# avikde/robobee3d

Measured on AMD Instinct MI355X. Metric: closed-loop MPC steps/sec (QP+dyn), higher is better.
Workload: dtype f32

## Files before the change

### robobee3d_amd/asmgen.py

```python
import os
import struct

from . import symbolic

HERE = os.path.dirname(os.path.abspath(__file__))

SWITCH_PREFIXES = ("UMPC_ASM_", "UMPC_ASM64_", "UMPC_QP_", "UMPC_X_")
NOT_SWITCHES = ("UMPC_QP_KERNEL", "UMPC_QP_NO_ASM", "UMPC_ASM_SKEW_US", "UMPC_ASM_SKEW_GROUPS")


def generator_switches():
    return {k: v for k, v in sorted(os.environ.items()) if k.startswith(SWITCH_PREFIXES) and k not in NOT_SWITCHES}


def switch_banner():
    sw = generator_switches()
    return "// generator switches: " + (" ".join("%s=%s" % kv for kv in sw.items()) if sw else "none (defaults = the shipped kernels)")

XV_COUNT, XV_BASE = 0, 246
NLDS = 160
NVZ = 36
FAC_L, FAC_DI, FAC_Q, FAC_LOEQ, FAC_M = 0, 213, 297, 342, 378
FAC_ROWS = 390
WS_DS, WS_ES, WS_C, WS_XPREV, WS_DY = 390, 435, 474, 475, 520
# ... 137 lines not shown
    while remaining:
        ready = [o for o in remaining if o[1] in final]
        used, emitted = set(), []
        for o in ready:
            if o[2] in used:
                continue
            for o2 in ready:
                if o2[2] not in used and ok(o, o2):
                    used.update((o[2], o2[2]))
                    emitted.append((o, o2) if reg[o[0]] % 2 == 0 else (o2, o))
                    break
        deferred = []
        for o in ready:
            if o[2] in used:
                continue
            if any(ok(o, o2) for o2 in remaining if o2[1] not in final and o2[2] not in used):
                deferred.append(o)
            else:
                used.add(o[2])
                emitted.append((o,))
        if not emitted:
            used.add(deferred[0][2])
            emitted.append((deferred[0],))
        out += emitted
        for o in remaining:
            if o[2] in used:
                indeg[o[0]] -= 1
                if indeg[o[0]] == 0:
                    final.add(o[0])
        remaining = [o for o in remaining if o[2] not in used]
    return out


def solve_plan(s):
    xs, zs, _, _ = slot_maps(s)
    reg = [w_reg(s, k, xs, zs) for k in range(s.nk)]
    fwd = solve_schedule(s, reg, "fwd", same_src=BCAST)
    couples, late = {}, {}
    if BCAST:
        singles = [(k, g[0]) for k, g in enumerate(fwd) if len(g) == 1]
        used = set()
        for a_, (ka, oa) in enumerate(singles):
            if oa[2] in used:
                continue
            for kb, ob in singles[a_ + 1:]:
                if ob[2] not in used and ob[0] == oa[0] and reg[ob[1]] == (reg[oa[1]] ^ 1):
                    couples[oa[2]] = ob[2]
                    used.update((oa[2], ob[2]))
                    break
        moved = {j for j in couples}
        late = {jb: ja for ja, jb in couples.items()}
        byj = {g[0][2]: g for g in fwd if len(g) == 1}
        out = []
        for g in fwd:
            if len(g) == 1 and g[0][2] in moved:
                continue
            if len(g) == 1 and g[0][2] in late:
                out.append(byj[late[g[0][2]]])
            out.append(g)
        fwd = out
    bwd = []
    k = len(fwd) - 1
    while k >= 0:
        g = fwd[k]
        if len(g) == 1 and g[0][2] in late:
            ob, oa = g[0], fwd[k - 1][0]
            h = [(oa[1], oa[0], oa[2]), (ob[1], ob[0], ob[2])]
            if reg[h[0][0]] % 2:
                h.reverse()
            bwd.append(tuple(h))
            k -= 2
            continue
        h = [(sr, d, j) for (d, sr, j) in g]
        if len(h) == 2 and h[0][0] == h[1][0]:
            bwd.append((h[1],))
            bwd.append((h[0],))
        else:
            if len(h) == 2 and reg[h[0][0]] % 2:
                h.reverse()
            bwd.append(tuple(h))
        k -= 1
    units = []
    k = 0
    while k < len(fwd):
        g = fwd[k]
        if len(g) == 1 and g[0][2] in couples and k + 1 < len(fwd) and len(fwd[k + 1]) == 1 and fwd[k + 1][0][2] == couples[g[0][2]]:
            units.append([g[0][2], fwd[k + 1][0][2]])
            k += 2
        else:
            units.append([o[2] for o in g])
            k += 1
    order, pending = [], []
    for u in units:
        if len(u) == 2 and len(order) % 2:
            pending.append(u)
            continue
        order += u
        while pending and len(order) % 2 == 0:
            order += pending.pop(0)
    assert not pending, "odd number of single entries before a trailing pair"
    pos = [0] * len(s.L_i)
    for p_, j in enumerate(order):
        pos[j] = p_
    for g in fwd + bwd:
        if len(g) == 2:
            a, b = pos[g[0][2]], pos[g[1][2]]
            assert a // 2 == b // 2, "paired entries must share an aligned pair"
    return fwd, bwd, pos


def l_positions(N=3, perm=None):
    return solve_plan(symbolic.analyse(N, perm))[2]


def prologue(e, s):
    import numpy as np
    for reg, val in ((S_ALPHA, 1.6), (S_OMA, float(np.float32(1.0) - np.float32(1.6))), (S_SIGMA, 1e-6),
                     (S_RINV, 0.01), (S_RHO, 100.0)):
        e("s_mov_b32", "s%d" % reg, f32bits(val))
        e("s_mov_b32", "s%d" % (reg + 1), f32bits(val))
    _row_ptr(e, S_P, S_WS, FAC_L + NLDS)
    nrest = len(s.L_i) - NLDS + s.nk + s.nx + 2 * s.N * symbolic.NY + 12
    assert A_LO == nrest - 12 - 2 * s.N * symbolic.NY and A_M == nrest - 12 and nrest <= 256
    for r in range(nrest):
        e("global_load_dword", "a%d" % r, "v0", "s[%d:%d]" % (S_P, S_P + 1))
        _adv(e, S_P)
    e("s_mov_b64", "s[%d:%d]" % (S_P, S_P + 1), "s[%d:%d]" % (S_CTRL, S_CTRL + 1))
    xs, zs, _, _ = slot_maps(s)
    for base, n, sl in ((V_X, s.nx, xs), (V_Y, s.nc, zs), (V_Z, s.nc, zs)):
        for r in range(n):
            e("global_load_dword", "v%d" % (base + sl[r]), "v0", "s[%d:%d]" % (S_P, S_P + 1))
            _adv(e, S_P)
    e("s_waitcnt", "vmcnt(0)")


def epilogue(e, s, z_is_l):
    w = 0
    xs, zs, _, _ = slot_maps(s)
    neq = 2 * s.N * symbolic.NY
    for base, n, sl in ((V_X, s.nx, xs), (V_Y, s.nc, zs), (V_Z, s.nc, zs)):
        for r in range(n):
            if base == V_Z and z_is_l and r < neq:
                t = V_RING + r % 16
                e("v_accvgpr_read_b32", "v%d" % t, "a%d" % (A_LO + r))
                e("ds_write_b32", "v1", "v%d" % t, (w // 4) * 1024 + (w % 4) * 4)
            else:
                e("ds_write_b32", "v1", "v%d" % (base + sl[r]), (w // 4) * 1024 + (w % 4) * 4)
            w += 1
    e("s_waitcnt", "vmcnt(0) lgkmcnt(0)")


class Fetcher:

    def __init__(self, e, la=3):
        self.e, self.la = e, la
        self.nds = 0
        self.waited = -1
        self.lds_ahead = int(os.environ.get("UMPC_ASM_LDS_AHEAD", "12" if NRING == 4 else "20"))
        self.merge = int(os.environ.get("UMPC_ASM_LDS_MERGE", "1" if NRING == 4 else "2"))

    def run(self, ops):
        e = self.e
        n = len(ops)
        inst_of = [None] * n
        insts = []
        slots = [None] * NRING
        for i, op in enumerate(ops):
            if op["src"] and op["src"][0] == "L":
                qd = op["src"][1] // 4
                hit = [k for k in slots if k is not None and insts[k]["quad"] == qd]
                if hit:
                    insts[hit[0]]["last"] = i
                    inst_of[i] = hit[0]
                    continue
                free = [sl for sl in range(NRING) if slots[sl] is None]
                sl = free[0] if free else min(range(NRING), key=lambda q: insts[slots[q]]["last"])
                insts.append(dict(quad=qd, first=i, last=i, slot=sl, prev=slots[sl], issued=None))
                slots[sl] = len(insts) - 1
                inst_of[i] = slots[sl]

        def issue(it):
            e("ds_read_b128", "v[%d:%d]" % (ring_base(it["slot"]), ring_base(it["slot"]) + 3), "v1",
              it["quad"] * 1024)
            it["issued"] = self.nds
            self.nds += 1

        next_inst = 0
        atemp = {}
        next_acc = 0
        acc_rr = 0
        for i in range(n):
            while next_acc < n and next_acc < i + self.la:
                op = ops[next_acc]
                if op["src"] and op["src"][0] in ("A", "A2"):
                    t = V_AT + 2 * (acc_rr % N_ATP)
                    acc_rr += 1
                    e("v_accvgpr_read_b32", "v%d" % t, "a%d" % op["src"][1])
                    if op["src"][0] == "A2":
                        e("v_accvgpr_read_b32", "v%d" % (t + 1), "a%d" % op["src"][2])
                    atemp[next_acc] = t
                next_acc += 1
            while next_inst < len(insts):
                it = insts[next_inst]
                prev = insts[it["prev"]] if it["prev"] is not None else None
                if it["first"] <= i + self.lds_ahead and (prev is None or prev["last"] < i):
                    issue(it)
                    next_inst += 1
                else:
                    break
            op = ops[i]
            if op["src"] is None:
                op["emit"](None)
            elif op["src"][0] in ("A", "A2"):
                op["emit"](atemp.pop(i))
            else:
                it = insts[inst_of[i]]
                if it["issued"] is None:
                    assert inst_of[i] == next_inst and (it["prev"] is None or insts[it["prev"]]["last"] < i)
                    issue(it)
                    next_inst += 1
                if it["first"] == i and it["issued"] > self.waited:
                    upto = min(self.nds - 1, it["issued"] + self.merge)
                    e("s_waitcnt", "lgkmcnt(%d)" % min(15, self.nds - 1 - upto))
                    self.waited = upto if self.nds - 1 - upto <= 15 else it["issued"]
                op["emit"](ring_base(it["slot"]) + op["src"][1] % 4)


def _vp(n):
    assert n % 2 == 0
    return ("v[%d:%d]" % (n, n + 1), 0, 1)


def _vb(n):
    lo = n - (n % 2)
    return ("v[%d:%d]" % (lo, lo + 1), n % 2, n % 2)


def _sb(n):
    assert n % 2 == 0
    return ("s[%d:%d]" % (n, n + 1), 0, 0)


def pk(e, mnem, dst, srcs, neg=None):
    assert dst % 2 == 0
    neg = neg or [0] * len(srcs)
    mods = dict(op_sel=[s_[1] for s_ in srcs], op_sel_hi=[s_[2] for s_ in srcs], neg_lo=list(neg), neg_hi=list(neg))
    e(mnem, "v[%d:%d]" % (dst, dst + 1), *[s_[0] for s_ in srcs], mods)


def despace(ops, window=int(os.environ.get("UMPC_ASM_WINDOW", "12"))):
    pending, out = list(ops), []
    last = [frozenset(), frozenset()]
    while pending:
        best, bscore = 0, None
        blocked_w, blocked_r = set(), set()
        for k, o in enumerate(pending[:window]):
            movable = not (o["r"] & blocked_w) and not (o["w"] & blocked_w) and not (o["w"] & blocked_r)
            if movable:
                score = (2 if (o["r"] | o["w"]) & last[1] else 0) + (1 if (o["r"] | o["w"]) & last[0] else 0)
                if bscore is None or score < bscore:
                    best, bscore = k, score
                    if score == 0:
                        break
            blocked_w |= o["w"]
            blocked_r |= o["r"]
        o = pending.pop(best)
        out.append(o)
        last = [last[1], o["w"]]
    return out


def body(e, s, first, capture, plan, lv=False, delta_in_w=False, qzero=frozenset(), lzero=frozenset(), dy3_in_w=False):
    nx, nc, nk = s.nx, s.nc, s.nk
    neq = 2 * s.N * symbolic.NY
    xs, zs, xinv, zinv = slot_maps(s)
    fwd, bwd, lpos = plan

    def wreg(k):
        return w_reg(s, k, xs, zs)
    W = lambda k: "v%d" % wreg(k)
    WX = lambda j: V_W + xs[j]
    WZ = lambda i: V_WZ + zs[i]
    XR = lambda j: V_X + xs[j]
    YR = lambda i: V_Y + zs[i]
    ZR = lambda i: V_Z + zs[i]
    X = lambda j: "v%d" % XR(j)
    Y = lambda i: "v%d" % YR(i)
    Z = lambda i: "v%d" % ZR(i)
    v = lambda n: "v%d" % n
    sA, sO, sS, sRi, sRh = ("s%d" % r for r in (S_ALPHA, S_OMA, S_SIGMA, S_RINV, S_RHO))
    ptr = "s[%d:%d]" % (S_P2, S_P2 + 1)
    f = Fetcher(e)
    ops = []

    def op(src, fn, w=(), r=()):
        ops.append(dict(src=src, emit=fn, w=frozenset(w), r=frozenset(r)))

    assert NVZ == neq and not (lv and first)

    def l_src(j):
        if lpos[j] < NLDS:
            return ("L", lpos[j])
        if lv and lpos[j] < NLDS + NVZ:
            return ("V", V_Z + lpos[j] - NLDS)
        if NLDS + NVZ <= lpos[j] < NLDS + NVZ + XV_COUNT:
            return ("V", XV_BASE + lpos[j] - NLDS - NVZ)
        return ("A", A_L + lpos[j] - NLDS)

    if capture and not delta_in_w:
        _row_ptr(e, S_P2, S_WS, WS_XPREV)
        for j in range(nx):
            e("global_store_dword", "v0", X(j), ptr)
            _adv(e, S_P2)
    for p_ in range(0, nx - 1, 2):
        j0, j1 = xinv[p_], xinv[p_ + 1]
        rw = dict(w=(V_W + p_, V_W + p_ + 1), r=(V_X + p_, V_X + p_ + 1))
        if j0 in qzero and j1 in qzero:
            op(None, lambda t, p_=p_: pk(e, "v_pk_mul_f32", V_W + p_, [_sb(S_SIGMA), _vp(V_X + p_)]), **rw)
        elif j0 in qzero or j1 in qzero:
            jn, h = (j1, 1) if j0 in qzero else (j0, 0)

            def mixed(t, p_=p_, h=h):
                pk(e, "v_pk_mul_f32", V_W + p_, [_sb(S_SIGMA), _vp(V_X + p_)])
                e("v_sub_f32", v(V_W + p_ + h), v(V_W + p_ + h), v(t))
            op(("A", A_Q + jn), mixed, **rw)
        else:
            op(("A2", A_Q + j0, A_Q + j1),
               lambda t, p_=p_: pk(e, "v_pk_fma_f32", V_W + p_, [_sb(S_SIGMA), _vp(V_X + p_), _vp(t)], [0, 0, 1]), **rw)
    if nx % 2:
        jl = xinv[nx - 1]
        if jl in qzero:
            op(None, lambda t, jl=jl: e("v_mul_f32", v(WX(jl)), sS, X(jl)), w=(WX(jl),), r=(XR(jl),))
        else:
            op(("A", A_Q + jl), lambda t, jl=jl: e("v_fma_f32", v(WX(jl)), sS, X(jl), "-" + v(t)), w=(WX(jl),), r=(XR(jl),))
    assert all(zinv[p_] < neq for p_ in range(neq)) and neq % 2 == 0
    for p_ in range(0, neq, 2):
        if lv:
            i0, i1 = zinv[p_], zinv[p_ + 1]
            rw = dict(w=(V_WZ + p_, V_WZ + p_ + 1), r=(V_Y + p_, V_Y + p_ + 1))
            if i0 in lzero and i1 in lzero:
                op(None, lambda t, p_=p_: pk(e, "v_pk_mul_f32", V_WZ + p_, [_sb(S_RINV), _vp(V_Y + p_)], [1, 0]), **rw)
            elif i0 in lzero or i1 in lzero:
                inz, h = (i1, 1) if i0 in lzero else (i0, 0)

                def mixed_z(t, p_=p_, h=h):
                    pk(e, "v_pk_mul_f32", V_WZ + p_, [_sb(S_RINV), _vp(V_Y + p_)], [1, 0])
                    e("v_add_f32", v(V_WZ + p_ + h), v(V_WZ + p_ + h), v(t))
                op(("A", A_LO + inz), mixed_z, **rw)
            else:
                op(("A2", A_LO + i0, A_LO + i1),
                   lambda t, p_=p_: pk(e, "v_pk_fma_f32", V_WZ + p_, [_sb(S_RINV), _vp(V_Y + p_), _vp(t)], [1, 0, 0]), **rw)
        else:
            op(None, lambda t, p_=p_: pk(e, "v_pk_fma_f32", V_WZ + p_, [_sb(S_RINV), _vp(V_Y + p_), _vp(V_Z + p_)], [1, 0, 0]),
               w=(V_WZ + p_, V_WZ + p_ + 1), r=(V_Y + p_, V_Y + p_ + 1, V_Z + p_, V_Z + p_ + 1))
    for i in range(neq, nc):
        op(("A", A_M + 9 + i - neq), lambda t, i=i: e("v_fma_f32", v(WZ(i)), "-" + v(t), Y(i), Z(i)),
           w=(WZ(i),), r=(YR(i), ZR(i)))

    def solve_ops(sched):
        for g in sched:
            if len(g) == 1:
                d, sr, j = g[0]
                src = l_src(j)
                if src[0] == "V":
                    op(None, lambda t, d=d, sr=sr, r=src[1]: e("v_fmac_f32", W(d), v(r), W(sr)),
                       w=(wreg(d),), r=(wreg(d), wreg(sr)))
                else:
                    op(src, lambda t, d=d, sr=sr: e("v_fmac_f32", W(d), v(t), W(sr)),
                       w=(wreg(d),), r=(wreg(d), wreg(sr)))
                continue
            (d0, s0_, j0), (d1, s1_, j1) = g
            rd, r0, r1 = wreg(d0), wreg(s0_), wreg(s1_)
            assert rd % 2 == 0 and wreg(d1) == rd + 1 and r0 // 2 == r1 // 2 and lpos[j0] // 2 == lpos[j1] // 2
            srcp = ("v[%d:%d]" % (r0 - r0 % 2, r0 - r0 % 2 + 1), r0 % 2, r1 % 2)
            rw = dict(w=(rd, rd + 1), r=(rd, rd + 1, r0, r1))
            pe = lpos[j0] - lpos[j0] % 2
            lsel = (lpos[j0] % 2, lpos[j1] % 2)
            if pe < NLDS:
                op(("L", pe), lambda t, rd=rd, srcp=srcp, lsel=lsel:
                   pk(e, "v_pk_fma_f32", rd, [("v[%d:%d]" % (t, t + 1), lsel[0], lsel[1]), srcp, _vp(rd)], [0, 0, 0]), **rw)
            elif (lv and pe < NLDS + NVZ) or NLDS + NVZ <= pe < NLDS + NVZ + XV_COUNT:
                t = V_Z + pe - NLDS if pe < NLDS + NVZ else XV_BASE + pe - NLDS - NVZ
                op(None, lambda _t, t=t, rd=rd, srcp=srcp, lsel=lsel:
                   pk(e, "v_pk_fma_f32", rd, [("v[%d:%d]" % (t, t + 1), lsel[0], lsel[1]), srcp, _vp(rd)], [0, 0, 0]), **rw)
            else:
                src = ("A2", A_L + lpos[j0] - NLDS, A_L + lpos[j1] - NLDS)
                op(src, lambda t, rd=rd, srcp=srcp: pk(e, "v_pk_fma_f32", rd, [_vp(t), srcp, _vp(rd)], [0, 0, 0]), **rw)

    solve_ops(fwd)
    kof = {wreg(k): k for k in range(nk)}
    for r0 in range(V_W, V_Z, 2):
        k0, k1 = kof.get(r0), kof.get(r0 + 1)
        if k0 is not None and k1 is not None:
            op(("A2", A_D + k0, A_D + k1), lambda t, r0=r0: pk(e, "v_pk_mul_f32", r0, [_vp(r0), _vp(t)]),
               w=(r0, r0 + 1), r=(r0, r0 + 1))
        elif k0 is not None or k1 is not None:
            k, r = (k0, r0) if k0 is not None else (k1, r0 + 1)
            op(("A", A_D + k), lambda t, r=r: e("v_mul_f32", v(r), v(t), v(r)), w=(r,), r=(r,))
    solve_ops(bwd)
    f.run(despace(ops) if os.environ.get("UMPC_ASM_DESPACE", "0") == "1" else ops)
    for p_ in range(0, nx - 1, 2):
        t = V_TT + 2 * ((p_ // 2) % 4)
        pk(e, "v_pk_mul_f32", t, [_sb(S_OMA), _vp(V_X + p_)])
        if capture and delta_in_w:
            pk(e, "v_pk_fma_f32", t, [_sb(S_ALPHA), _vp(V_W + p_), _vp(t)])
            pk(e, "v_pk_add_f32", V_W + p_, [_vp(t), _vp(V_X + p_)], [0, 1])
            e("v_pk_mov_b32", "v[%d:%d]" % (V_X + p_, V_X + p_ + 1), "v[%d:%d]" % (t, t + 1), "v[%d:%d]" % (t, t + 1),
              dict(op_sel=[0, 1], op_sel_hi=[0, 0], neg_lo=[0, 0], neg_hi=[0, 0]))
        else:
            pk(e, "v_pk_fma_f32", V_X + p_, [_sb(S_ALPHA), _vp(V_W + p_), _vp(t)])
    if nx % 2:
        jl = xinv[nx - 1]
        e("v_mul_f32", v(V_TT), sO, X(jl))
        if capture and delta_in_w:
            e("v_fma_f32", v(V_TT), sA, v(WX(jl)), v(V_TT))
            e("v_sub_f32", v(WX(jl)), v(V_TT), X(jl))
            e("v_mov_b32", X(jl), v(V_TT))
        else:
            e("v_fma_f32", X(jl), sA, v(WX(jl)), v(V_TT))
    if capture and first and not delta_in_w:
        _row_ptr(e, S_P2, S_WS, WS_DY)
    if not first:
        for p_ in range(0, neq, 2):
            t = V_TT + 2 * ((p_ // 2) % 2)
            pk(e, "v_pk_add_f32", t, [_vp(V_WZ + p_), _vp(V_Y + p_)], [0, 1])
            if capture and delta_in_w:
                pk(e, "v_pk_mul_f32", V_WZ + p_, [_sb(S_ALPHA), _vp(t)])
            elif capture:
                pk(e, "v_pk_mul_f32", t + 4, [_sb(S_ALPHA), _vp(t)])
                for h in range(2):
                    _row_ptr(e, S_P2, S_WS, WS_DY + zinv[p_ + h])
                    e("global_store_dword", "v0", v(t + 4 + h), ptr)
            pk(e, "v_pk_fma_f32", V_Y + p_, [_sb(S_ALPHA), _vp(t), _vp(V_Y + p_)])
    for i in range(nc):
        eq = i < neq
        if eq and not first:
            continue
        if first and eq and i % 16 == 0:
            for w in range(min(16, neq - i)):
                e("v_accvgpr_read_b32", v(V_RING + w), "a%d" % (A_LO + i + w))
        b = V_TT + 4 * (i % 2)
        t1, t2, t3, t4 = v(b), v(b + 1), v(b + 2), v(b + 3)
        if eq:
            rinv, rho = sRi, sRh
        else:
            k = i - neq
            rinv, rho = v(V_AT), v(V_AT + 1)
            e("v_accvgpr_read_b32", rinv, "a%d" % (A_M + 9 + k))
            e("v_accvgpr_read_b32", rho, "a%d" % (A_M + 6 + k))
            e("v_accvgpr_read_b32", v(V_AT + 2), "a%d" % (A_M + k))
            e("v_accvgpr_read_b32", v(V_AT + 3), "a%d" % (A_M + 3 + k))
        nu = v(WZ(i))
        e("v_fma_f32", t1, "-" + rinv, Y(i), Z(i))
        e("v_fma_f32", t1, rinv, nu, t1)
        e("v_mul_f32", t2, sO, Z(i))
        e("v_fma_f32", t1, sA, t1, t2)
        if eq:
            zn = v(V_RING + i % 16)
            e("v_sub_f32", t2, t1, zn)
        else:
            e("v_fma_f32", t3, rinv, Y(i), t1)
            e("v_max_f32", t3, t3, v(V_AT + 2))
            e("v_min_f32", Z(i), t3, v(V_AT + 3))
            e("v_sub_f32", t2, t1, Z(i))
        if dy3_in_w and not eq and not capture:
            e("v_mul_f32", nu, rho, t2)
            e("v_add_f32", Y(i), Y(i), nu)
            continue
        e("v_mul_f32", t2, rho, t2)
        e("v_add_f32", Y(i), Y(i), t2)
        if capture and delta_in_w:
            e("v_mov_b32", nu, t2)
        elif capture:
            if not first:
                _row_ptr(e, S_P2, S_WS, WS_DY + i)
            e("global_store_dword", "v0", t2, ptr)
            if first:
                _adv(e, S_P2)


def program(N=3, perm=None):
    s = symbolic.analyse(N, perm)
    plan = solve_plan(s)
    e = Emit()
    prologue(e, s)
    e("s_cmp_lt_i32", "s%d" % S_ITERS, 1)
    e("s_cbranch_scc1", "9f")
    body(e, s, first=True, capture=True, plan=plan)
    for p_ in range(NVZ):
        e("v_accvgpr_read_b32", "v%d" % (V_Z + p_), "a%d" % (A_L + p_))
    e("s_sub_i32", "s%d" % S_CNT, "s%d" % S_ITERS, 2)
    e("s_cmp_lt_i32", "s%d" % S_CNT, 1)
    e("s_cbranch_scc1", "8f")
    e("label", "7")
    body(e, s, first=False, capture=False, plan=plan, lv=True)
    e("s_sub_i32", "s%d" % S_CNT, "s%d" % S_CNT, 1)
    e("s_cmp_gt_i32", "s%d" % S_CNT, 0)
    e("s_cbranch_scc1", "7b")
    e("label", "8")
    e("s_cmp_lt_i32", "s%d" % S_ITERS, 2)
    e("s_cbranch_scc1", "6f")
    body(e, s, first=False, capture=True, plan=plan, lv=True)
    e("label", "6")
    epilogue(e, s, z_is_l=True)
    e("s_branch", "5f")
    e("label", "9")
    epilogue(e, s, z_is_l=False)
    e("label", "5")
    return e.ins, s


def fmt(t):
    m = t[0]
    if m == "label":
        return "%s:" % t[1]
    mods = ""
    if isinstance(t[-1], dict):
        d = t[-1]
        t = t[:-1]
        mods = " " + " ".join("%s:[%s]" % (k, ",".join(map(str, d[k]))) for k in ("op_sel", "op_sel_hi", "neg_lo", "neg_hi"))
    a = [("0x%x" % x if (m == "s_mov_b32" and isinstance(x, int)) else str(x)) for x in t[1:]]
    if m in ("ds_read_b128", "ds_write_b128", "ds_write_b32"):
        return "%s %s, %s offset:%s" % (m, a[0], a[1], a[2])
    if m in ("global_load_dword", "global_store_dword"):
        return "%s %s, %s, %s" % (m, a[0], a[1], a[2])
    if m == "s_waitcnt":
        return "s_waitcnt " + " ".join(a)
    return "%s %s%s" % (m, ", ".join(a), mods)


def write(path=None, N=3, perm=None):
    path = path or os.path.join(HERE, "csrc", "umpc_admm_asm.h")
    ins, s = program(N, perm)
    lpos = solve_plan(s)[2]
    store_l = " ".join("LDSW_(%d) = -LX_(%d);" % (lpos[j], j) if lpos[j] < NLDS else "ROW_(%d) = -LX_(%d);" % (FAC_L + lpos[j], j)
                       for j in range(len(lpos)))
    used_s = [S_P, S_P + 1, S_CNT, S_P2, S_P2 + 1] + list(range(S_ALPHA, S_RHO + 2))
    clob = ['"memory"', '"scc"', '"vcc"'] + ['"v%d"' % i for i in range(2, V_END)] + \
           ['"a%d"' % i for i in range(256)] + ['"s%d"' % i for i in used_s]
    lab7 = [k for k, t in enumerate(ins) if t == ("label", "7")][0]
    lab8 = [k for k, t in enumerate(ins) if t == ("label", "8")][0]
    out = ["// GENERATED by robobee3d_amd/asmgen.py -- do not edit.", switch_banner(),
           "// ADMM phase of the fp32 step kernel: %d instructions, middle-iteration body %d." % (len(ins), lab8 - lab7),
           "#pragma once",
           "namespace umpcasm {",
           "constexpr int FAC_L = %d, FAC_DI = %d, FAC_Q = %d, FAC_LOEQ = %d, FAC_M = %d, FAC_ROWS = %d;" %
           (FAC_L, FAC_DI, FAC_Q, FAC_LOEQ, FAC_M, FAC_ROWS),
           "constexpr int WS_DS = %d, WS_ES = %d, WS_C = %d, WS_XPREV = %d, WS_DY = %d, WS_ROWS = %d;" %
           (WS_DS, WS_ES, WS_C, WS_XPREV, WS_DY, WS_ROWS),
           "constexpr int LDS_BYTES_PER_LANE = %d;" % (NLDS * 4),
           "}  // namespace umpcasm",
           "// Phase A -> loop hand-off of the factor: entry j of L (CSC order) goes NEGATED to its storage position (asmgen.solve_plan):",
           "// LDS word LDSW_(p) for p < %d, workspace row ROW_(FAC_L + p) (-> AGPR) otherwise." % NLDS,
           "#define UMPC_ASM_STORE_L(LDSW_, ROW_, LX_) do { %s } while (0)" % store_l,
           "// inputs: v0 = 4*robot, v1 = lane LDS address, s[4:5] = workspace, s[6:7] = ctrl, s10 = 4*B, s11 = maxIter",
           "#define UMPC_ADMM_ASM(voff, ldsaddr, ws, ctrl, stride, iters) asm volatile( \\"]
    for t in ins:
        out.append('  "%s\\n" \\' % fmt(t))
    out.append('  : : "{v0}"(voff), "{v1}"(ldsaddr), "{s[4:5]}"(ws), "{s[6:7]}"(ctrl), "{s10}"(stride), "{s11}"(iters) \\')
    out.append("  : " + ", ".join(clob) + ")")
    txt = "\n".join(out) + "\n"
    old = open(path).read() if os.path.exists(path) else None
    if old != txt:
        with open(path, "w") as fh:
            fh.write(txt)
    return path, len(ins)


WS_BASE, CTRL_BASE, STRIDE = 1 << 20, 1 << 30, 4096


def simulate(ins, mem_ws, mem_ctrl, iters, lds=None):
    import numpy as np
    from . import isasim
    lds = np.zeros(NLDS, np.float32) if lds is None else lds
    m = isasim.Machine(ins, regions=[(WS_BASE, STRIDE, mem_ws), (CTRL_BASE, STRIDE, mem_ctrl)],
                       sgpr={S_WS: WS_BASE, S_CTRL: CTRL_BASE, S_STRIDE: STRIDE, S_ITERS: iters}, vgpr={0: 0},
                       lds=lds.view(np.uint32).reshape(1, -1), max_exec=400000)
    return isasim.run(m)


if __name__ == "__main__":
    p, n = write()
    print("wrote", p, n, "instructions")
```

### robobee3d_amd/asmstep.py

```python
import os
import struct

from . import asmgen, symbolic
from .asmgen import (A_D, A_L, A_LO, A_M, A_Q, NLDS, NVZ, S_ALPHA, S_CNT, S_ITERS, S_OMA, S_RHO, S_RINV, S_SIGMA,
                     V_W, V_WZ, V_X, V_Y, V_Z, Emit, f32bits, pk, _sb, _vp)

HERE = os.path.dirname(os.path.abspath(__file__))

PTRS = ["state", "ctrl", "ref", "ws", "out", "stats", "status", "info", "Ib", "gain", "aT0",
        "taskf", "weights", "wl", "wlu", "wlw",
        "done"]
NPTR_RES = 11
INTS = ["stride", "K", "maxIter", "nsub", "plant", "seq"]
TAIL_INTS = ["refstep"]
FLOATS = ["dt", "dtg", "Tmax", "wpr", "wpf", "ws_", "wvr", "wvf", "wds", "wthrust", "wmom",
          "iwpr", "iwpf", "iws", "iwvr", "iwvf", "iwds", "iwthrust", "iwmom",
          "Ib0", "Ib1", "Ib2", "Ibi0", "Ibi1", "Ibi2", "h", "hh", "h6", "taulim", "gpl", "idt", "mbg"]
WNAMES = ["wpr", "wpf", "ws_", "wvr", "wvf", "wds", "wthrust", "wmom"]
WROW = {"ws_": 0, "wds": 1, "wpr": 2, "wpf": 3, "wvr": 4, "wvf": 5, "wthrust": 6, "wmom": 7}
A_W, A_IW = 230, 238
S_PARAM = 4
S_PBLK = 2
S_PTR = {n: 40 + 2 * k for k, n in enumerate(PTRS[:NPTR_RES])}
S_PTR["taskf"], S_PTR["weights"] = 0, 96
S_PTR["wl"], S_PTR["wlu"], S_PTR["wlw"] = 30, 32, 34
S_INT = {"stride": 10, "K": 13, "maxIter": S_ITERS, "nsub": 5, "plant": 39}
S_F = {n: 64 + k for k, n in enumerate(FLOATS)}
assert max(S_F.values()) <= 95
S_STEP, S_SUB, S_RUIZ = 12, 15, 15
S_MBAD, S_MP0 = 62, 14
S_M0, S_M1, S_M2, S_M3 = 30, 32, 34, 36
S_C = {"minscal": 16, "maxscal": 17, "c45": 18, "eps10": 19, "eps": 38, "rho": 6, "rinv": 7, "rmin": 8,
       "rmininv": 9, "infty_ms": 100, "rhotol": 101}
S_TMP = 4
OFF = {}
_o = 0
for _n in PTRS:
    OFF[_n] = _o
    _o += 8
for _n in INTS + FLOATS + TAIL_INTS:
    OFF[_n] = _o
    _o += 4
PARAM_BYTES = _o
HIST_INTS = ["statestep", "outstep", "statusstep", "infostep"]
HIST_OFF = (PARAM_BYTES + 7) // 8 * 8
for _k, _n in enumerate(HIST_INTS):
    OFF[_n] = HIST_OFF + 4 * _k
HIST_BYTES = 4 * len(HIST_INTS)
S_HIST = 32
IMP_OFF = HIST_OFF + HIST_BYTES
assert IMP_OFF % 8 == 0
OFF["imp"], OFF["impstep"] = IMP_OFF, IMP_OFF + 8
IMP_BYTES = 16
S_IMP = 32

VFIRST, VEND = 2, 256
XV_N, XV_B = 10, 246
OPT_RING = int(os.environ.get("UMPC_ASM_RING", "6"))
assert OPT_RING in (4, 6)
OPT_XV = os.environ.get("UMPC_ASM_XV", "1") == "1"
if OPT_RING == 6:
    XV_N, XV_B = 2, 254
OPT_LIMIT_FAST = os.environ.get("UMPC_ASM_LIMIT_FAST", "0") == "1"
OPT_ZSKIP = os.environ.get("UMPC_ASM_ZSKIP", "1") == "1"
OPT_NT = os.environ.get("UMPC_ASM_NT", "1")
NT_PTRS = ("state", "ctrl", "ref", "out", "stats")
A_SPARE, N_SPARE_D = 246, 9
OPT_WS_ST = os.environ.get("UMPC_ASM_WS_ST", "nt")
OPT_WS_LD = os.environ.get("UMPC_ASM_WS_LD", "nt")


class Pool:

    def __init__(self, e):
        self.e = e
        self.free_ = set(range(VFIRST, VEND))
        self.peak = 0
        self.fixed = set()

    def _take(self, regs):
        for r in regs:
            assert r in self.free_, "v%d is not free" % r
            self.free_.discard(r)
        self.peak = max(self.peak, VEND - VFIRST - len(self.free_))

    def reserve(self, lo, n):
        self._take(range(lo, lo + n))
        return lo

    def get(self):
        cand = sorted(self.free_)
        assert cand, "out of VGPRs"
        for r in cand:
            if (r ^ 1) not in self.free_:
                self._take([r])
                return r
        self._take([cand[0]])
        return cand[0]

    def get2(self):
        for r in sorted(self.free_):
            if r % 2 == 0 and r + 1 in self.free_:
                self._take([r, r + 1])
                return r
        raise AssertionError("out of aligned VGPR pairs")

    def get4(self):
        for r in sorted(self.free_):
            if r % 4 == 0 and all(r + k in self.free_ for k in range(4)):
                self._take([r, r + 1, r + 2, r + 3])
                return r
        raise AssertionError("out of aligned VGPR quads")

    def getn(self, n):
        for r in sorted(self.free_):
            if r % 2 == 0 and all(r + k in self.free_ for k in range(n)):
                self._take(range(r, r + n))
                return r
        raise AssertionError("out of consecutive VGPRs")

    def getn_high(self, n):
        r = VEND - n - (VEND - n) % 2
        assert all(r + k in self.free_ for k in range(n)), "top of the register file is not free"
        self._take(range(r, r + n))
        return r

    def free(self, *regs, kill=True):
        for r in regs:
            assert r not in self.free_ and VFIRST <= r < VEND, "double free v%d" % r
            self.free_.add(r)
            if kill:
                self.e("kill", "v%d" % r)

    def free_range(self, lo, n, kill=True):
        self.free(*range(lo, lo + n), kill=kill)


def v(n):
    return "v%d" % n


def SF_(n):
    return "s%d" % S_F[n]


def sg(n):
    return "s%d" % n


def sp(n):
    return "s[%d:%d]" % (n, n + 1)


def vp2(n):
    return "v[%d:%d]" % (n, n + 1)


def P2(n):
    return _vp(n)


def PB(n):
    lo = n - n % 2
    return ("v[%d:%d]" % (lo, lo + 1), n % 2, n % 2)


def PSEL(lo_reg, hi_reg):
    assert lo_reg // 2 == hi_reg // 2
    base = lo_reg - lo_reg % 2
    return ("v[%d:%d]" % (base, base + 1), lo_reg % 2, hi_reg % 2)


def PS(sreg):
    if sreg % 2 == 0:
        return ("s[%d:%d]" % (sreg, sreg + 1), 0, 0)
    return ("s[%d:%d]" % (sreg - 1, sreg), 1, 1)


class Struct:
    def __init__(self, N=3, perm=None):
        s = symbolic.analyse(N, perm)
        self.s = s
        self.plan = asmgen.solve_plan(s)
        self.lpos = self.plan[2]
        self.xs, self.zs, self.xinv, self.zinv = asmgen.slot_maps(s)
        nx, nc = s.nx, s.nc
        self.neq = 2 * s.N * symbolic.NY
        self.col_of = [0] * len(s.A_i)
        self.rows = [[] for _ in range(nc)]
        for j in range(nx):
            for p in range(s.A_p[j], s.A_p[j + 1]):
                self.col_of[p] = j
                self.rows[s.A_i[p]].append(p)
        self.unit = {}
        for p, tag in enumerate(s.A_tag):
            if tag[0] == 'c' and abs(tag[1]) == 1.0 and s.A_i[p] not in self.unit:
                self.unit[s.A_i[p]] = (p, self.col_of[p])
        assert len(self.unit) == nc
        used, pairs = set(), []
        for p in range(len(s.A_i)):
            if p in used:
                continue
            i0, j0 = s.A_i[p], self.col_of[p]
            for q_ in range(p + 1, len(s.A_i)):
                if q_ in used:
                    continue
                i1, j1 = s.A_i[q_], self.col_of[q_]
                if (self.zs[i0] ^ 1) == self.zs[i1] and (j0 == j1 or (self.xs[j0] ^ 1) == self.xs[j1]):
                    lo, hi = (p, q_) if self.zs[i0] % 2 == 0 else (q_, p)
                    pairs.append((lo, hi))
                    used.update((p, q_))
                    break
        self.apairs = pairs
        self.asingles = [p for p in range(len(s.A_i)) if p not in used]
        self.apos = [0] * len(s.A_i)
        k = 0
        for (lo, hi) in pairs:
            self.apos[lo], self.apos[hi] = k, k + 1
            k += 2
        for p in self.asingles:
            self.apos[p] = k
            k += 1
        self.na = k
        self.pair_of = {}
        for (lo, hi) in pairs:
            self.pair_of[lo] = self.pair_of[hi] = (lo, hi)
        NYv = symbolic.NY
        self.qnz = list(range(s.N * NYv)) + [s.N * NYv + k_ * NYv + i for k_ in range(s.N) for i in range(3)]
        self.qslot = {}
        for j in range(s.N * NYv):
            self.qslot[j] = self.xs[j]
        base = s.N * NYv
        for k_ in range(s.N):
            for i in range(3):
                self.qslot[s.N * NYv + k_ * NYv + i] = base + 3 * k_ + i
        self.nq = base + 3 * s.N
        self.qzero = frozenset(j for j in range(nx) if j not in self.qslot)
        lnz = set(range(6)) | set(range(3 * 6, 3 * 6 + 6)) | set(range(4 * 6, 4 * 6 + 3)) | {5 * 6 + 2}
        self.lzero = frozenset(i for i in range(self.neq) if i not in lnz) if s.N == 3 else frozenset()

    def weight_of(self, j):
        N, NYv = self.s.N, symbolic.NY
        if j < N * NYv:
            k, i = divmod(j, NYv)
            return ("wpf" if k == N - 1 else "wpr") if i < 3 else "ws_"
        if j < 2 * N * NYv:
            k, i = divmod(j - N * NYv, NYv)
            return ("wvf" if k == N - 1 else "wvr") if i < 3 else "wds"
        return "wthrust" if (j - 2 * N * NYv) % 3 == 0 else "wmom"


class StepGen:
    def __init__(self, N=3, perm=None, quad=False):
        self.st = Struct(N, perm)
        self.s = self.st.s
        self.e = Emit()
        self.pool = Pool(self.e)
        self.lab = 20
        self.quad = quad
        self.nt = "0" if quad else OPT_NT

    def label(self):
        self.lab += 1
        return str(self.lab)

    def rcp_nr(self, dst, src, t):
        e = self.e
        e("v_rcp_f32", v(dst), v(src))
        e("s_nop", 0)
        e("v_fma_f32", v(t), "-" + v(src), v(dst), 1.0)
        e("v_fma_f32", v(dst), v(t), v(dst), v(dst))

    def rows_ptr(self, voff, first_row):
        e = self.e
        if first_row == 0:
            e("v_mov_b32", v(voff), "v0")
        else:
            e("s_mul_i32", sg(S_TMP), sg(S_INT["stride"]), first_row)
            e("v_add_u32", v(voff), sg(S_TMP), "v0")

    def load_taskf(self):
        e = self.e
        e("s_lshl_b32", sg(S_TMP), sg(S_STEP), 5)
        e("s_load_dwordx2", sp(S_M0), sp(S_PTR["taskf"]), sg(S_TMP), "offset:0")
        e("s_load_dwordx4", "s[%d:%d]" % (S_M0 + 2, S_M0 + 5), sp(S_PTR["taskf"]), sg(S_TMP), "offset:8")
        e("s_load_dwordx2", sp(S_M0 + 6), sp(S_PTR["taskf"]), sg(S_TMP), "offset:24")
        e("s_waitcnt", "vmcnt(0) lgkmcnt(0)")

    def adv(self, voff):
        self.e("v_add_u32", v(voff), sg(S_INT["stride"]), v(voff))

    def advance_ptr(self, ptr, sstep):
        e, lo = self.e, S_PTR[ptr]
        e("s_add_i32", sg(lo), sg(lo), sg(sstep))
        e("s_cmp_lt_u32", sg(lo), sg(sstep))
        e("s_cselect_b32", sg(sstep), 1, 0)
        e("s_add_i32", sg(lo + 1), sg(lo + 1), sg(sstep))

    def impulse(self, Y0, YS):
        e = self.e
        lab_off = self.label()
        lo, hi, st, oh = S_IMP, S_IMP + 1, S_IMP + 2, S_IMP + 3
        e("s_mov_b32", sg(S_TMP), IMP_OFF)
        e("s_load_dwordx4", "s[%d:%d]" % (S_IMP, S_IMP + 3), sp(S_PBLK), sg(S_TMP))
        e("s_waitcnt", "lgkmcnt(0)")
        e("s_cmp_eq_u64", sp(lo), 0)
        e("s_cbranch_scc1", lab_off + "f")
        e("s_mul_hi_u32", sg(oh), sg(S_STEP), sg(st))
        e("s_mul_i32", sg(st), sg(S_STEP), sg(st))
        e("s_add_i32", sg(hi), sg(hi), sg(oh))
        for i in range(6):
            addend = st if i == 0 else S_INT["stride"]
            lab_nc = self.label()
            e("s_add_i32", sg(lo), sg(lo), sg(addend))
            e("s_cmp_gt_u32", sg(addend), sg(lo))
            e("s_cbranch_scc0", lab_nc + "f")
            e("s_add_i32", sg(hi), sg(hi), 1)
            e("label", lab_nc)
            e("global_load_dword", v(YS + i), "v0", sp(lo))
        e("s_waitcnt", "vmcnt(0)")
        for i in range(6):
            e("v_add_f32", v(Y0 + 12 + i), v(Y0 + 12 + i), v(YS + i))
        e("label", lab_off)

    def load_rows(self, ptr, first_row, regs, voff=None):
        own = voff is None
        if own:
            voff = self.pool.get()
        self.rows_ptr(voff, first_row)
        for k, r in enumerate(regs):
            self.e("global_load_dword", r if isinstance(r, str) else v(r), v(voff), sp(S_PTR[ptr]),
                   *(("nt",) if self.nt in ("1", "ld") and ptr in NT_PTRS else (OPT_WS_LD,) if ptr == "ws" and OPT_WS_LD and not self.quad else ()))
            if k + 1 < len(regs):
                self.adv(voff)
        if own:
            self.pool.free(voff, kill=False)

    def store_rows(self, ptr, first_row, regs, voff=None):
        own = voff is None
        if own:
            voff = self.pool.get()
        self.rows_ptr(voff, first_row)
        for k, r in enumerate(regs):
            self.e("global_store_dword", v(voff), v(r), sp(S_PTR[ptr]),
                   *(("nt",) if self.nt in ("1", "st") and ptr in NT_PTRS else ()))
            if k + 1 < len(regs):
                self.adv(voff)
        if own:
            self.pool.free(voff, kill=False)

    def prologue(self):
        e = self.e
        P = sp(S_PARAM)
        e("s_mov_b64", sp(S_PBLK), P)
        P = sp(S_PBLK)
        e("s_load_dwordx16", "s[40:55]", P, OFF["state"])
        e("s_load_dwordx4", "s[56:59]", P, OFF["state"] + 64)
        e("s_load_dwordx2", "s[60:61]", P, OFF["state"] + 80)
        e("s_load_dwordx2", sp(S_PTR["taskf"]), P, OFF["taskf"])
        e("s_load_dwordx2", sp(S_PTR["weights"]), P, OFF["weights"])
        e("s_load_dwordx16", "s[64:79]", P, OFF[FLOATS[0]])
        e("s_load_dwordx16", "s[80:95]", P, OFF[FLOATS[0]] + 64)
        for n in S_INT:
            e("s_load_dword", sg(S_INT[n]), P, OFF[n])
        assert len(FLOATS) == 32
        import numpy as np
        f32 = np.float32
        for reg, val in ((S_ALPHA, 1.6), (S_OMA, float(f32(1.0) - f32(1.6))), (S_SIGMA, 1e-6), (S_RINV, 0.01), (S_RHO, 100.0)):
            e("s_mov_b32", sg(reg), f32bits(val))
            e("s_mov_b32", sg(reg + 1), f32bits(val))
        for name, val in (("minscal", 1e-4), ("maxscal", 1e4), ("c45", float(f32(1.0) / f32(self.s.nx))),
                          ("eps", 1e-4), ("eps10", float(f32(10) * f32(1e-4))), ("rho", 0.1), ("rinv", float(f32(1.0) / f32(0.1))),
                          ("rmin", 1e-6), ("rmininv", float(f32(1.0) / f32(1e-6))),
                          ("infty_ms", float(f32(1e30) * f32(1e-4))), ("rhotol", 1e-4)):
            e("s_mov_b32", sg(S_C[name]), f32bits(val))
        e("s_waitcnt", "lgkmcnt(0)")
        e("s_mov_b32", sg(S_STEP), 0)

    def phase_a(self):
        e, pool, st, s = self.e, self.pool, self.st, self.s
        N, NYv = s.N, symbolic.NY
        nx, nc, neq = s.nx, s.nc, st.neq
        SF = lambda n: sg(S_F[n])
        ST = [pool.get() for _ in range(18)]
        RF = [pool.get() for _ in range(9)]
        T0, EP = pool.get(), [pool.get() for _ in range(N)]
        voff = pool.get()
        self.load_rows("state", 0, ST, voff)
        self.load_rows("ref", 0, RF, voff)
        self.load_rows("ctrl", nx + 2 * nc, [T0] + EP, voff)
        WV = {n: pool.get() for n in WNAMES}
        IWV = {n: pool.get() for n in WNAMES}
        self.WV = WV
        lab_w, lab_w2 = self.label(), self.label()
        e("s_cmp_eq_u64", sp(S_PTR["weights"]), 0)
        e("s_cbranch_scc1", lab_w + "f")
        self.rows_ptr(voff, 0)
        by_row = sorted(WNAMES, key=lambda n: WROW[n])
        for k, n in enumerate(by_row):
            e("global_load_dword", v(WV[n]), v(voff), sp(S_PTR["weights"]))
            if k + 1 < len(by_row):
                self.adv(voff)
        e("s_waitcnt", "vmcnt(0)")
        t = pool.get()
        for n in WNAMES:
            self.rcp_nr(IWV[n], WV[n], t)
        pool.free(t)
        e("s_branch", lab_w2 + "f")
        e("label", lab_w)
        for n in WNAMES:
            e("v_mov_b32", v(WV[n]), SF(n))
            e("v_mov_b32", v(IWV[n]), SF("i" + n.rstrip("_")))
# ... 517 lines not shown
            e("global_store_dword", v(voff), v(cs), sp(S_PTR["ws"]))
        self.store_rows("ctrl", nx + 2 * nc + 1, [RE(neq + k) for k in range(N)], voff)
        pool.free(cinv, d, r, voff, cs, *IWV.values())
        LS = pool.getn(20)
        for qd in range(5):
            e("ds_read_b128", "v[%d:%d]" % (LS + 4 * qd, LS + 4 * qd + 3), "v1", qd * 1024)
        zero = pool.get()
        e("v_mov_b32", v(zero), 0)
        for j in range(nx):
            e("v_accvgpr_write_b32", "a%d" % (A_Q + j), v(RQ(j)) if j in st.qslot else v(zero))
        e("s_waitcnt", "lgkmcnt(0)")
        src = {}
        for i in range(6):
            src[i] = LS + i
            src[3 * 6 + i] = LS + 6 + i
        for i in range(3):
            src[4 * 6 + i] = LS + 12 + i
        for i in range(neq):
            if i in src:
                e("v_mul_f32", v(t), v(src[i]), v(RE(i)))
                e("v_accvgpr_write_b32", "a%d" % (A_LO + i), v(t))
            elif i == 5 * 6 + 2:
                e("v_mul_f32", v(t), SF("dtg"), v(RE(i)))
                e("v_accvgpr_write_b32", "a%d" % (A_LO + i), v(t))
            else:
                e("v_accvgpr_write_b32", "a%d" % (A_LO + i), v(zero))
        for k in range(N):
            e("v_mul_f32", v(t), v(LS + 15), v(RE(neq + k)))
            e("v_accvgpr_write_b32", "a%d" % (A_M + k), v(t))
            e("v_mul_f32", v(t), v(LS + 16), v(RE(neq + k)))
            e("v_accvgpr_write_b32", "a%d" % (A_M + N + k), v(t))
        pool.free(zero, t)
        pool.free_range(LS, 20)
        pool.free_range(self.VE, nc + 1)
        pool.free_range(self.VQ, st.nq + st.nq % 2)

    def factor(self):
        e, pool, st, s = self.e, self.pool, self.st, self.s
        nx, nc, nk, neq = s.nx, s.nc, s.nk, st.neq
        RP, RA = self.RP, self.RA
        lpos = st.lpos
        last_row = {}
        for c in range(nk):
            if s.L_p[c + 1] > s.L_p[c]:
                last_row[c] = s.L_i[s.L_p[c + 1] - 1]
        done_at = {}
        for c, r in last_row.items():
            done_at.setdefault(r, []).append(c)
        nL, Dinv = {}, {}
        asmgen.XV_COUNT, asmgen.XV_BASE = (XV_N if OPT_XV and not self.quad else 0), XV_B
        pool.reserve(246, 10)
        t = pool.get()

        def retire_dinv(k):
            e("v_accvgpr_write_b32", "a%d" % (A_D + k), v(Dinv[k]))
            pool.free(Dinv.pop(k))

        def retire_col(c):
            for j in range(s.L_p[c], s.L_p[c + 1]):
                pos = lpos[j]
                if pos < NLDS:
                    e("ds_write_b32", "v1", v(nL[j]), (pos // 4) * 1024 + (pos % 4) * 4)
                elif NLDS + NVZ <= pos < NLDS + NVZ + asmgen.XV_COUNT:
                    e("v_mov_b32", v(XV_B + pos - NLDS - NVZ), v(nL[j]))
                else:
                    e("v_accvgpr_write_b32", "a%d" % (A_L + pos - NLDS), v(nL[j]))
                pool.free(nL.pop(j))
            retire_dinv(c)

        for op in s.factor_ops:
            k = op["k"]
            src = s.K_src[op["diag"]]
            dk = pool.get()
            if src[0] == 'P':
                e("v_add_f32", v(dk), sg(S_SIGMA), v(RP(src[1])))
                pool.free(RP(src[1]))
            else:
                assert src[0] == 'R'
                i = src[1]
                if i < neq:
                    e("v_mul_f32", v(dk), -1.0, self._vconst_rinv())
                else:
                    e("v_accvgpr_read_b32", v(dk), "a%d" % (A_M + 9 + i - neq))
                    e("s_nop", 0)
                    e("v_mul_f32", v(dk), -1.0, v(dk))
            y = {}
            for (b, p) in op["init"]:
                assert s.K_src[p][0] == 'A'
                y[b] = (RA(s.K_src[p][1]), False)
            for (c, upd, new) in op["elim"]:
                yc, owned = y.pop(c)
                for (lj, row) in upd:
                    if row in y:
                        reg, own = y[row]
                        if own:
                            e("v_fmac_f32", v(reg), v(nL[lj]), v(yc))
                        else:
                            nr = pool.get()
                            e("v_fma_f32", v(nr), v(nL[lj]), v(yc), v(reg))
                            pool.free(reg)
                            y[row] = (nr, True)
                    else:
                        nr = pool.get()
                        e("v_mul_f32", v(nr), v(nL[lj]), v(yc))
                        y[row] = (nr, True)
                nl = pool.get()
                e("v_mul_f32", v(nl), "-" + v(yc), v(Dinv[c]))
                e("v_fmac_f32", v(dk), v(yc), v(nl))
                nL[new] = nl
                pool.free(yc)
            assert not y
            di = pool.get()
            self.rcp_nr(di, dk, t)
            pool.free(dk)
            Dinv[k] = di
            for c in done_at.get(k, []):
                retire_col(c)
            if k not in last_row:
                retire_dinv(k)
        assert not nL and not Dinv
        pool.free(t)
        if self._rinv_reg is not None:
            pool.free(self._rinv_reg)
            self._rinv_reg = None
        if st.na % 2:
            pool.free(self.VA + st.na)
        pool.free(self.VP + nx)

    _rinv_reg = None

    def _vconst_rinv(self):
        if self._rinv_reg is None:
            self._rinv_reg = self.pool.get()
            self.e("v_mov_b32", v(self._rinv_reg), sg(S_RINV))
        return v(self._rinv_reg)

    def admm(self):
        e, pool, st, s = self.e, self.pool, self.st, self.s
        nx, nc = s.nx, s.nc
        left = set(range(VFIRST, VEND)) - pool.free_ - set(range(246, 256))
        assert not left, "phase A leaked registers: %s" % sorted(left)
        pool.reserve(V_W, V_X - V_W)
        pool.reserve(V_X, V_Y - V_X)
        pool.reserve(V_Y, V_Z - V_Y)
        pool.reserve(V_Z, 40)
        voff = 245
        self.load_rows("ctrl", 0, [V_X + st.xs[r] for r in range(nx)] + [V_Y + st.zs[r] for r in range(nc)] +
                       [V_Z + st.zs[r] for r in range(nc)], voff)
        for pad in (V_X + nx, V_Y + nc, V_Z + nc, V_W + nx, V_WZ + nc):
            e("v_mov_b32", v(pad), 0)
        e("s_waitcnt", "vmcnt(0) lgkmcnt(0)")
        plan = st.plan
        zk = dict(qzero=st.qzero, lzero=st.lzero) if OPT_ZSKIP else {}
        asmgen.body(e, s, first=True, capture=True, plan=plan, delta_in_w=True, **zk)
        if self.quad:
            from . import asmquad
            lab6 = self.label()
            e("s_cmp_lt_i32", sg(S_ITERS), 2)
            e("s_cbranch_scc1", lab6 + "f")
            asmquad.section(e, asmquad.QuadPlan(st), self.label)
            e("label", lab6)
        else:
            self._admm_rest(plan, zk)
        for i in range(st.neq):
            pool.free(V_Z + st.zs[i], kill=True)
        pool.free_range(246, 10)


    def _admm_rest(self, plan, zk):
        e, s, st = self.e, self.s, self.st
        import numpy as np
        for p_ in range(NVZ):
            e("v_accvgpr_read_b32", v(V_Z + p_), "a%d" % (A_L + p_))
        lab7, lab6 = self.label(), self.label()
        e("s_sub_i32", sg(S_CNT), sg(S_ITERS), 1)
        e("s_cmp_lt_i32", sg(S_CNT), 1)
        e("s_cbranch_scc1", lab6 + "f")
        e("label", lab7)
        asmgen.body(e, s, first=False, capture=False, plan=plan, lv=True, dy3_in_w=True, **zk)
        e("s_sub_i32", sg(S_CNT), sg(S_CNT), 1)
        e("s_cmp_gt_i32", sg(S_CNT), 0)
        e("s_cbranch_scc1", lab7 + "b")
        k = float(np.float32(1.6) / (np.float32(1.6) - np.float32(1.0)))
        e("s_mov_b32", sg(S_TMP), f32bits(k))
        nx, neq = s.nx, st.neq
        for p_ in range(0, nx - 1, 2):
            pk(e, "v_pk_add_f32", V_W + p_, [P2(V_X + p_), P2(V_W + p_)], [0, 1])
        for p_ in range(0, nx - 1, 2):
            pk(e, "v_pk_mul_f32", V_W + p_, [PS(S_TMP), P2(V_W + p_)])
        if nx % 2:
            jl = st.xinv[nx - 1]
            e("v_sub_f32", v(V_W + st.xs[jl]), v(V_X + st.xs[jl]), v(V_W + st.xs[jl]))
            e("v_mul_f32", v(V_W + st.xs[jl]), sg(S_TMP), v(V_W + st.xs[jl]))
        for p_ in range(0, neq, 2):
            pk(e, "v_pk_add_f32", V_WZ + p_, [P2(V_Y + p_), P2(V_WZ + p_)], [0, 1])
        for p_ in range(0, neq, 2):
            pk(e, "v_pk_mul_f32", V_WZ + p_, [PS(S_TMP), P2(V_WZ + p_)])
        e("label", lab6)

    def phase_c(self):
        e, pool, st, s = self.e, self.pool, self.st, self.s
        N, NYv = s.N, symbolic.NY
        nx, nc, neq = s.nx, s.nc, st.neq
        SF = lambda n: sg(S_F[n])
        g_ = pool.get
        XR = lambda j: V_X + st.xs[j]
        YR = lambda i: V_Y + st.zs[i]
        ZR = lambda i: V_Z + st.zs[i]
        DXR = lambda j: V_W + st.xs[j]
        DYR = lambda i: V_WZ + st.zs[i]
        voff = g_()
        def slot_blocks(n, chunk=16):
            n2 = n + n % 2
            blocks = [(lo, pool.getn(min(chunk, n2 - lo))) for lo in range(0, n2, chunk)]
            def reg(slot):
                for lo, base in reversed(blocks):
                    if slot >= lo:
                        return base + slot - lo
            return reg, [(base, min(chunk, n2 - lo)) for lo, base in blocks]
        DS, dblocks = slot_blocks(nx)
        DR = lambda j: DS(st.xs[j])
        cr, T0 = g_(), g_()
        npark = 0 if self.quad else N_SPARE_D
        self.load_rows("ws", npark, [DR(j) for j in range(npark, nx)], voff)
        if npark:
            for j in range(npark):
                e("v_accvgpr_read_b32", v(DR(j)), "a%d" % (A_SPARE + j))
            e("v_accvgpr_read_b32", v(cr), "a%d" % (A_SPARE + N_SPARE_D))
        else:
            self.load_rows("ws", asmgen.WS_C - asmgen.WS_DS, [cr], voff)
        self.load_rows("ctrl", nx + 2 * nc, [T0], voff)
        e("v_mov_b32", v(DS(nx)), 0)
        zt = [g_() for _ in range(4)]
        NT_ST = ("nt",) if self.nt in ("1", "st") else ()
        self.rows_ptr(voff, 0)
        for r in range(nx):
            e("global_store_dword", v(voff), v(XR(r)), sp(S_PTR["ctrl"]), *NT_ST)
            self.adv(voff)
        for r in range(nc):
            e("global_store_dword", v(voff), v(YR(r)), sp(S_PTR["ctrl"]), *NT_ST)
            self.adv(voff)
        for r in range(nc):
            if r < neq:
                t_ = zt[r % 4]
                e("v_accvgpr_read_b32", v(t_), "a%d" % (A_LO + r))
                e("global_store_dword", v(voff), v(t_), sp(S_PTR["ctrl"]), *NT_ST)
            else:
                e("global_store_dword", v(voff), v(ZR(r)), sp(S_PTR["ctrl"]), *NT_ST)
            self.adv(voff)
        pool.free(*zt)
        e("s_waitcnt", "vmcnt(0)")
        for k in range(0, nx + 1, 2):
            pk(e, "v_pk_mul_f32", V_W + k, [P2(DS(k)), P2(V_W + k)])
            pk(e, "v_pk_mul_f32", V_X + k, [P2(DS(k)), P2(V_X + k)])
        for base, n_ in dblocks:
            pool.free_range(base, n_)
        ES, eblocks = slot_blocks(nc)
        ER = lambda i: ES(st.zs[i])
        ST = [g_() for _ in range(18)]
        RF = [g_() for _ in range(9)]
        self.load_rows("ws", asmgen.WS_ES - asmgen.WS_DS, [ER(i) for i in range(nc)], voff)
        self.load_rows("state", 0, ST, voff)
        self.load_rows("ref", 0, RF, voff)
        e("v_mov_b32", v(ES(nc)), 1.0)
        lab_tk = self.label()
        e("s_cmp_eq_u64", sp(S_PTR["taskf"]), 0)
        e("s_cbranch_scc1", lab_tk + "f")
        self.load_taskf()
        for i in range(3):
            e("v_add_f32", v(RF[i]), sg(S_M0 + i), v(RF[i]))
            e("v_mov_b32", v(RF[3 + i]), sg(S_M0 + 3 + i))
        e("v_mov_b32", v(RF[6]), sg(S_M0 + 6))
        e("v_mov_b32", v(RF[7]), 0)
        e("v_mov_b32", v(RF[8]), sg(S_M0 + 7))
        e("label", lab_tk)
        cinv, t = g_(), g_()
        self.rcp_nr(cinv, cr, t)
        pool.free(cr)
        ibi0, ibi1 = g_(), g_()
        lab_ib, lab_ib2 = self.label(), self.label()
        e("s_cmp_eq_u64", sp(S_PTR["Ib"]), 0)
        e("s_cbranch_scc1", lab_ib + "f")
        self.load_rows("Ib", 0, [ibi0, ibi1], voff)
        e("s_waitcnt", "vmcnt(0)")
        tt = g_()
        for r in (ibi0, ibi1):
            e("v_mov_b32", v(tt), v(r))
            self.rcp_nr(r, tt, t)
        pool.free(tt)
        e("s_branch", lab_ib2 + "f")
        e("label", lab_ib)
        e("v_mov_b32", v(ibi0), SF("Ibi0"))
        e("v_mov_b32", v(ibi1), SF("Ibi1"))
        e("label", lab_ib2)
        e("s_waitcnt", "vmcnt(0)")
        for k in range(0, nc + 1, 2):
            pk(e, "v_pk_mul_f32", V_WZ + k, [P2(ES(k)), P2(V_WZ + k)])
            pk(e, "v_pk_mul_f32", V_Y + k, [P2(ES(k)), P2(V_Y + k)])
        for k in range(0, nc + 1, 2):
            pk(e, "v_pk_mul_f32", V_Y + k, [P2(V_Y + k), PB(cinv)])
        pool.free(cinv)
        zu3 = [g_() for _ in range(N)]
        for k in range(N):
            e("v_rcp_f32", v(zu3[k]), v(ER(neq + k)))
        e("s_nop", 0)
        for k in range(N):
            e("v_mul_f32", v(zu3[k]), v(ZR(neq + k)), v(zu3[k]))
        for base, n_ in eblocks:
            pool.free_range(base, n_)
        for k in range(N):
            pool.free(ZR(neq + k))
        pool.free(V_Z + nc)
        p0, R0, dq0 = ST[0:3], ST[3:12], ST[12:18]
        dtT0 = g_()
        e("v_mul_f32", v(dtT0), SF("dt"), v(T0))
        s0dt = [g_() for _ in range(3)]
        Bdt = [g_() for _ in range(6)]
        for i in range(3):
            e("v_mul_f32", v(s0dt[i]), SF("dt"), v(R0[6 + i]))
            e("v_mul_f32", v(Bdt[i]), "-" + v(R0[i + 3]), v(ibi0))
            e("v_mul_f32", v(Bdt[3 + i]), v(R0[i]), v(ibi1))
        for i in range(6):
            e("v_mul_f32", v(Bdt[i]), SF("dt"), v(Bdt[i]))
        pool.free(ibi0, ibi1)
        ds0 = [g_() for _ in range(3)]
        for r in range(3):
            e("v_mul_f32", v(t), "-" + v(R0[r]), v(dq0[4]))
            e("v_mul_f32", v(ds0[r]), v(R0[r + 3]), v(dq0[3]))
            e("v_add_f32", v(ds0[r]), v(t), v(ds0[r]))
            e("v_mul_f32", v(ds0[r]), -1.0, v(ds0[r]))
        y0 = p0 + R0[6:9]
        dy0 = dq0[0:3] + ds0
# ... 901 lines not shown
```

### robobee3d_amd/csrc/umpc_step_asm.h

```cpp
#pragma once
#include <stddef.h>
#include <stdint.h>
namespace umpcasm {
struct StepParams {
  const void *state;
  const void *ctrl;
  const void *ref;
  const void *ws;
  const void *out;
  const void *stats;
  const void *status;
  const void *info;
  const void *Ib;
  const void *gain;
  const void *aT0;
  const void *taskf;
  const void *weights;
  const void *wl;
  const void *wlu;
  const void *wlw;
  const void *done;
  int32_t stride;
  int32_t K;
  int32_t maxIter;
// ... 4589 lines not shown
  "v_mov_b32 v76, v243\n" \
  "v_fma_f32 v238, -s26, v163, v203\n" \
  "v_fma_f32 v238, s26, v77, v238\n" \
  "v_mul_f32 v239, s22, v203\n" \
  "v_fma_f32 v238, s20, v238, v239\n" \
  "v_sub_f32 v239, v238, v226\n" \
  "v_mul_f32 v239, s28, v239\n" \
  "v_add_f32 v163, v163, v239\n" \
  "v_mov_b32 v77, v239\n" \
  "v_fma_f32 v242, -s26, v161, v201\n" \
  "v_fma_f32 v242, s26, v75, v242\n" \
  "v_mul_f32 v243, s22, v201\n" \
  "v_fma_f32 v242, s20, v242, v243\n" \
  "v_sub_f32 v243, v242, v227\n" \
  "v_mul_f32 v243, s28, v243\n" \
  "v_add_f32 v161, v161, v243\n" \
  "v_mov_b32 v75, v243\n" \
  "v_fma_f32 v238, -s26, v164, v204\n" \
  "v_fma_f32 v238, s26, v78, v238\n" \
  "v_mul_f32 v239, s22, v204\n" \
  "v_fma_f32 v238, s20, v238, v239\n" \
  "v_sub_f32 v239, v238, v228\n" \
  "v_mul_f32 v239, s28, v239\n" \
  "v_add_f32 v164, v164, v239\n" \
  "v_mov_b32 v78, v239\n" \
  "v_fma_f32 v242, -s26, v165, v205\n" \
  "v_fma_f32 v242, s26, v79, v242\n" \
  "v_mul_f32 v243, s22, v205\n" \
  "v_fma_f32 v242, s20, v242, v243\n" \
  "v_sub_f32 v243, v242, v229\n" \
  "v_mul_f32 v243, s28, v243\n" \
  "v_add_f32 v165, v165, v243\n" \
  "v_mov_b32 v79, v243\n" \
  "v_accvgpr_read_b32 v214, a214\n" \
  "v_accvgpr_read_b32 v215, a215\n" \
  "v_accvgpr_read_b32 v216, a216\n" \
  "v_accvgpr_read_b32 v217, a217\n" \
  "v_fma_f32 v238, -s26, v166, v206\n" \
  "v_fma_f32 v238, s26, v80, v238\n" \
  "v_mul_f32 v239, s22, v206\n" \
  "v_fma_f32 v238, s20, v238, v239\n" \
  "v_sub_f32 v239, v238, v214\n" \
  "v_mul_f32 v239, s28, v239\n" \
  "v_add_f32 v166, v166, v239\n" \
  "v_mov_b32 v80, v239\n" \
  "v_fma_f32 v242, -s26, v168, v208\n" \
  "v_fma_f32 v242, s26, v82, v242\n" \
  "v_mul_f32 v243, s22, v208\n" \
  "v_fma_f32 v242, s20, v242, v243\n" \
  "v_sub_f32 v243, v242, v215\n" \
  "v_mul_f32 v243, s28, v243\n" \
  "v_add_f32 v168, v168, v243\n" \
  "v_mov_b32 v82, v243\n" \
  "v_fma_f32 v238, -s26, v169, v209\n" \
  "v_fma_f32 v238, s26, v83, v238\n" \
  "v_mul_f32 v239, s22, v209\n" \
  "v_fma_f32 v238, s20, v238, v239\n" \
  "v_sub_f32 v239, v238, v216\n" \
  "v_mul_f32 v239, s28, v239\n" \
  "v_add_f32 v169, v169, v239\n" \
  "v_mov_b32 v83, v239\n" \
  "v_fma_f32 v242, -s26, v167, v207\n" \
  "v_fma_f32 v242, s26, v81, v242\n" \
  "v_mul_f32 v243, s22, v207\n" \
  "v_fma_f32 v242, s20, v242, v243\n" \
  "v_sub_f32 v243, v242, v217\n" \
  "v_mul_f32 v243, s28, v243\n" \
  "v_add_f32 v167, v167, v243\n" \
  "v_mov_b32 v81, v243\n" \
  "v_accvgpr_read_b32 v230, a227\n" \
  "v_accvgpr_read_b32 v231, a224\n" \
  "v_accvgpr_read_b32 v232, a218\n" \
  "v_accvgpr_read_b32 v233, a221\n" \
  "v_fma_f32 v238, -v230, v170, v210\n" \
  "v_fma_f32 v238, v230, v84, v238\n" \
  "v_mul_f32 v239, s22, v210\n" \
  "v_fma_f32 v238, s20, v238, v239\n" \
  "v_fma_f32 v240, v230, v170, v238\n" \
  "v_max_f32 v240, v240, v232\n" \
  "v_min_f32 v210, v240, v233\n" \
  "v_sub_f32 v239, v238, v210\n" \
  "v_mul_f32 v239, v231, v239\n" \
  "v_add_f32 v170, v170, v239\n" \
  "v_mov_b32 v84, v239\n" \
  "v_accvgpr_read_b32 v230, a228\n" \
  "v_accvgpr_read_b32 v231, a225\n" \
  "v_accvgpr_read_b32 v232, a219\n" \
  "v_accvgpr_read_b32 v233, a222\n" \
  "v_fma_f32 v242, -v230, v171, v211\n" \
  "v_fma_f32 v242, v230, v85, v242\n" \
  "v_mul_f32 v243, s22, v211\n" \
  "v_fma_f32 v242, s20, v242, v243\n" \
  "v_fma_f32 v244, v230, v171, v242\n" \
  "v_max_f32 v244, v244, v232\n" \
  "v_min_f32 v211, v244, v233\n" \
  "v_sub_f32 v243, v242, v211\n" \
  "v_mul_f32 v243, v231, v243\n" \
  "v_add_f32 v171, v171, v243\n" \
  "v_mov_b32 v85, v243\n" \
  "v_accvgpr_read_b32 v230, a229\n" \
  "v_accvgpr_read_b32 v231, a226\n" \
  "v_accvgpr_read_b32 v232, a220\n" \
  "v_accvgpr_read_b32 v233, a223\n" \
  "v_fma_f32 v238, -v230, v172, v212\n" \
  "v_fma_f32 v238, v230, v86, v238\n" \
  "v_mul_f32 v239, s22, v212\n" \
  "v_fma_f32 v238, s20, v238, v239\n" \
  "v_fma_f32 v240, v230, v172, v238\n" \
  "v_max_f32 v240, v240, v232\n" \
  "v_min_f32 v212, v240, v233\n" \
  "v_sub_f32 v239, v238, v212\n" \
  "v_mul_f32 v239, v231, v239\n" \
  "v_add_f32 v172, v172, v239\n" \
  "v_mov_b32 v86, v239\n" \
  "v_accvgpr_read_b32 v174, a0\n" \
  "v_accvgpr_read_b32 v175, a1\n" \
  "v_accvgpr_read_b32 v176, a2\n" \
  "v_accvgpr_read_b32 v177, a3\n" \
  "v_accvgpr_read_b32 v178, a4\n" \
  "v_accvgpr_read_b32 v179, a5\n" \
  "v_accvgpr_read_b32 v180, a6\n" \
  "v_accvgpr_read_b32 v181, a7\n" \
  "v_accvgpr_read_b32 v182, a8\n" \
  "v_accvgpr_read_b32 v183, a9\n" \
  "v_accvgpr_read_b32 v184, a10\n" \
  "v_accvgpr_read_b32 v185, a11\n" \
  "v_accvgpr_read_b32 v186, a12\n" \
  "v_accvgpr_read_b32 v187, a13\n" \
  "v_accvgpr_read_b32 v188, a14\n" \
  "v_accvgpr_read_b32 v189, a15\n" \
  "v_accvgpr_read_b32 v190, a16\n" \
  "v_accvgpr_read_b32 v191, a17\n" \
  "v_accvgpr_read_b32 v192, a18\n" \
  "v_accvgpr_read_b32 v193, a19\n" \
  "v_accvgpr_read_b32 v194, a20\n" \
  "v_accvgpr_read_b32 v195, a21\n" \
  "v_accvgpr_read_b32 v196, a22\n" \
  "v_accvgpr_read_b32 v197, a23\n" \
  "v_accvgpr_read_b32 v198, a24\n" \
  "v_accvgpr_read_b32 v199, a25\n" \
  "v_accvgpr_read_b32 v200, a26\n" \
  "v_accvgpr_read_b32 v201, a27\n" \
  "v_accvgpr_read_b32 v202, a28\n" \
  "v_accvgpr_read_b32 v203, a29\n" \
  "v_accvgpr_read_b32 v204, a30\n" \
  "v_accvgpr_read_b32 v205, a31\n" \
  "v_accvgpr_read_b32 v206, a32\n" \
  "v_accvgpr_read_b32 v207, a33\n" \
  "v_accvgpr_read_b32 v208, a34\n" \
  "v_accvgpr_read_b32 v209, a35\n" \
  "s_sub_i32 s14, s11, 1\n" \
  "s_cmp_lt_i32 s14, 1\n" \
  "s_cbranch_scc1 30f\n" \
  "29:\n" \
  "v_accvgpr_read_b32 v230, a137\n" \
  "v_accvgpr_read_b32 v231, a138\n" \
  "v_accvgpr_read_b32 v232, a139\n" \
  "v_accvgpr_read_b32 v233, a142\n" \
  "v_accvgpr_read_b32 v234, a140\n" \
  "v_accvgpr_read_b32 v235, a141\n" \
  "v_pk_fma_f32 v[2:3], s[24:25], v[88:89], v[230:231] op_sel:[0,0,0] op_sel_hi:[0,1,1] neg_lo:[0,0,1] neg_hi:[0,0,1]\n" \
  "v_accvgpr_read_b32 v236, a143\n" \
  "v_accvgpr_read_b32 v237, a144\n" \
  "v_pk_fma_f32 v[4:5], s[24:25], v[90:91], v[232:233] op_sel:[0,0,0] op_sel_hi:[0,1,1] neg_lo:[0,0,1] neg_hi:[0,0,1]\n" \
  "v_accvgpr_read_b32 v230, a145\n" \
  "v_accvgpr_read_b32 v231, a148\n" \
  "v_pk_fma_f32 v[6:7], s[24:25], v[92:93], v[234:235] op_sel:[0,0,0] op_sel_hi:[0,1,1] neg_lo:[0,0,1] neg_hi:[0,0,1]\n" \
  "v_accvgpr_read_b32 v232, a146\n" \
  "v_accvgpr_read_b32 v233, a147\n" \
  "v_pk_fma_f32 v[8:9], s[24:25], v[94:95], v[236:237] op_sel:[0,0,0] op_sel_hi:[0,1,1] neg_lo:[0,0,1] neg_hi:[0,0,1]\n" \
  "v_accvgpr_read_b32 v234, a149\n" \
  "v_accvgpr_read_b32 v235, a150\n" \
  "v_pk_fma_f32 v[10:11], s[24:25], v[96:97], v[230:231] op_sel:[0,0,0] op_sel_hi:[0,1,1] neg_lo:[0,0,1] neg_hi:[0,0,1]\n" \
  "v_accvgpr_read_b32 v236, a151\n" \
  "v_accvgpr_read_b32 v237, a154\n" \
  "v_pk_fma_f32 v[12:13], s[24:25], v[98:99], v[232:233] op_sel:[0,0,0] op_sel_hi:[0,1,1] neg_lo:[0,0,1] neg_hi:[0,0,1]\n" \
  "v_accvgpr_read_b32 v230, a152\n" \
  "v_accvgpr_read_b32 v231, a153\n" \
  "v_pk_fma_f32 v[14:15], s[24:25], v[100:101], v[234:235] op_sel:[0,0,0] op_sel_hi:[0,1,1] neg_lo:[0,0,1] neg_hi:[0,0,1]\n" \
  "v_accvgpr_read_b32 v232, a155\n" \
  "v_accvgpr_read_b32 v233, a156\n" \
  "v_pk_fma_f32 v[16:17], s[24:25], v[102:103], v[236:237] op_sel:[0,0,0] op_sel_hi:[0,1,1] neg_lo:[0,0,1] neg_hi:[0,0,1]\n" \
  "v_accvgpr_read_b32 v234, a157\n" \
  "v_pk_fma_f32 v[18:19], s[24:25], v[104:105], v[230:231] op_sel:[0,0,0] op_sel_hi:[0,1,1] neg_lo:[0,0,1] neg_hi:[0,0,1]\n" \
  "v_pk_fma_f32 v[20:21], s[24:25], v[106:107], v[232:233] op_sel:[0,0,0] op_sel_hi:[0,1,1] neg_lo:[0,0,1] neg_hi:[0,0,1]\n" \
  "v_accvgpr_read_b32 v236, a161\n" \
  "v_accvgpr_read_b32 v237, a162\n" \
  "v_pk_mul_f32 v[22:23], s[24:25], v[108:109] op_sel:[0,0] op_sel_hi:[0,1] neg_lo:[0,0] neg_hi:[0,0]\n" \
  "v_sub_f32 v22, v22, v234\n" \
  "v_accvgpr_read_b32 v230, a163\n" \
  "v_pk_mul_f32 v[24:25], s[24:25], v[110:111] op_sel:[0,0] op_sel_hi:[0,1] neg_lo:[0,0] neg_hi:[0,0]\n" \
  "v_pk_fma_f32 v[26:27], s[24:25], v[112:113], v[236:237] op_sel:[0,0,0] op_sel_hi:[0,1,1] neg_lo:[0,0,1] neg_hi:[0,0,1]\n" \
  "v_accvgpr_read_b32 v232, a167\n" \
  "v_accvgpr_read_b32 v233, a168\n" \
  "v_pk_mul_f32 v[28:29], s[24:25], v[114:115] op_sel:[0,0] op_sel_hi:[0,1] neg_lo:[0,0] neg_hi:[0,0]\n" \
  "v_sub_f32 v28, v28, v230\n" \
  "v_accvgpr_read_b32 v234, a169\n" \
  "v_pk_mul_f32 v[30:31], s[24:25], v[116:117] op_sel:[0,0] op_sel_hi:[0,1] neg_lo:[0,0] neg_hi:[0,0]\n" \
  "v_pk_fma_f32 v[32:33], s[24:25], v[118:119], v[232:233] op_sel:[0,0,0] op_sel_hi:[0,1,1] neg_lo:[0,0,1] neg_hi:[0,0,1]\n" \
  "v_pk_mul_f32 v[34:35], s[24:25], v[120:121] op_sel:[0,0] op_sel_hi:[0,1] neg_lo:[0,0] neg_hi:[0,0]\n" \
  "v_sub_f32 v34, v34, v234\n" \
  "v_pk_mul_f32 v[36:37], s[24:25], v[122:123] op_sel:[0,0] op_sel_hi:[0,1] neg_lo:[0,0] neg_hi:[0,0]\n" \
  "v_pk_mul_f32 v[38:39], s[24:25], v[124:125] op_sel:[0,0] op_sel_hi:[0,1] neg_lo:[0,0] neg_hi:[0,0]\n" \
  "v_pk_mul_f32 v[40:41], s[24:25], v[126:127] op_sel:[0,0] op_sel_hi:[0,1] neg_lo:[0,0] neg_hi:[0,0]\n" \
  "v_pk_mul_f32 v[42:43], s[24:25], v[128:129] op_sel:[0,0] op_sel_hi:[0,1] neg_lo:[0,0] neg_hi:[0,0]\n" \
  "v_accvgpr_read_b32 v236, a182\n" \
  "v_accvgpr_read_b32 v237, a183\n" \
  "v_pk_mul_f32 v[44:45], s[24:25], v[130:131] op_sel:[0,0] op_sel_hi:[0,1] neg_lo:[0,0] neg_hi:[0,0]\n" \
  "v_accvgpr_read_b32 v230, a184\n" \
  "v_accvgpr_read_b32 v231, a187\n" \
  "v_mul_f32 v46, s24, v132\n" \
  "v_accvgpr_read_b32 v232, a185\n" \
  "v_accvgpr_read_b32 v233, a186\n" \
  "v_pk_fma_f32 v[48:49], s[26:27], v[134:135], v[236:237] op_sel:[0,0,0] op_sel_hi:[0,1,1] neg_lo:[1,0,0] neg_hi:[1,0,0]\n" \
  "ds_read_b128 v[214:217], v1 offset:0\n" \
  "v_pk_fma_f32 v[50:51], s[26:27], v[136:137], v[230:231] op_sel:[0,0,0] op_sel_hi:[0,1,1] neg_lo:[1,0,0] neg_hi:[1,0,0]\n" \
  "v_pk_fma_f32 v[52:53], s[26:27], v[138:139], v[232:233] op_sel:[0,0,0] op_sel_hi:[0,1,1] neg_lo:[1,0,0] neg_hi:[1,0,0]\n" \
  "ds_read_b128 v[218:221], v1 offset:1024\n" \
  "v_pk_mul_f32 v[54:55], s[26:27], v[140:141] op_sel:[0,0] op_sel_hi:[0,1] neg_lo:[1,0] neg_hi:[1,0]\n" \
  "v_pk_mul_f32 v[56:57], s[26:27], v[142:143] op_sel:[0,0] op_sel_hi:[0,1] neg_lo:[1,0] neg_hi:[1,0]\n" \
  "ds_read_b128 v[222:225], v1 offset:2048\n" \
  "v_pk_mul_f32 v[58:59], s[26:27], v[144:145] op_sel:[0,0] op_sel_hi:[0,1] neg_lo:[1,0] neg_hi:[1,0]\n" \
  "v_pk_mul_f32 v[60:61], s[26:27], v[146:147] op_sel:[0,0] op_sel_hi:[0,1] neg_lo:[1,0] neg_hi:[1,0]\n" \
  "v_accvgpr_read_b32 v234, a200\n" \
  "v_accvgpr_read_b32 v235, a201\n" \
  "ds_read_b128 v[226:229], v1 offset:3072\n" \
  "v_pk_mul_f32 v[62:63], s[26:27], v[148:149] op_sel:[0,0] op_sel_hi:[0,1] neg_lo:[1,0] neg_hi:[1,0]\n" \
  "v_accvgpr_read_b32 v236, a202\n" \
  "v_accvgpr_read_b32 v237, a205\n" \
  "v_pk_mul_f32 v[64:65], s[26:27], v[150:151] op_sel:[0,0] op_sel_hi:[0,1] neg_lo:[1,0] neg_hi:[1,0]\n" \
  "v_accvgpr_read_b32 v230, a203\n" \
  "v_accvgpr_read_b32 v231, a204\n" \
  "ds_read_b128 v[246:249], v1 offset:4096\n" \
  "v_pk_fma_f32 v[66:67], s[26:27], v[152:153], v[234:235] op_sel:[0,0,0] op_sel_hi:[0,1,1] neg_lo:[1,0,0] neg_hi:[1,0,0]\n" \
  "v_accvgpr_read_b32 v232, a206\n" \
  "v_accvgpr_read_b32 v233, a207\n" \
  "v_pk_fma_f32 v[68:69], s[26:27], v[154:155], v[236:237] op_sel:[0,0,0] op_sel_hi:[0,1,1] neg_lo:[1,0,0] neg_hi:[1,0,0]\n" \
  "v_accvgpr_read_b32 v234, a208\n" \
  "ds_read_b128 v[250:253], v1 offset:5120\n" \
  "v_pk_fma_f32 v[70:71], s[26:27], v[156:157], v[230:231] op_sel:[0,0,0] op_sel_hi:[0,1,1] neg_lo:[1,0,0] neg_hi:[1,0,0]\n" \
  "v_pk_fma_f32 v[72:73], s[26:27], v[158:159], v[232:233] op_sel:[0,0,0] op_sel_hi:[0,1,1] neg_lo:[1,0,0] neg_hi:[1,0,0]\n" \
  "v_pk_mul_f32 v[74:75], s[26:27], v[160:161] op_sel:[0,0] op_sel_hi:[0,1] neg_lo:[1,0] neg_hi:[1,0]\n" \
  "v_add_f32 v74, v74, v234\n" \
  "v_accvgpr_read_b32 v236, a214\n" \
  "v_pk_mul_f32 v[76:77], s[26:27], v[162:163] op_sel:[0,0] op_sel_hi:[0,1] neg_lo:[1,0] neg_hi:[1,0]\n" \
  "v_pk_mul_f32 v[78:79], s[26:27], v[164:165] op_sel:[0,0] op_sel_hi:[0,1] neg_lo:[1,0] neg_hi:[1,0]\n" \
  "v_accvgpr_read_b32 v230, a227\n" \
  "v_pk_mul_f32 v[80:81], s[26:27], v[166:167] op_sel:[0,0] op_sel_hi:[0,1] neg_lo:[1,0] neg_hi:[1,0]\n" \
  "v_add_f32 v80, v80, v236\n" \
  "v_accvgpr_read_b32 v232, a228\n" \
  "v_pk_mul_f32 v[82:83], s[26:27], v[168:169] op_sel:[0,0] op_sel_hi:[0,1] neg_lo:[1,0] neg_hi:[1,0]\n" \
  "v_accvgpr_read_b32 v234, a229\n" \
  "v_fma_f32 v84, -v230, v170, v210\n" \
  "v_fma_f32 v85, -v232, v171, v211\n" \
  "v_fma_f32 v86, -v234, v172, v212\n" \
  "s_waitcnt lgkmcnt(3)\n" \
  "v_pk_fma_f32 v[60:61], v[214:215], v[14:15], v[60:61] op_sel:[0,0,0] op_sel_hi:[1,1,1] neg_lo:[0,0,0] neg_hi:[0,0,0]\n" \
  "v_pk_fma_f32 v[62:63], v[216:217], v[16:17], v[62:63] op_sel:[0,0,0] op_sel_hi:[1,1,1] neg_lo:[0,0,0] neg_hi:[0,0,0]\n" \
  "ds_read_b128 v[214:217], v1 offset:6144\n" \
  "v_pk_fma_f32 v[64:65], v[218:219], v[18:19], v[64:65] op_sel:[0,0,0] op_sel_hi:[1,1,1] neg_lo:[0,0,0] neg_hi:[0,0,0]\n" \
  "v_pk_fma_f32 v[48:49], v[220:221], v[2:3], v[48:49] op_sel:[0,0,0] op_sel_hi:[1,1,1] neg_lo:[0,0,0] neg_hi:[0,0,0]\n" \
  "ds_read_b128 v[218:221], v1 offset:7168\n" \
  "v_pk_fma_f32 v[54:55], v[222:223], v[2:3], v[54:55] op_sel:[0,0,0] op_sel_hi:[1,1,1] neg_lo:[0,0,0] neg_hi:[0,0,0]\n" \
  "v_pk_fma_f32 v[60:61], v[224:225], v[8:9], v[60:61] op_sel:[0,0,0] op_sel_hi:[1,1,1] neg_lo:[0,0,0] neg_hi:[0,0,0]\n" \
  "ds_read_b128 v[222:225], v1 offset:8192\n" \
  "s_waitcnt lgkmcnt(3)\n" \
  "v_pk_fma_f32 v[54:55], v[226:227], v[8:9], v[54:55] op_sel:[0,0,0] op_sel_hi:[1,1,1] neg_lo:[0,0,0] neg_hi:[0,0,0]\n" \
  "v_pk_fma_f32 v[62:63], v[228:229], v[10:11], v[62:63] op_sel:[0,0,0] op_sel_hi:[1,1,1] neg_lo:[0,0,0] neg_hi:[0,0,0]\n" \
  "ds_read_b128 v[226:229], v1 offset:9216\n" \
  "v_pk_fma_f32 v[56:57], v[246:247], v[10:11], v[56:57] op_sel:[0,0,0] op_sel_hi:[1,1,1] neg_lo:[0,0,0] neg_hi:[0,0,0]\n" \
  "v_pk_fma_f32 v[64:65], v[248:249], v[12:13], v[64:65] op_sel:[0,0,0] op_sel_hi:[1,1,1] neg_lo:[0,0,0] neg_hi:[0,0,0]\n" \
  "ds_read_b128 v[246:249], v1 offset:10240\n" \
  "v_pk_fma_f32 v[58:59], v[250:251], v[12:13], v[58:59] op_sel:[0,0,0] op_sel_hi:[1,1,1] neg_lo:[0,0,0] neg_hi:[0,0,0]\n" \
  "v_pk_fma_f32 v[60:61], v[252:253], v[32:33], v[60:61] op_sel:[0,0,0] op_sel_hi:[1,1,1] neg_lo:[0,0,0] neg_hi:[0,0,0]\n" \
  "ds_read_b128 v[250:253], v1 offset:11264\n" \
  "s_waitcnt lgkmcnt(3)\n" \
  "v_pk_fma_f32 v[78:79], v[214:215], v[32:33], v[78:79] op_sel:[0,0,0] op_sel_hi:[1,1,1] neg_lo:[0,0,0] neg_hi:[0,0,0]\n" \
  "v_pk_fma_f32 v[62:63], v[216:217], v[34:35], v[62:63] op_sel:[0,0,0] op_sel_hi:[1,1,1] neg_lo:[0,0,0] neg_hi:[0,0,0]\n" \
  "ds_read_b128 v[214:217], v1 offset:12288\n" \
  "v_pk_fma_f32 v[80:81], v[218:219], v[34:35], v[80:81] op_sel:[0,0,0] op_sel_hi:[1,1,1] neg_lo:[0,0,0] neg_hi:[0,0,0]\n" \
  "v_pk_fma_f32 v[64:65], v[220:221], v[36:37], v[64:65] op_sel:[0,0,0] op_sel_hi:[1,1,1] neg_lo:[0,0,0] neg_hi:[0,0,0]\n" \
  "ds_read_b128 v[218:221], v1 offset:13312\n" \
  "v_pk_fma_f32 v[82:83], v[222:223], v[36:37], v[82:83] op_sel:[0,0,0] op_sel_hi:[1,1,1] neg_lo:[0,0,0] neg_hi:[0,0,0]\n" \
  "v_pk_fma_f32 v[24:25], v[224:225], v[52:53], v[24:25] op_sel:[0,0,0] op_sel_hi:[1,1,1] neg_lo:[0,0,0] neg_hi:[0,0,0]\n" \
  "ds_read_b128 v[222:225], v1 offset:14336\n" \
  "s_waitcnt lgkmcnt(3)\n" \
  "v_pk_fma_f32 v[6:7], v[226:227], v[52:53], v[6:7] op_sel:[0,0,0] op_sel_hi:[1,1,1] neg_lo:[0,0,0] neg_hi:[0,0,0]\n" \
  "v_pk_fma_f32 v[20:21], v[228:229], v[66:67], v[20:21] op_sel:[0,0,0] op_sel_hi:[1,1,1] neg_lo:[0,0,0] neg_hi:[0,0,0]\n" \
  "ds_read_b128 v[226:229], v1 offset:15360\n" \
  "v_pk_fma_f32 v[54:55], v[246:247], v[26:27], v[54:55] op_sel:[0,0,0] op_sel_hi:[1,1,1] neg_lo:[0,0,0] neg_hi:[0,0,0]\n" \
  "v_pk_fma_f32 v[72:73], v[248:249], v[26:27], v[72:73] op_sel:[0,0,0] op_sel_hi:[1,1,1] neg_lo:[0,0,0] neg_hi:[0,0,0]\n" \
  "ds_read_b128 v[246:249], v1 offset:16384\n" \
  "v_pk_fma_f32 v[78:79], v[250:251], v[26:27], v[78:79] op_sel:[0,0,0] op_sel_hi:[1,1,1] neg_lo:[0,0,0] neg_hi:[0,0,0]\n" \
  "v_pk_fma_f32 v[56:57], v[252:253], v[28:29], v[56:57] op_sel:[0,0,0] op_sel_hi:[1,1,1] neg_lo:[0,0,0] neg_hi:[0,0,0]\n" \
  "ds_read_b128 v[250:253], v1 offset:17408\n" \
  "s_waitcnt lgkmcnt(3)\n" \
  "v_pk_fma_f32 v[74:75], v[214:215], v[28:29], v[74:75] op_sel:[0,0,0] op_sel_hi:[1,1,1] neg_lo:[0,0,0] neg_hi:[0,0,0]\n" \
  "v_pk_fma_f32 v[80:81], v[216:217], v[28:29], v[80:81] op_sel:[0,0,0] op_sel_hi:[1,1,1] neg_lo:[0,0,0] neg_hi:[0,0,0]\n" \
  "ds_read_b128 v[214:217], v1 offset:18432\n" \
  "v_pk_fma_f32 v[58:59], v[218:219], v[30:31], v[58:59] op_sel:[0,0,0] op_sel_hi:[1,1,1] neg_lo:[0,0,0] neg_hi:[0,0,0]\n" \
  "v_pk_fma_f32 v[82:83], v[220:221], v[30:31], v[82:83] op_sel:[0,0,0] op_sel_hi:[1,1,1] neg_lo:[0,0,0] neg_hi:[0,0,0]\n" \
  "ds_read_b128 v[218:221], v1 offset:19456\n" \
  "v_pk_fma_f32 v[76:77], v[222:223], v[30:31], v[76:77] op_sel:[0,0,0] op_sel_hi:[1,1,1] neg_lo:[0,0,0] neg_hi:[0,0,0]\n" \
  "v_pk_fma_f32 v[76:77], v[224:225], v[42:43], v[76:77] op_sel:[0,0,0] op_sel_hi:[1,1,1] neg_lo:[0,0,0] neg_hi:[0,0,0]\n" \
  "ds_read_b128 v[222:225], v1 offset:20480\n" \
  "s_waitcnt lgkmcnt(3)\n" \
  "v_pk_fma_f32 v[76:77], v[226:227], v[42:43], v[76:77] op_sel:[0,1,0] op_sel_hi:[1,0,1] neg_lo:[0,0,0] neg_hi:[0,0,0]\n" \
  "v_fmac_f32 v38, v228, v84\n" \
  "v_fmac_f32 v41, v229, v85\n" \
  "ds_read_b128 v[226:229], v1 offset:21504\n" \
  "v_fmac_f32 v44, v246, v86\n" \
  "v_fmac_f32 v50, v247, v4\n" \
  "v_fmac_f32 v56, v248, v4\n" \
  "v_fmac_f32 v5, v249, v51\n" \
  "ds_read_b128 v[246:249], v1 offset:22528\n" \
  "v_fmac_f32 v38, v250, v66\n" \
  "v_fmac_f32 v38, v251, v67\n" \
  "v_fmac_f32 v22, v252, v68\n" \
  "v_fmac_f32 v38, v253, v68\n" \
  "ds_read_b128 v[250:253], v1 offset:23552\n" \
  "s_waitcnt lgkmcnt(3)\n" \
  "v_fmac_f32 v70, v214, v39\n" \
  "v_fmac_f32 v71, v215, v39\n" \
  "v_fmac_f32 v69, v216, v39\n" \
  "v_fmac_f32 v70, v217, v40\n" \
  "ds_read_b128 v[214:217], v1 offset:24576\n" \
  "v_fmac_f32 v71, v218, v40\n" \
  "v_fmac_f32 v69, v219, v40\n" \
  "v_fmac_f32 v75, v220, v42\n" \
  "v_fmac_f32 v75, v221, v43\n" \
  "ds_read_b128 v[218:221], v1 offset:25600\n" \
  "v_fmac_f32 v82, v222, v45\n" \
  "v_fmac_f32 v83, v223, v45\n" \
  "v_fmac_f32 v82, v224, v46\n" \
  "v_fmac_f32 v83, v225, v46\n" \
  "ds_read_b128 v[222:225], v1 offset:26624\n" \
  "s_waitcnt lgkmcnt(3)\n" \
  "v_fmac_f32 v81, v226, v46\n" \
  "v_pk_fma_f32 v[54:55], v[228:229], v[48:49], v[54:55] op_sel:[0,0,0] op_sel_hi:[1,1,1] neg_lo:[0,0,0] neg_hi:[0,0,0]\n" \
  "ds_read_b128 v[226:229], v1 offset:27648\n" \
  "v_pk_fma_f32 v[20:21], v[246:247], v[48:49], v[20:21] op_sel:[0,0,0] op_sel_hi:[1,1,1] neg_lo:[0,0,0] neg_hi:[0,0,0]\n" \
  "v_pk_fma_f32 v[22:23], v[248:249], v[50:51], v[22:23] op_sel:[0,0,0] op_sel_hi:[1,1,1] neg_lo:[0,0,0] neg_hi:[0,0,0]\n" \
  "ds_read_b128 v[246:249], v1 offset:21504\n" \
  "v_pk_fma_f32 v[54:55], v[250:251], v[60:61], v[54:55] op_sel:[0,0,0] op_sel_hi:[1,1,1] neg_lo:[0,0,0] neg_hi:[0,0,0]\n" \
  "v_pk_fma_f32 v[78:79], v[252:253], v[60:61], v[78:79] op_sel:[0,0,0] op_sel_hi:[1,1,1] neg_lo:[0,0,0] neg_hi:[0,0,0]\n" \
  "ds_read_b128 v[250:253], v1 offset:28672\n" \
  "s_waitcnt lgkmcnt(3)\n" \
  "v_pk_fma_f32 v[56:57], v[214:215], v[62:63], v[56:57] op_sel:[0,0,0] op_sel_hi:[1,1,1] neg_lo:[0,0,0] neg_hi:[0,0,0]\n" \
  "v_pk_fma_f32 v[80:81], v[216:217], v[62:63], v[80:81] op_sel:[0,0,0] op_sel_hi:[1,1,1] neg_lo:[0,0,0] neg_hi:[0,0,0]\n" \
  "ds_read_b128 v[214:217], v1 offset:29696\n" \
  "v_pk_fma_f32 v[58:59], v[218:219], v[64:65], v[58:59] op_sel:[0,0,0] op_sel_hi:[1,1,1] neg_lo:[0,0,0] neg_hi:[0,0,0]\n" \
  "v_pk_fma_f32 v[82:83], v[220:221], v[64:65], v[82:83] op_sel:[0,0,0] op_sel_hi:[1,1,1] neg_lo:[0,0,0] neg_hi:[0,0,0]\n" \
  "ds_read_b128 v[218:221], v1 offset:30720\n" \
  "v_pk_fma_f32 v[70:71], v[222:223], v[24:25], v[70:71] op_sel:[0,0,0] op_sel_hi:[1,1,1] neg_lo:[0,0,0] neg_hi:[0,0,0]\n" \
  "v_pk_fma_f32 v[6:7], v[224:225], v[24:25], v[6:7] op_sel:[0,0,0] op_sel_hi:[1,1,1] neg_lo:[0,0,0] neg_hi:[0,0,0]\n" \
  "ds_read_b128 v[222:225], v1 offset:31744\n" \
  "s_waitcnt lgkmcnt(3)\n" \
  "v_pk_fma_f32 v[76:77], v[226:227], v[24:25], v[76:77] op_sel:[0,0,0] op_sel_hi:[1,1,1] neg_lo:[0,0,0] neg_hi:[0,0,0]\n" \
  "v_pk_fma_f32 v[80:81], v[228:229], v[44:45], v[80:81] op_sel:[0,0,0] op_sel_hi:[1,1,1] neg_lo:[0,0,0] neg_hi:[0,0,0]\n" \
  "ds_read_b128 v[226:229], v1 offset:32768\n" \
  "v_fmac_f32 v56, v247, v50\n" \
  "ds_read_b128 v[246:249], v1 offset:33792\n" \
  "v_fmac_f32 v78, v250, v44\n" \
  "v_fmac_f32 v79, v251, v44\n" \
  "v_pk_fma_f32 v[20:21], v[252:253], v[54:55], v[20:21] op_sel:[0,0,0] op_sel_hi:[1,1,1] neg_lo:[0,0,0] neg_hi:[0,0,0]\n" \
  "ds_read_b128 v[250:253], v1 offset:34816\n" \
  "s_waitcnt lgkmcnt(3)\n" \
  "v_pk_fma_f32 v[72:73], v[214:215], v[54:55], v[72:73] op_sel:[0,0,0] op_sel_hi:[1,1,1] neg_lo:[0,0,0] neg_hi:[0,0,0]\n" \
  "v_pk_fma_f32 v[78:79], v[216:217], v[54:55], v[78:79] op_sel:[0,0,0] op_sel_hi:[1,1,1] neg_lo:[0,0,0] neg_hi:[0,0,0]\n" \
  "ds_read_b128 v[214:217], v1 offset:35840\n" \
  "v_pk_fma_f32 v[74:75], v[218:219], v[56:57], v[74:75] op_sel:[0,0,0] op_sel_hi:[1,1,1] neg_lo:[0,0,0] neg_hi:[0,0,0]\n" \
  "v_pk_fma_f32 v[80:81], v[220:221], v[56:57], v[80:81] op_sel:[0,0,0] op_sel_hi:[1,1,1] neg_lo:[0,0,0] neg_hi:[0,0,0]\n" \
  "ds_read_b128 v[218:221], v1 offset:36864\n" \
  "v_pk_fma_f32 v[82:83], v[222:223], v[58:59], v[82:83] op_sel:[0,0,0] op_sel_hi:[1,1,1] neg_lo:[0,0,0] neg_hi:[0,0,0]\n" \
  "v_pk_fma_f32 v[6:7], v[224:225], v[58:59], v[6:7] op_sel:[0,0,0] op_sel_hi:[1,1,1] neg_lo:[0,0,0] neg_hi:[0,0,0]\n" \
  "ds_read_b128 v[222:225], v1 offset:37888\n" \
  "s_waitcnt lgkmcnt(3)\n" \
  "v_pk_fma_f32 v[76:77], v[226:227], v[58:59], v[76:77] op_sel:[0,0,0] op_sel_hi:[1,1,1] neg_lo:[0,0,0] neg_hi:[0,0,0]\n" \
  "v_fmac_f32 v22, v228, v56\n" \
  "v_fmac_f32 v5, v229, v57\n" \
  "ds_read_b128 v[226:229], v1 offset:38912\n" \
  "v_fmac_f32 v5, v246, v23\n" \
  "v_fmac_f32 v69, v247, v23\n" \
  "v_fmac_f32 v71, v248, v70\n" \
  "v_fmac_f32 v69, v249, v70\n" \
  "ds_read_b128 v[246:249], v1 offset:39936\n" \
  "v_pk_fma_f32 v[72:73], v[250:251], v[20:21], v[72:73] op_sel:[0,0,0] op_sel_hi:[1,1,1] neg_lo:[0,0,0] neg_hi:[0,0,0]\n" \
  "v_pk_fma_f32 v[78:79], v[252:253], v[20:21], v[78:79] op_sel:[0,0,0] op_sel_hi:[1,1,1] neg_lo:[0,0,0] neg_hi:[0,0,0]\n" \
  "s_waitcnt lgkmcnt(2)\n" \
  "v_pk_fma_f32 v[74:75], v[214:215], v[22:23], v[74:75] op_sel:[0,0,0] op_sel_hi:[1,1,1] neg_lo:[0,0,0] neg_hi:[0,0,0]\n" \
  "v_pk_fma_f32 v[6:7], v[216:217], v[70:71], v[6:7] op_sel:[0,0,0] op_sel_hi:[1,1,1] neg_lo:[0,0,0] neg_hi:[0,0,0]\n" \
  "v_pk_fma_f32 v[76:77], v[218:219], v[70:71], v[76:77] op_sel:[0,0,0] op_sel_hi:[1,1,1] neg_lo:[0,0,0] neg_hi:[0,0,0]\n" \
  "v_fmac_f32 v38, v220, v20\n" \
  "v_fmac_f32 v38, v221, v21\n" \
  "v_fmac_f32 v38, v222, v22\n" \
  "v_fmac_f32 v80, v223, v22\n" \
  "v_fmac_f32 v83, v224, v82\n" \
  "v_fmac_f32 v81, v225, v82\n" \
  "s_waitcnt lgkmcnt(0)\n" \
  "v_fmac_f32 v6, v226, v71\n" \
  "v_fmac_f32 v69, v227, v71\n" \
  "v_fmac_f32 v76, v228, v71\n" \
  "v_pk_fma_f32 v[78:79], v[246:247], v[72:73], v[78:79] op_sel:[0,0,0] op_sel_hi:[1,1,1] neg_lo:[0,0,0] neg_hi:[0,0,0]\n" \
  "v_pk_fma_f32 v[6:7], v[248:249], v[82:83], v[6:7] op_sel:[0,0,0] op_sel_hi:[1,1,1] neg_lo:[0,0,0] neg_hi:[0,0,0]\n" \
  "v_pk_fma_f32 v[76:77], v[174:175], v[82:83], v[76:77] op_sel:[0,0,0] op_sel_hi:[1,1,1] neg_lo:[0,0,0] neg_hi:[0,0,0]\n" \
  "v_fmac_f32 v38, v229, v72\n" \
  "v_fmac_f32 v41, v176, v72\n" \
  "v_fmac_f32 v38, v177, v73\n" \
  "v_fmac_f32 v41, v178, v73\n" \
  "v_fmac_f32 v38, v179, v74\n" \
  "v_fmac_f32 v41, v180, v74\n" \
  "v_fmac_f32 v6, v181, v83\n" \
  "v_fmac_f32 v76, v182, v83\n" \
  "v_fmac_f32 v81, v183, v83\n" \
  "v_fmac_f32 v41, v184, v38\n" \
  "v_fmac_f32 v78, v185, v38\n" \
  "v_fmac_f32 v79, v186, v38\n" \
  "v_fmac_f32 v80, v187, v38\n" \
  "v_fmac_f32 v78, v188, v41\n" \
  "v_fmac_f32 v79, v189, v41\n" \
  "v_fmac_f32 v80, v190, v41\n" \
  "v_fmac_f32 v79, v191, v78\n" \
  "v_fmac_f32 v80, v192, v78\n" \
  "v_pk_fma_f32 v[6:7], v[194:195], v[78:79], v[6:7] op_sel:[0,0,0] op_sel_hi:[1,1,1] neg_lo:[0,0,0] neg_hi:[0,0,0]\n" \
  "v_fmac_f32 v80, v193, v79\n" \
  "v_fmac_f32 v6, v196, v79\n" \
  "v_fmac_f32 v80, v197, v74\n" \
  "v_fmac_f32 v5, v198, v80\n" \
  "v_fmac_f32 v6, v199, v80\n" \
  "v_fmac_f32 v7, v200, v80\n" \
  "v_fmac_f32 v6, v201, v5\n" \
  "v_fmac_f32 v7, v202, v5\n" \
  "v_fmac_f32 v69, v203, v5\n" \
  "v_fmac_f32 v75, v204, v5\n" \
  "v_fmac_f32 v81, v205, v5\n" \
  "v_fmac_f32 v7, v206, v6\n" \
  "v_fmac_f32 v69, v207, v6\n" \
  "v_fmac_f32 v75, v208, v6\n" \
  "v_accvgpr_read_b32 v236, a38\n" \
  "v_accvgpr_read_b32 v237, a39\n" \
  "v_fmac_f32 v81, v209, v6\n" \
  "v_accvgpr_read_b32 v230, a40\n" \
  "v_pk_fma_f32 v[76:77], v[254:255], v[6:7], v[76:77] op_sel:[0,0,0] op_sel_hi:[1,1,1] neg_lo:[0,0,0] neg_hi:[0,0,0]\n" \
  "v_accvgpr_read_b32 v232, a41\n" \
  "v_pk_fma_f32 v[76:77], v[236:237], v[6:7], v[76:77] op_sel:[0,1,0] op_sel_hi:[1,0,1] neg_lo:[0,0,0] neg_hi:[0,0,0]\n" \
  "v_accvgpr_read_b32 v234, a42\n" \
  "v_fmac_f32 v69, v230, v7\n" \
  "v_accvgpr_read_b32 v236, a43\n" \
  "v_fmac_f32 v75, v232, v7\n" \
  "v_accvgpr_read_b32 v230, a44\n" \
  "v_fmac_f32 v81, v234, v7\n" \
  "v_accvgpr_read_b32 v232, a45\n" \
  "v_fmac_f32 v76, v236, v69\n" \
  "v_accvgpr_read_b32 v234, a46\n" \
  "v_fmac_f32 v77, v230, v69\n" \
  "v_accvgpr_read_b32 v236, a47\n" \
  "v_fmac_f32 v75, v232, v69\n" \
  "v_accvgpr_read_b32 v230, a48\n" \
  "v_fmac_f32 v81, v234, v69\n" \
  "v_accvgpr_read_b32 v232, a49\n" \
  "v_fmac_f32 v77, v236, v76\n" \
  "v_accvgpr_read_b32 v234, a50\n" \
  "v_fmac_f32 v75, v230, v76\n" \
  "v_accvgpr_read_b32 v236, a51\n" \
  "v_fmac_f32 v81, v232, v76\n" \
  "v_accvgpr_read_b32 v230, a52\n" \
  "v_fmac_f32 v75, v234, v77\n" \
  "v_accvgpr_read_b32 v232, a62\n" \
  "v_accvgpr_read_b32 v233, a63\n" \
  "v_fmac_f32 v81, v236, v77\n" \
  "v_accvgpr_read_b32 v234, a64\n" \
  "v_accvgpr_read_b32 v235, a129\n" \
  "v_fmac_f32 v81, v230, v75\n" \
  "v_accvgpr_read_b32 v236, a130\n" \
  "v_accvgpr_read_b32 v237, a131\n" \
  "v_pk_mul_f32 v[2:3], v[2:3], v[232:233] op_sel:[0,0] op_sel_hi:[1,1] neg_lo:[0,0] neg_hi:[0,0]\n" \
  "v_accvgpr_read_b32 v230, a65\n" \
  "v_accvgpr_read_b32 v231, a66\n" \
  "v_pk_mul_f32 v[4:5], v[4:5], v[234:235] op_sel:[0,0] op_sel_hi:[1,1] neg_lo:[0,0] neg_hi:[0,0]\n" \
  "v_accvgpr_read_b32 v232, a67\n" \
  "v_accvgpr_read_b32 v233, a70\n" \
  "v_pk_mul_f32 v[6:7], v[6:7], v[236:237] op_sel:[0,0] op_sel_hi:[1,1] neg_lo:[0,0] neg_hi:[0,0]\n" \
  "v_accvgpr_read_b32 v234, a68\n" \
  "v_accvgpr_read_b32 v235, a69\n" \
  "v_pk_mul_f32 v[8:9], v[8:9], v[230:231] op_sel:[0,0] op_sel_hi:[1,1] neg_lo:[0,0] neg_hi:[0,0]\n" \
  "v_accvgpr_read_b32 v236, a53\n" \
  "v_accvgpr_read_b32 v237, a54\n" \
  "v_pk_mul_f32 v[10:11], v[10:11], v[232:233] op_sel:[0,0] op_sel_hi:[1,1] neg_lo:[0,0] neg_hi:[0,0]\n" \
  "v_accvgpr_read_b32 v230, a55\n" \
  "v_accvgpr_read_b32 v231, a58\n" \
  "v_pk_mul_f32 v[12:13], v[12:13], v[234:235] op_sel:[0,0] op_sel_hi:[1,1] neg_lo:[0,0] neg_hi:[0,0]\n" \
  "v_accvgpr_read_b32 v232, a56\n" \
  "v_accvgpr_read_b32 v233, a57\n" \
  "v_pk_mul_f32 v[14:15], v[14:15], v[236:237] op_sel:[0,0] op_sel_hi:[1,1] neg_lo:[0,0] neg_hi:[0,0]\n" \
  "v_accvgpr_read_b32 v234, a94\n" \
  "v_accvgpr_read_b32 v235, a97\n" \
  "v_pk_mul_f32 v[16:17], v[16:17], v[230:231] op_sel:[0,0] op_sel_hi:[1,1] neg_lo:[0,0] neg_hi:[0,0]\n" \
  "v_accvgpr_read_b32 v236, a100\n" \
  "v_accvgpr_read_b32 v237, a109\n" \
  "v_pk_mul_f32 v[18:19], v[18:19], v[232:233] op_sel:[0,0] op_sel_hi:[1,1] neg_lo:[0,0] neg_hi:[0,0]\n" \
  "v_accvgpr_read_b32 v230, a105\n" \
  "v_accvgpr_read_b32 v231, a107\n" \
  "v_pk_mul_f32 v[20:21], v[20:21], v[234:235] op_sel:[0,0] op_sel_hi:[1,1] neg_lo:[0,0] neg_hi:[0,0]\n" \
  "v_accvgpr_read_b32 v232, a92\n" \
  "v_accvgpr_read_b32 v233, a95\n" \
  "v_pk_mul_f32 v[22:23], v[22:23], v[236:237] op_sel:[0,0] op_sel_hi:[1,1] neg_lo:[0,0] neg_hi:[0,0]\n" \
  "v_accvgpr_read_b32 v234, a98\n" \
  "v_accvgpr_read_b32 v235, a103\n" \
  "v_pk_mul_f32 v[24:25], v[24:25], v[230:231] op_sel:[0,0] op_sel_hi:[1,1] neg_lo:[0,0] neg_hi:[0,0]\n" \
  "v_accvgpr_read_b32 v236, a101\n" \
  "v_accvgpr_read_b32 v237, a102\n" \
  "v_pk_mul_f32 v[26:27], v[26:27], v[232:233] op_sel:[0,0] op_sel_hi:[1,1] neg_lo:[0,0] neg_hi:[0,0]\n" \
  "v_accvgpr_read_b32 v230, a71\n" \
  "v_accvgpr_read_b32 v231, a72\n" \
  "v_pk_mul_f32 v[28:29], v[28:29], v[234:235] op_sel:[0,0] op_sel_hi:[1,1] neg_lo:[0,0] neg_hi:[0,0]\n" \
  "v_accvgpr_read_b32 v232, a73\n" \
  "v_accvgpr_read_b32 v233, a76\n" \
  "v_pk_mul_f32 v[30:31], v[30:31], v[236:237] op_sel:[0,0] op_sel_hi:[1,1] neg_lo:[0,0] neg_hi:[0,0]\n" \
  "v_accvgpr_read_b32 v234, a74\n" \
  "v_accvgpr_read_b32 v235, a75\n" \
  "v_pk_mul_f32 v[32:33], v[32:33], v[230:231] op_sel:[0,0] op_sel_hi:[1,1] neg_lo:[0,0] neg_hi:[0,0]\n" \
  "v_accvgpr_read_b32 v236, a118\n" \
  "v_accvgpr_read_b32 v237, a113\n" \
  "v_pk_mul_f32 v[34:35], v[34:35], v[232:233] op_sel:[0,0] op_sel_hi:[1,1] neg_lo:[0,0] neg_hi:[0,0]\n" \
  "v_accvgpr_read_b32 v230, a114\n" \
  "v_accvgpr_read_b32 v231, a119\n" \
  "v_pk_mul_f32 v[36:37], v[36:37], v[234:235] op_sel:[0,0] op_sel_hi:[1,1] neg_lo:[0,0] neg_hi:[0,0]\n" \
  "v_accvgpr_read_b32 v232, a115\n" \
  "v_accvgpr_read_b32 v233, a116\n" \
  "v_pk_mul_f32 v[38:39], v[38:39], v[236:237] op_sel:[0,0] op_sel_hi:[1,1] neg_lo:[0,0] neg_hi:[0,0]\n" \
  "v_accvgpr_read_b32 v234, a117\n" \
  "v_accvgpr_read_b32 v235, a123\n" \
  "v_pk_mul_f32 v[40:41], v[40:41], v[230:231] op_sel:[0,0] op_sel_hi:[1,1] neg_lo:[0,0] neg_hi:[0,0]\n" \
  "v_accvgpr_read_b32 v236, a124\n" \
  "v_pk_mul_f32 v[42:43], v[42:43], v[232:233] op_sel:[0,0] op_sel_hi:[1,1] neg_lo:[0,0] neg_hi:[0,0]\n" \
  "v_accvgpr_read_b32 v230, a77\n" \
  "v_accvgpr_read_b32 v231, a78\n" \
  "v_pk_mul_f32 v[44:45], v[44:45], v[234:235] op_sel:[0,0] op_sel_hi:[1,1] neg_lo:[0,0] neg_hi:[0,0]\n" \
  "v_accvgpr_read_b32 v232, a79\n" \
  "v_accvgpr_read_b32 v233, a82\n" \
  "v_mul_f32 v46, v236, v46\n" \
  "v_accvgpr_read_b32 v234, a80\n" \
  "v_accvgpr_read_b32 v235, a81\n" \
  "v_pk_mul_f32 v[48:49], v[48:49], v[230:231] op_sel:[0,0] op_sel_hi:[1,1] neg_lo:[0,0] neg_hi:[0,0]\n" \
  "v_accvgpr_read_b32 v236, a93\n" \
  "v_accvgpr_read_b32 v237, a96\n" \
  "v_pk_mul_f32 v[50:51], v[50:51], v[232:233] op_sel:[0,0] op_sel_hi:[1,1] neg_lo:[0,0] neg_hi:[0,0]\n" \
  "v_accvgpr_read_b32 v230, a99\n" \
  "v_accvgpr_read_b32 v231, a108\n" \
  "v_pk_mul_f32 v[52:53], v[52:53], v[234:235] op_sel:[0,0] op_sel_hi:[1,1] neg_lo:[0,0] neg_hi:[0,0]\n" \
  "v_accvgpr_read_b32 v232, a104\n" \
  "v_accvgpr_read_b32 v233, a106\n" \
  "v_pk_mul_f32 v[54:55], v[54:55], v[236:237] op_sel:[0,0] op_sel_hi:[1,1] neg_lo:[0,0] neg_hi:[0,0]\n" \
  "v_accvgpr_read_b32 v234, a83\n" \
  "v_accvgpr_read_b32 v235, a84\n" \
  "v_pk_mul_f32 v[56:57], v[56:57], v[230:231] op_sel:[0,0] op_sel_hi:[1,1] neg_lo:[0,0] neg_hi:[0,0]\n" \
  "v_accvgpr_read_b32 v236, a85\n" \
  "v_accvgpr_read_b32 v237, a88\n" \
  "v_pk_mul_f32 v[58:59], v[58:59], v[232:233] op_sel:[0,0] op_sel_hi:[1,1] neg_lo:[0,0] neg_hi:[0,0]\n" \
  "v_accvgpr_read_b32 v230, a86\n" \
  "v_accvgpr_read_b32 v231, a87\n" \
  "v_pk_mul_f32 v[60:61], v[60:61], v[234:235] op_sel:[0,0] op_sel_hi:[1,1] neg_lo:[0,0] neg_hi:[0,0]\n" \
  "v_accvgpr_read_b32 v232, a89\n" \
  "v_accvgpr_read_b32 v233, a90\n" \
  "v_pk_mul_f32 v[62:63], v[62:63], v[236:237] op_sel:[0,0] op_sel_hi:[1,1] neg_lo:[0,0] neg_hi:[0,0]\n" \
  "v_accvgpr_read_b32 v234, a91\n" \
  "v_accvgpr_read_b32 v235, a132\n" \
  "v_pk_mul_f32 v[64:65], v[64:65], v[230:231] op_sel:[0,0] op_sel_hi:[1,1] neg_lo:[0,0] neg_hi:[0,0]\n" \
  "v_accvgpr_read_b32 v236, a125\n" \
  "v_accvgpr_read_b32 v237, a127\n" \
  "v_pk_mul_f32 v[66:67], v[66:67], v[232:233] op_sel:[0,0] op_sel_hi:[1,1] neg_lo:[0,0] neg_hi:[0,0]\n" \
  "v_accvgpr_read_b32 v230, a110\n" \
  "v_accvgpr_read_b32 v231, a111\n" \
  "v_pk_mul_f32 v[68:69], v[68:69], v[234:235] op_sel:[0,0] op_sel_hi:[1,1] neg_lo:[0,0] neg_hi:[0,0]\n" \
  "v_accvgpr_read_b32 v232, a112\n" \
  "v_accvgpr_read_b32 v233, a135\n" \
  "v_pk_mul_f32 v[70:71], v[70:71], v[236:237] op_sel:[0,0] op_sel_hi:[1,1] neg_lo:[0,0] neg_hi:[0,0]\n" \
  "v_accvgpr_read_b32 v234, a133\n" \
  "v_accvgpr_read_b32 v235, a134\n" \
  "v_pk_mul_f32 v[72:73], v[72:73], v[230:231] op_sel:[0,0] op_sel_hi:[1,1] neg_lo:[0,0] neg_hi:[0,0]\n" \
  "v_accvgpr_read_b32 v236, a120\n" \
  "v_accvgpr_read_b32 v237, a121\n" \
  "v_pk_mul_f32 v[74:75], v[74:75], v[232:233] op_sel:[0,0] op_sel_hi:[1,1] neg_lo:[0,0] neg_hi:[0,0]\n" \
  "v_accvgpr_read_b32 v230, a122\n" \
  "v_accvgpr_read_b32 v231, a136\n" \
  "v_pk_mul_f32 v[76:77], v[76:77], v[234:235] op_sel:[0,0] op_sel_hi:[1,1] neg_lo:[0,0] neg_hi:[0,0]\n" \
  "v_accvgpr_read_b32 v232, a126\n" \
  "v_accvgpr_read_b32 v233, a128\n" \
  "v_pk_mul_f32 v[78:79], v[78:79], v[236:237] op_sel:[0,0] op_sel_hi:[1,1] neg_lo:[0,0] neg_hi:[0,0]\n" \
  "v_accvgpr_read_b32 v234, a59\n" \
  "v_accvgpr_read_b32 v235, a60\n" \
  "v_pk_mul_f32 v[80:81], v[80:81], v[230:231] op_sel:[0,0] op_sel_hi:[1,1] neg_lo:[0,0] neg_hi:[0,0]\n" \
  "v_accvgpr_read_b32 v236, a61\n" \
  "v_pk_mul_f32 v[82:83], v[82:83], v[232:233] op_sel:[0,0] op_sel_hi:[1,1] neg_lo:[0,0] neg_hi:[0,0]\n" \
  "v_accvgpr_read_b32 v230, a52\n" \
  "v_pk_mul_f32 v[84:85], v[84:85], v[234:235] op_sel:[0,0] op_sel_hi:[1,1] neg_lo:[0,0] neg_hi:[0,0]\n" \
  "v_accvgpr_read_b32 v232, a51\n" \
  "v_mul_f32 v86, v236, v86\n" \
  "v_accvgpr_read_b32 v234, a50\n" \
  "v_fmac_f32 v75, v230, v81\n" \
  "v_accvgpr_read_b32 v236, a49\n" \
  "v_fmac_f32 v77, v232, v81\n" \
  "v_accvgpr_read_b32 v230, a48\n" \
  "v_fmac_f32 v77, v234, v75\n" \
  "v_accvgpr_read_b32 v232, a47\n" \
  "v_fmac_f32 v76, v236, v81\n" \
  "v_accvgpr_read_b32 v234, a46\n" \
  "v_fmac_f32 v76, v230, v75\n" \
  "v_accvgpr_read_b32 v236, a45\n" \
  "v_fmac_f32 v76, v232, v77\n" \
  "v_accvgpr_read_b32 v230, a44\n" \
  "v_fmac_f32 v69, v234, v81\n" \
  "v_accvgpr_read_b32 v232, a43\n" \
  "v_fmac_f32 v69, v236, v75\n" \
  "v_accvgpr_read_b32 v234, a42\n" \
  "v_fmac_f32 v69, v230, v77\n" \
  "v_accvgpr_read_b32 v236, a41\n" \
  "v_fmac_f32 v69, v232, v76\n" \
  "v_accvgpr_read_b32 v230, a40\n" \
  "v_fmac_f32 v7, v234, v81\n" \
  "v_accvgpr_read_b32 v232, a39\n" \
  "v_accvgpr_read_b32 v233, a38\n" \
  "v_fmac_f32 v7, v236, v75\n" \
  "v_fmac_f32 v7, v230, v69\n" \
  "v_pk_fma_f32 v[6:7], v[232:233], v[76:77], v[6:7] op_sel:[0,1,0] op_sel_hi:[1,0,1] neg_lo:[0,0,0] neg_hi:[0,0,0]\n" \
  "v_pk_fma_f32 v[6:7], v[254:255], v[76:77], v[6:7] op_sel:[0,0,0] op_sel_hi:[1,1,1] neg_lo:[0,0,0] neg_hi:[0,0,0]\n" \
  "v_fmac_f32 v6, v209, v81\n" \
  "v_fmac_f32 v6, v208, v75\n" \
  "v_fmac_f32 v6, v207, v69\n" \
  "v_fmac_f32 v6, v206, v7\n" \
  "v_fmac_f32 v5, v205, v81\n" \
  "v_fmac_f32 v5, v204, v75\n" \
  "v_fmac_f32 v5, v203, v69\n" \
  "v_fmac_f32 v5, v202, v7\n" \
  "v_fmac_f32 v5, v201, v6\n" \
  "v_fmac_f32 v80, v200, v7\n" \
  "v_fmac_f32 v80, v199, v6\n" \
  "v_fmac_f32 v80, v198, v5\n" \
  "v_fmac_f32 v74, v197, v80\n" \
  "v_fmac_f32 v79, v196, v6\n" \
  "v_fmac_f32 v79, v193, v80\n" \
  "v_pk_fma_f32 v[78:79], v[194:195], v[6:7], v[78:79] op_sel:[0,0,0] op_sel_hi:[1,1,1] neg_lo:[0,0,0] neg_hi:[0,0,0]\n" \
  "v_fmac_f32 v78, v192, v80\n" \
  "v_fmac_f32 v78, v191, v79\n" \
  "v_fmac_f32 v41, v190, v80\n" \
  "v_fmac_f32 v41, v189, v79\n" \
  "v_fmac_f32 v41, v188, v78\n" \
  "v_fmac_f32 v38, v187, v80\n" \
  "v_fmac_f32 v38, v186, v79\n" \
  "v_fmac_f32 v38, v185, v78\n" \
  "v_fmac_f32 v38, v184, v41\n" \
  "v_fmac_f32 v83, v183, v81\n" \
  "v_fmac_f32 v83, v182, v76\n" \
  "v_fmac_f32 v83, v181, v6\n" \
  "v_fmac_f32 v74, v180, v41\n" \
  "v_fmac_f32 v74, v179, v38\n" \
  "v_fmac_f32 v73, v178, v41\n" \
  "v_fmac_f32 v73, v177, v38\n" \
  "v_fmac_f32 v72, v176, v41\n" \
  "v_fmac_f32 v72, v229, v38\n" \
  "v_pk_fma_f32 v[82:83], v[174:175], v[76:77], v[82:83] op_sel:[0,0,0] op_sel_hi:[1,1,1] neg_lo:[0,0,0] neg_hi:[0,0,0]\n" \
  "v_pk_fma_f32 v[82:83], v[248:249], v[6:7], v[82:83] op_sel:[0,0,0] op_sel_hi:[1,1,1] neg_lo:[0,0,0] neg_hi:[0,0,0]\n" \
  "v_pk_fma_f32 v[72:73], v[246:247], v[78:79], v[72:73] op_sel:[0,0,0] op_sel_hi:[1,1,1] neg_lo:[0,0,0] neg_hi:[0,0,0]\n" \
  "ds_read_b128 v[246:249], v1 offset:33792\n" \
  "v_fmac_f32 v71, v228, v76\n" \
  "v_fmac_f32 v71, v227, v69\n" \
  "v_fmac_f32 v71, v226, v6\n" \
  "ds_read_b128 v[226:229], v1 offset:32768\n" \
  "v_fmac_f32 v82, v225, v81\n" \
  "v_fmac_f32 v82, v224, v83\n" \
  "v_fmac_f32 v22, v223, v80\n" \
  "v_fmac_f32 v22, v222, v38\n" \
  "ds_read_b128 v[222:225], v1 offset:31744\n" \
  "v_fmac_f32 v21, v221, v38\n" \
  "v_fmac_f32 v20, v220, v38\n" \
  "v_pk_fma_f32 v[70:71], v[218:219], v[76:77], v[70:71] op_sel:[0,0,0] op_sel_hi:[1,1,1] neg_lo:[0,0,0] neg_hi:[0,0,0]\n" \
  "ds_read_b128 v[218:221], v1 offset:30720\n" \
  "v_pk_fma_f32 v[70:71], v[216:217], v[6:7], v[70:71] op_sel:[0,0,0] op_sel_hi:[1,1,1] neg_lo:[0,0,0] neg_hi:[0,0,0]\n" \
  "v_pk_fma_f32 v[22:23], v[214:215], v[74:75], v[22:23] op_sel:[0,0,0] op_sel_hi:[1,1,1] neg_lo:[0,0,0] neg_hi:[0,0,0]\n" \
  "ds_read_b128 v[214:217], v1 offset:29696\n" \
  "v_pk_fma_f32 v[20:21], v[252:253], v[78:79], v[20:21] op_sel:[0,0,0] op_sel_hi:[1,1,1] neg_lo:[0,0,0] neg_hi:[0,0,0]\n" \
  "v_pk_fma_f32 v[20:21], v[250:251], v[72:73], v[20:21] op_sel:[0,0,0] op_sel_hi:[1,1,1] neg_lo:[0,0,0] neg_hi:[0,0,0]\n" \
  "ds_read_b128 v[250:253], v1 offset:28672\n" \
  "s_waitcnt lgkmcnt(3)\n" \
  "v_fmac_f32 v70, v249, v69\n" \
  "v_fmac_f32 v70, v248, v71\n" \
  "v_fmac_f32 v23, v247, v69\n" \
  "v_fmac_f32 v23, v246, v5\n" \
  "ds_read_b128 v[246:249], v1 offset:21504\n" \
  "v_fmac_f32 v57, v229, v5\n" \
  "v_fmac_f32 v56, v228, v22\n" \
  "v_pk_fma_f32 v[58:59], v[226:227], v[76:77], v[58:59] op_sel:[0,0,0] op_sel_hi:[1,1,1] neg_lo:[0,0,0] neg_hi:[0,0,0]\n" \
  "ds_read_b128 v[226:229], v1 offset:27648\n" \
  "v_pk_fma_f32 v[58:59], v[224:225], v[6:7], v[58:59] op_sel:[0,0,0] op_sel_hi:[1,1,1] neg_lo:[0,0,0] neg_hi:[0,0,0]\n" \
  "v_pk_fma_f32 v[58:59], v[222:223], v[82:83], v[58:59] op_sel:[0,0,0] op_sel_hi:[1,1,1] neg_lo:[0,0,0] neg_hi:[0,0,0]\n" \
  "ds_read_b128 v[222:225], v1 offset:26624\n" \
  "s_waitcnt lgkmcnt(3)\n" \
  "v_pk_fma_f32 v[56:57], v[220:221], v[80:81], v[56:57] op_sel:[0,0,0] op_sel_hi:[1,1,1] neg_lo:[0,0,0] neg_hi:[0,0,0]\n" \
  "v_pk_fma_f32 v[56:57], v[218:219], v[74:75], v[56:57] op_sel:[0,0,0] op_sel_hi:[1,1,1] neg_lo:[0,0,0] neg_hi:[0,0,0]\n" \
  "ds_read_b128 v[218:221], v1 offset:25600\n" \
  "v_pk_fma_f32 v[54:55], v[216:217], v[78:79], v[54:55] op_sel:[0,0,0] op_sel_hi:[1,1,1] neg_lo:[0,0,0] neg_hi:[0,0,0]\n" \
  "v_pk_fma_f32 v[54:55], v[214:215], v[72:73], v[54:55] op_sel:[0,0,0] op_sel_hi:[1,1,1] neg_lo:[0,0,0] neg_hi:[0,0,0]\n" \
  "ds_read_b128 v[214:217], v1 offset:24576\n" \
  "v_pk_fma_f32 v[54:55], v[252:253], v[20:21], v[54:55] op_sel:[0,0,0] op_sel_hi:[1,1,1] neg_lo:[0,0,0] neg_hi:[0,0,0]\n" \
  "v_fmac_f32 v44, v251, v79\n" \
  "v_fmac_f32 v44, v250, v78\n" \
  "ds_read_b128 v[250:253], v1 offset:23552\n" \
  "s_waitcnt lgkmcnt(3)\n" \
  "v_fmac_f32 v50, v247, v56\n" \
  "ds_read_b128 v[246:249], v1 offset:22528\n" \
  "v_pk_fma_f32 v[44:45], v[228:229], v[80:81], v[44:45] op_sel:[0,0,0] op_sel_hi:[1,1,1] neg_lo:[0,0,0] neg_hi:[0,0,0]\n" \
  "v_pk_fma_f32 v[24:25], v[226:227], v[76:77], v[24:25] op_sel:[0,0,0] op_sel_hi:[1,1,1] neg_lo:[0,0,0] neg_hi:[0,0,0]\n" \
  "ds_read_b128 v[226:229], v1 offset:21504\n" \
  "v_pk_fma_f32 v[24:25], v[224:225], v[6:7], v[24:25] op_sel:[0,0,0] op_sel_hi:[1,1,1] neg_lo:[0,0,0] neg_hi:[0,0,0]\n" \
  "v_pk_fma_f32 v[24:25], v[222:223], v[70:71], v[24:25] op_sel:[0,0,0] op_sel_hi:[1,1,1] neg_lo:[0,0,0] neg_hi:[0,0,0]\n" \
  "ds_read_b128 v[222:225], v1 offset:20480\n" \
  "s_waitcnt lgkmcnt(3)\n" \
  "v_pk_fma_f32 v[64:65], v[220:221], v[82:83], v[64:65] op_sel:[0,0,0] op_sel_hi:[1,1,1] neg_lo:[0,0,0] neg_hi:[0,0,0]\n" \
  "v_pk_fma_f32 v[64:65], v[218:219], v[58:59], v[64:65] op_sel:[0,0,0] op_sel_hi:[1,1,1] neg_lo:[0,0,0] neg_hi:[0,0,0]\n" \
  "ds_read_b128 v[218:221], v1 offset:19456\n" \
  "v_pk_fma_f32 v[62:63], v[216:217], v[80:81], v[62:63] op_sel:[0,0,0] op_sel_hi:[1,1,1] neg_lo:[0,0,0] neg_hi:[0,0,0]\n" \
  "v_pk_fma_f32 v[62:63], v[214:215], v[56:57], v[62:63] op_sel:[0,0,0] op_sel_hi:[1,1,1] neg_lo:[0,0,0] neg_hi:[0,0,0]\n" \
  "ds_read_b128 v[214:217], v1 offset:18432\n" \
  "v_pk_fma_f32 v[60:61], v[252:253], v[78:79], v[60:61] op_sel:[0,0,0] op_sel_hi:[1,1,1] neg_lo:[0,0,0] neg_hi:[0,0,0]\n" \
  "v_pk_fma_f32 v[60:61], v[250:251], v[54:55], v[60:61] op_sel:[0,0,0] op_sel_hi:[1,1,1] neg_lo:[0,0,0] neg_hi:[0,0,0]\n" \
  "ds_read_b128 v[250:253], v1 offset:17408\n" \
  "s_waitcnt lgkmcnt(3)\n" \
  "v_pk_fma_f32 v[50:51], v[248:249], v[22:23], v[50:51] op_sel:[0,0,0] op_sel_hi:[1,1,1] neg_lo:[0,0,0] neg_hi:[0,0,0]\n" \
  "v_pk_fma_f32 v[48:49], v[246:247], v[20:21], v[48:49] op_sel:[0,0,0] op_sel_hi:[1,1,1] neg_lo:[0,0,0] neg_hi:[0,0,0]\n" \
  "ds_read_b128 v[246:249], v1 offset:16384\n" \
  "v_pk_fma_f32 v[48:49], v[228:229], v[54:55], v[48:49] op_sel:[0,0,0] op_sel_hi:[1,1,1] neg_lo:[0,0,0] neg_hi:[0,0,0]\n" \
  "v_fmac_f32 v46, v226, v81\n" \
  "ds_read_b128 v[226:229], v1 offset:15360\n" \
  "v_fmac_f32 v46, v225, v83\n" \
  "v_fmac_f32 v46, v224, v82\n" \
  "v_fmac_f32 v45, v223, v83\n" \
  "v_fmac_f32 v45, v222, v82\n" \
  "ds_read_b128 v[222:225], v1 offset:14336\n" \
  "s_waitcnt lgkmcnt(3)\n" \
  "v_fmac_f32 v43, v221, v75\n" \
  "v_fmac_f32 v42, v220, v75\n" \
  "v_fmac_f32 v40, v219, v69\n" \
  "v_fmac_f32 v40, v218, v71\n" \
  "ds_read_b128 v[218:221], v1 offset:13312\n" \
  "v_fmac_f32 v40, v217, v70\n" \
  "v_fmac_f32 v39, v216, v69\n" \
  "v_fmac_f32 v39, v215, v71\n" \
  "v_fmac_f32 v39, v214, v70\n" \
  "ds_read_b128 v[214:217], v1 offset:12288\n" \
  "v_fmac_f32 v68, v253, v38\n" \
  "v_fmac_f32 v68, v252, v22\n" \
  "v_fmac_f32 v67, v251, v38\n" \
  "v_fmac_f32 v66, v250, v38\n" \
  "ds_read_b128 v[250:253], v1 offset:11264\n" \
  "s_waitcnt lgkmcnt(3)\n" \
  "v_fmac_f32 v51, v249, v5\n" \
  "v_fmac_f32 v4, v248, v56\n" \
  "v_fmac_f32 v4, v247, v50\n" \
  "v_fmac_f32 v86, v246, v44\n" \
  "ds_read_b128 v[246:249], v1 offset:10240\n" \
  "v_fmac_f32 v85, v229, v41\n" \
  "v_fmac_f32 v84, v228, v38\n" \
  "v_pk_fma_f32 v[42:43], v[226:227], v[76:77], v[42:43] op_sel:[1,1,0] op_sel_hi:[0,0,1] neg_lo:[0,0,0] neg_hi:[0,0,0]\n" \
  "ds_read_b128 v[226:229], v1 offset:9216\n" \
  "v_pk_fma_f32 v[42:43], v[224:225], v[76:77], v[42:43] op_sel:[0,0,0] op_sel_hi:[1,1,1] neg_lo:[0,0,0] neg_hi:[0,0,0]\n" \
  "v_pk_fma_f32 v[30:31], v[222:223], v[76:77], v[30:31] op_sel:[0,0,0] op_sel_hi:[1,1,1] neg_lo:[0,0,0] neg_hi:[0,0,0]\n" \
  "ds_read_b128 v[222:225], v1 offset:8192\n" \
  "s_waitcnt lgkmcnt(3)\n" \
  "v_pk_fma_f32 v[30:31], v[220:221], v[82:83], v[30:31] op_sel:[0,0,0] op_sel_hi:[1,1,1] neg_lo:[0,0,0] neg_hi:[0,0,0]\n" \
  "v_pk_fma_f32 v[30:31], v[218:219], v[58:59], v[30:31] op_sel:[0,0,0] op_sel_hi:[1,1,1] neg_lo:[0,0,0] neg_hi:[0,0,0]\n" \
  "ds_read_b128 v[218:221], v1 offset:7168\n" \
  "v_pk_fma_f32 v[28:29], v[216:217], v[80:81], v[28:29] op_sel:[0,0,0] op_sel_hi:[1,1,1] neg_lo:[0,0,0] neg_hi:[0,0,0]\n" \
  "v_pk_fma_f32 v[28:29], v[214:215], v[74:75], v[28:29] op_sel:[0,0,0] op_sel_hi:[1,1,1] neg_lo:[0,0,0] neg_hi:[0,0,0]\n" \
  "ds_read_b128 v[214:217], v1 offset:6144\n" \
  "v_pk_fma_f32 v[28:29], v[252:253], v[56:57], v[28:29] op_sel:[0,0,0] op_sel_hi:[1,1,1] neg_lo:[0,0,0] neg_hi:[0,0,0]\n" \
  "v_pk_fma_f32 v[26:27], v[250:251], v[78:79], v[26:27] op_sel:[0,0,0] op_sel_hi:[1,1,1] neg_lo:[0,0,0] neg_hi:[0,0,0]\n" \
  "ds_read_b128 v[250:253], v1 offset:5120\n" \
  "s_waitcnt lgkmcnt(3)\n" \
// ... 3852 lines not shown
```

Before: 538.5 million.

## Hoist LDS ring preload out of ADMM loop and hold accumulator operands across solves

In the steady-state ADMM loop, the generator now finds a fixed point of the LDS ring contents across the loop back edge. It preloads those quads once before the loop label, so the per-iteration ds_read_b128 issues and their waits go away. It also reserves spare VGPRs (V_TT..V_END plus one accumulator temp pair) to keep factor values read from AGPRs that are used twice in the forward and backward solves, which removes repeated v_accvgpr_read instructions. The cost is one fewer rotating AGPR-temp pair, which shortens the accumulator-read lookahead. Correctness relies on the ring contents being identical at the top of every iteration.

```diff
diff --git a/robobee3d_amd/asmgen.py b/robobee3d_amd/asmgen.py
--- a/robobee3d_amd/asmgen.py
+++ b/robobee3d_amd/asmgen.py
@@ -313,8 +313,12 @@
 
 class Fetcher:
 
-    def __init__(self, e, la=3):
+    def __init__(self, e, la=3, hold=None, ring_in=None):
         self.e, self.la = e, la
+        self.hold, self.ring_in, self.ring_out = hold, ring_in, None
+        self.kept = []
+        self.natp = N_ATP if hold is None else N_ATP - 1
+        assert la <= self.natp and (hold is None or not set(hold) & set(range(V_AT, V_AT + 2 * self.natp)))
         self.nds = 0
         self.waited = -1
         self.lds_ahead = int(os.environ.get("UMPC_ASM_LDS_AHEAD", "12" if NRING == 4 else "20"))
@@ -326,6 +330,9 @@
         inst_of = [None] * n
         insts = []
         slots = [None] * NRING
+        for sl, qd in enumerate(self.ring_in or ()):
+            insts.append(dict(quad=qd, first=-1, last=-1, slot=sl, prev=None, issued=-1))
+            slots[sl] = sl
         for i, op in enumerate(ops):
             if op["src"] and op["src"][0] == "L":
                 qd = op["src"][1] // 4
@@ -346,15 +353,43 @@
             it["issued"] = self.nds
             self.nds += 1
 
-        next_inst = 0
+        self.ring_out = [insts[k]["quad"] if k is not None else None for k in slots]
+        held = {}
+        if self.hold:
+            free, users = sorted(self.hold), {}
+            for i, op in enumerate(ops):
+                if op.get("keep") and op["src"] and op["src"][0] in ("A", "A2"):
+                    users.setdefault(frozenset(op["src"][1:]), []).append(i)
+            for i1, i2 in sorted(u for u in users.values() if len(u) == 2):
+                a = ops[i1]["src"]
+                if a[0] == "A":
+                    if not free:
+                        continue
+                    r = free.pop(0)
+                else:
+                    r = next((q for q in free if q % 2 == 0 and q + 1 in free), None)
+                    if r is None:
+                        continue
+                    free.remove(r)
+                    free.remove(r + 1)
+                held[i1] = (r, True, False)
+                held[i2] = (r, False, ops[i2]["src"][1:] != a[1:])
+                self.kept += [(r + k, ag) for k, ag in enumerate(a[1:])]
+        next_inst = len(self.ring_in or ())
         atemp = {}
         next_acc = 0
         acc_rr = 0
         for i in range(n):
             while next_acc < n and next_acc < i + self.la:
                 op = ops[next_acc]
-                if op["src"] and op["src"][0] in ("A", "A2"):
-                    t = V_AT + 2 * (acc_rr % N_ATP)
+                if next_acc in held:
+                    t, fetch, swap = held[next_acc]
+                    if fetch:
+                        for k, ag in enumerate(op["src"][1:]):
+                            e("v_accvgpr_read_b32", "v%d" % (t + k), "a%d" % ag)
+                    atemp[next_acc] = ("v[%d:%d]" % (t, t + 1), 1, 0) if swap else t
+                elif op["src"] and op["src"][0] in ("A", "A2"):
+                    t = V_AT + 2 * (acc_rr % self.natp)
                     acc_rr += 1
                     e("v_accvgpr_read_b32", "v%d" % t, "a%d" % op["src"][1])
                     if op["src"][0] == "A2":
@@ -431,7 +466,8 @@
     return out
 
 
-def body(e, s, first, capture, plan, lv=False, delta_in_w=False, qzero=frozenset(), lzero=frozenset(), dy3_in_w=False):
+def body(e, s, first, capture, plan, lv=False, delta_in_w=False, qzero=frozenset(), lzero=frozenset(), dy3_in_w=False,
+         hold=None, ring_in=None):
     nx, nc, nk = s.nx, s.nc, s.nk
     neq = 2 * s.N * symbolic.NY
     xs, zs, xinv, zinv = slot_maps(s)
@@ -451,11 +487,11 @@
     v = lambda n: "v%d" % n
     sA, sO, sS, sRi, sRh = ("s%d" % r for r in (S_ALPHA, S_OMA, S_SIGMA, S_RINV, S_RHO))
     ptr = "s[%d:%d]" % (S_P2, S_P2 + 1)
-    f = Fetcher(e)
+    f = Fetcher(e, hold=hold, ring_in=ring_in)
     ops = []
 
-    def op(src, fn, w=(), r=()):
-        ops.append(dict(src=src, emit=fn, w=frozenset(w), r=frozenset(r)))
+    def op(src, fn, w=(), r=(), keep=False):
+        ops.append(dict(src=src, emit=fn, w=frozenset(w), r=frozenset(r), keep=keep))
 
     assert NVZ == neq and not (lv and first)
 
@@ -528,7 +564,7 @@
                        w=(wreg(d),), r=(wreg(d), wreg(sr)))
                 else:
                     op(src, lambda t, d=d, sr=sr: e("v_fmac_f32", W(d), v(t), W(sr)),
-                       w=(wreg(d),), r=(wreg(d), wreg(sr)))
+                       w=(wreg(d),), r=(wreg(d), wreg(sr)), keep=True)
                 continue
             (d0, s0_, j0), (d1, s1_, j1) = g
             rd, r0, r1 = wreg(d0), wreg(s0_), wreg(s1_)
@@ -546,7 +582,8 @@
                    pk(e, "v_pk_fma_f32", rd, [("v[%d:%d]" % (t, t + 1), lsel[0], lsel[1]), srcp, _vp(rd)], [0, 0, 0]), **rw)
             else:
                 src = ("A2", A_L + lpos[j0] - NLDS, A_L + lpos[j1] - NLDS)
-                op(src, lambda t, rd=rd, srcp=srcp: pk(e, "v_pk_fma_f32", rd, [_vp(t), srcp, _vp(rd)], [0, 0, 0]), **rw)
+                op(src, lambda t, rd=rd, srcp=srcp:
+                   pk(e, "v_pk_fma_f32", rd, [t if isinstance(t, tuple) else _vp(t), srcp, _vp(rd)], [0, 0, 0]), keep=True, **rw)
 
     solve_ops(fwd)
     kof = {wreg(k): k for k in range(nk)}
@@ -638,6 +675,7 @@
             e("global_store_dword", "v0", t2, ptr)
             if first:
                 _adv(e, S_P2)
+    return f
 
 
 def program(N=3, perm=None):
diff --git a/robobee3d_amd/asmstep.py b/robobee3d_amd/asmstep.py
--- a/robobee3d_amd/asmstep.py
+++ b/robobee3d_amd/asmstep.py
@@ -66,6 +66,7 @@
 OPT_NT = os.environ.get("UMPC_ASM_NT", "1")
 NT_PTRS = ("state", "ctrl", "ref", "out", "stats")
 A_SPARE, N_SPARE_D = 246, 9
+OPT_TURN = os.environ.get("UMPC_ASM_TURNAROUND", "1") == "1"
 OPT_WS_ST = os.environ.get("UMPC_ASM_WS_ST", "nt")
 OPT_WS_LD = os.environ.get("UMPC_ASM_WS_LD", "nt")
 
@@ -251,13 +252,15 @@
 
 
 class StepGen:
-    def __init__(self, N=3, perm=None, quad=False):
+    def __init__(self, N=3, perm=None, quad=False, turnaround=None):
         self.st = Struct(N, perm)
         self.s = self.st.s
         self.e = Emit()
         self.pool = Pool(self.e)
         self.lab = 20
         self.quad = quad
+        self.turnaround = (OPT_TURN if turnaround is None else turnaround) and not quad
+        self.turn = None
         self.nt = "0" if quad else OPT_NT
 
     def label(self):
@@ -1081,6 +1084,7 @@
         e("s_waitcnt", "vmcnt(0) lgkmcnt(0)")
         plan = st.plan
         zk = dict(qzero=st.qzero, lzero=st.lzero) if OPT_ZSKIP else {}
+        self.admm_span = [len(e.ins), None]
         asmgen.body(e, s, first=True, capture=True, plan=plan, delta_in_w=True, **zk)
         if self.quad:
             from . import asmquad
@@ -1091,6 +1095,7 @@
             e("label", lab6)
         else:
             self._admm_rest(plan, zk)
+        self.admm_span[1] = len(e.ins)
         for i in range(st.neq):
             pool.free(V_Z + st.zs[i], kill=True)
         pool.free_range(246, 10)
@@ -1105,8 +1110,24 @@
         e("s_sub_i32", sg(S_CNT), sg(S_ITERS), 1)
         e("s_cmp_lt_i32", sg(S_CNT), 1)
         e("s_cbranch_scc1", lab6 + "f")
+        kw = dict(first=False, capture=False, plan=plan, lv=True, dy3_in_w=True, **zk)
+        if self.turnaround:
+            kw["hold"] = list(range(asmgen.V_TT, asmgen.V_END)) + [asmgen.V_AT + 2 * (asmgen.N_ATP - 1) + h for h in range(2)]
+            ring = None
+            for _ in range(8):
+                out = asmgen.body(Emit(), s, ring_in=ring, **kw).ring_out
+                if out == ring:
+                    break
+                ring = out
+            assert out == ring and None not in ring, "the LDS ring does not settle across the loop's back edge"
+            kw["ring_in"] = ring
+            for sl, qd in enumerate(ring):
+                e("ds_read_b128", "v[%d:%d]" % (asmgen.ring_base(sl), asmgen.ring_base(sl) + 3), "v1", qd * 1024)
+            e("s_waitcnt", "lgkmcnt(0)")
         e("label", lab7)
-        asmgen.body(e, s, first=False, capture=False, plan=plan, lv=True, dy3_in_w=True, **zk)
+        i0 = len(e.ins)
+        f = asmgen.body(e, s, **kw)
+        self.turn = dict(span=(i0, len(e.ins)), kept=f.kept, ring=kw.get("ring_in"))
         e("s_sub_i32", sg(S_CNT), sg(S_CNT), 1)
         e("s_cmp_gt_i32", sg(S_CNT), 0)
         e("s_cbranch_scc1", lab7 + "b")
diff --git a/robobee3d_amd/csrc/umpc_step_asm.h b/robobee3d_amd/csrc/umpc_step_asm.h
--- a/robobee3d_amd/csrc/umpc_step_asm.h
+++ b/robobee3d_amd/csrc/umpc_step_asm.h
@@ -4765,6 +4765,13 @@
   "s_sub_i32 s14, s11, 1\n" \
   "s_cmp_lt_i32 s14, 1\n" \
   "s_cbranch_scc1 30f\n" \
+  "ds_read_b128 v[214:217], v1 offset:0\n" \
+  "ds_read_b128 v[218:221], v1 offset:1024\n" \
+  "ds_read_b128 v[222:225], v1 offset:2048\n" \
+  "ds_read_b128 v[226:229], v1 offset:3072\n" \
+  "ds_read_b128 v[246:249], v1 offset:4096\n" \
+  "ds_read_b128 v[250:253], v1 offset:5120\n" \
+  "s_waitcnt lgkmcnt(0)\n" \
   "29:\n" \
   "v_accvgpr_read_b32 v230, a137\n" \
   "v_accvgpr_read_b32 v231, a138\n" \
@@ -4773,37 +4780,37 @@
   "v_accvgpr_read_b32 v234, a140\n" \
   "v_accvgpr_read_b32 v235, a141\n" \
   "v_pk_fma_f32 v[2:3], s[24:25], v[88:89], v[230:231] op_sel:[0,0,0] op_sel_hi:[0,1,1] neg_lo:[0,0,1] neg_hi:[0,0,1]\n" \
-  "v_accvgpr_read_b32 v236, a143\n" \
-  "v_accvgpr_read_b32 v237, a144\n" \
+  "v_accvgpr_read_b32 v230, a143\n" \
+  "v_accvgpr_read_b32 v231, a144\n" \
   "v_pk_fma_f32 v[4:5], s[24:25], v[90:91], v[232:233] op_sel:[0,0,0] op_sel_hi:[0,1,1] neg_lo:[0,0,1] neg_hi:[0,0,1]\n" \
-  "v_accvgpr_read_b32 v230, a145\n" \
-  "v_accvgpr_read_b32 v231, a148\n" \
+  "v_accvgpr_read_b32 v232, a145\n" \
+  "v_accvgpr_read_b32 v233, a148\n" \
   "v_pk_fma_f32 v[6:7], s[24:25], v[92:93], v[234:235] op_sel:[0,0,0] op_sel_hi:[0,1,1] neg_lo:[0,0,1] neg_hi:[0,0,1]\n" \
-  "v_accvgpr_read_b32 v232, a146\n" \
-  "v_accvgpr_read_b32 v233, a147\n" \
-  "v_pk_fma_f32 v[8:9], s[24:25], v[94:95], v[236:237] op_sel:[0,0,0] op_sel_hi:[0,1,1] neg_lo:[0,0,1] neg_hi:[0,0,1]\n" \
-  "v_accvgpr_read_b32 v234, a149\n" \
-  "v_accvgpr_read_b32 v235, a150\n" \
-  "v_pk_fma_f32 v[10:11], s[24:25], v[96:97], v[230:231] op_sel:[0,0,0] op_sel_hi:[0,1,1] neg_lo:[0,0,1] neg_hi:[0,0,1]\n" \
-  "v_accvgpr_read_b32 v236, a151\n" \
-  "v_accvgpr_read_b32 v237, a154\n" \
-  "v_pk_fma_f32 v[12:13], s[24:25], v[98:99], v[232:233] op_sel:[0,0,0] op_sel_hi:[0,1,1] neg_lo:[0,0,1] neg_hi:[0,0,1]\n" \
-  "v_accvgpr_read_b32 v230, a152\n" \
-  "v_accvgpr_read_b32 v231, a153\n" \
-  "v_pk_fma_f32 v[14:15], s[24:25], v[100:101], v[234:235] op_sel:[0,0,0] op_sel_hi:[0,1,1] neg_lo:[0,0,1] neg_hi:[0,0,1]\n" \
-  "v_accvgpr_read_b32 v232, a155\n" \
-  "v_accvgpr_read_b32 v233, a156\n" \
-  "v_pk_fma_f32 v[16:17], s[24:25], v[102:103], v[236:237] op_sel:[0,0,0] op_sel_hi:[0,1,1] neg_lo:[0,0,1] neg_hi:[0,0,1]\n" \
-  "v_accvgpr_read_b32 v234, a157\n" \
-  "v_pk_fma_f32 v[18:19], s[24:25], v[104:105], v[230:231] op_sel:[0,0,0] op_sel_hi:[0,1,1] neg_lo:[0,0,1] neg_hi:[0,0,1]\n" \
-  "v_pk_fma_f32 v[20:21], s[24:25], v[106:107], v[232:233] op_sel:[0,0,0] op_sel_hi:[0,1,1] neg_lo:[0,0,1] neg_hi:[0,0,1]\n" \
-  "v_accvgpr_read_b32 v236, a161\n" \
-  "v_accvgpr_read_b32 v237, a162\n" \
+  "v_accvgpr_read_b32 v234, a146\n" \
+  "v_accvgpr_read_b32 v235, a147\n" \
+  "v_pk_fma_f32 v[8:9], s[24:25], v[94:95], v[230:231] op_sel:[0,0,0] op_sel_hi:[0,1,1] neg_lo:[0,0,1] neg_hi:[0,0,1]\n" \
+  "v_accvgpr_read_b32 v230, a149\n" \
+  "v_accvgpr_read_b32 v231, a150\n" \
+  "v_pk_fma_f32 v[10:11], s[24:25], v[96:97], v[232:233] op_sel:[0,0,0] op_sel_hi:[0,1,1] neg_lo:[0,0,1] neg_hi:[0,0,1]\n" \
+  "v_accvgpr_read_b32 v232, a151\n" \
+  "v_accvgpr_read_b32 v233, a154\n" \
+  "v_pk_fma_f32 v[12:13], s[24:25], v[98:99], v[234:235] op_sel:[0,0,0] op_sel_hi:[0,1,1] neg_lo:[0,0,1] neg_hi:[0,0,1]\n" \
+  "v_accvgpr_read_b32 v234, a152\n" \
+  "v_accvgpr_read_b32 v235, a153\n" \
+  "v_pk_fma_f32 v[14:15], s[24:25], v[100:101], v[230:231] op_sel:[0,0,0] op_sel_hi:[0,1,1] neg_lo:[0,0,1] neg_hi:[0,0,1]\n" \
+  "v_accvgpr_read_b32 v230, a155\n" \
+  "v_accvgpr_read_b32 v231, a156\n" \
+  "v_pk_fma_f32 v[16:17], s[24:25], v[102:103], v[232:233] op_sel:[0,0,0] op_sel_hi:[0,1,1] neg_lo:[0,0,1] neg_hi:[0,0,1]\n" \
+  "v_accvgpr_read_b32 v232, a157\n" \
+  "v_pk_fma_f32 v[18:19], s[24:25], v[104:105], v[234:235] op_sel:[0,0,0] op_sel_hi:[0,1,1] neg_lo:[0,0,1] neg_hi:[0,0,1]\n" \
+  "v_pk_fma_f32 v[20:21], s[24:25], v[106:107], v[230:231] op_sel:[0,0,0] op_sel_hi:[0,1,1] neg_lo:[0,0,1] neg_hi:[0,0,1]\n" \
+  "v_accvgpr_read_b32 v234, a161\n" \
+  "v_accvgpr_read_b32 v235, a162\n" \
   "v_pk_mul_f32 v[22:23], s[24:25], v[108:109] op_sel:[0,0] op_sel_hi:[0,1] neg_lo:[0,0] neg_hi:[0,0]\n" \
-  "v_sub_f32 v22, v22, v234\n" \
+  "v_sub_f32 v22, v22, v232\n" \
   "v_accvgpr_read_b32 v230, a163\n" \
   "v_pk_mul_f32 v[24:25], s[24:25], v[110:111] op_sel:[0,0] op_sel_hi:[0,1] neg_lo:[0,0] neg_hi:[0,0]\n" \
-  "v_pk_fma_f32 v[26:27], s[24:25], v[112:113], v[236:237] op_sel:[0,0,0] op_sel_hi:[0,1,1] neg_lo:[0,0,1] neg_hi:[0,0,1]\n" \
+  "v_pk_fma_f32 v[26:27], s[24:25], v[112:113], v[234:235] op_sel:[0,0,0] op_sel_hi:[0,1,1] neg_lo:[0,0,1] neg_hi:[0,0,1]\n" \
   "v_accvgpr_read_b32 v232, a167\n" \
   "v_accvgpr_read_b32 v233, a168\n" \
   "v_pk_mul_f32 v[28:29], s[24:25], v[114:115] op_sel:[0,0] op_sel_hi:[0,1] neg_lo:[0,0] neg_hi:[0,0]\n" \
@@ -4817,57 +4824,50 @@
   "v_pk_mul_f32 v[38:39], s[24:25], v[124:125] op_sel:[0,0] op_sel_hi:[0,1] neg_lo:[0,0] neg_hi:[0,0]\n" \
   "v_pk_mul_f32 v[40:41], s[24:25], v[126:127] op_sel:[0,0] op_sel_hi:[0,1] neg_lo:[0,0] neg_hi:[0,0]\n" \
   "v_pk_mul_f32 v[42:43], s[24:25], v[128:129] op_sel:[0,0] op_sel_hi:[0,1] neg_lo:[0,0] neg_hi:[0,0]\n" \
-  "v_accvgpr_read_b32 v236, a182\n" \
-  "v_accvgpr_read_b32 v237, a183\n" \
+  "v_accvgpr_read_b32 v230, a182\n" \
+  "v_accvgpr_read_b32 v231, a183\n" \
   "v_pk_mul_f32 v[44:45], s[24:25], v[130:131] op_sel:[0,0] op_sel_hi:[0,1] neg_lo:[0,0] neg_hi:[0,0]\n" \
-  "v_accvgpr_read_b32 v230, a184\n" \
-  "v_accvgpr_read_b32 v231, a187\n" \
+  "v_accvgpr_read_b32 v232, a184\n" \
+  "v_accvgpr_read_b32 v233, a187\n" \
   "v_mul_f32 v46, s24, v132\n" \
-  "v_accvgpr_read_b32 v232, a185\n" \
-  "v_accvgpr_read_b32 v233, a186\n" \
-  "v_pk_fma_f32 v[48:49], s[26:27], v[134:135], v[236:237] op_sel:[0,0,0] op_sel_hi:[0,1,1] neg_lo:[1,0,0] neg_hi:[1,0,0]\n" \
-  "ds_read_b128 v[214:217], v1 offset:0\n" \
-  "v_pk_fma_f32 v[50:51], s[26:27], v[136:137], v[230:231] op_sel:[0,0,0] op_sel_hi:[0,1,1] neg_lo:[1,0,0] neg_hi:[1,0,0]\n" \
-  "v_pk_fma_f32 v[52:53], s[26:27], v[138:139], v[232:233] op_sel:[0,0,0] op_sel_hi:[0,1,1] neg_lo:[1,0,0] neg_hi:[1,0,0]\n" \
-  "ds_read_b128 v[218:221], v1 offset:1024\n" \
+  "v_accvgpr_read_b32 v234, a185\n" \
+  "v_accvgpr_read_b32 v235, a186\n" \
+  "v_pk_fma_f32 v[48:49], s[26:27], v[134:135], v[230:231] op_sel:[0,0,0] op_sel_hi:[0,1,1] neg_lo:[1,0,0] neg_hi:[1,0,0]\n" \
+  "v_pk_fma_f32 v[50:51], s[26:27], v[136:137], v[232:233] op_sel:[0,0,0] op_sel_hi:[0,1,1] neg_lo:[1,0,0] neg_hi:[1,0,0]\n" \
+  "v_pk_fma_f32 v[52:53], s[26:27], v[138:139], v[234:235] op_sel:[0,0,0] op_sel_hi:[0,1,1] neg_lo:[1,0,0] neg_hi:[1,0,0]\n" \
   "v_pk_mul_f32 v[54:55], s[26:27], v[140:141] op_sel:[0,0] op_sel_hi:[0,1] neg_lo:[1,0] neg_hi:[1,0]\n" \
   "v_pk_mul_f32 v[56:57], s[26:27], v[142:143] op_sel:[0,0] op_sel_hi:[0,1] neg_lo:[1,0] neg_hi:[1,0]\n" \
-  "ds_read_b128 v[222:225], v1 offset:2048\n" \
   "v_pk_mul_f32 v[58:59], s[26:27], v[144:145] op_sel:[0,0] op_sel_hi:[0,1] neg_lo:[1,0] neg_hi:[1,0]\n" \
   "v_pk_mul_f32 v[60:61], s[26:27], v[146:147] op_sel:[0,0] op_sel_hi:[0,1] neg_lo:[1,0] neg_hi:[1,0]\n" \
-  "v_accvgpr_read_b32 v234, a200\n" \
-  "v_accvgpr_read_b32 v235, a201\n" \
-  "ds_read_b128 v[226:229], v1 offset:3072\n" \
+  "v_accvgpr_read_b32 v230, a200\n" \
+  "v_accvgpr_read_b32 v231, a201\n" \
   "v_pk_mul_f32 v[62:63], s[26:27], v[148:149] op_sel:[0,0] op_sel_hi:[0,1] neg_lo:[1,0] neg_hi:[1,0]\n" \
-  "v_accvgpr_read_b32 v236, a202\n" \
-  "v_accvgpr_read_b32 v237, a205\n" \
+  "v_accvgpr_read_b32 v232, a202\n" \
+  "v_accvgpr_read_b32 v233, a205\n" \
   "v_pk_mul_f32 v[64:65], s[26:27], v[150:151] op_sel:[0,0] op_sel_hi:[0,1] neg_lo:[1,0] neg_hi:[1,0]\n" \
-  "v_accvgpr_read_b32 v230, a203\n" \
-  "v_accvgpr_read_b32 v231, a204\n" \
-  "ds_read_b128 v[246:249], v1 offset:4096\n" \
-  "v_pk_fma_f32 v[66:67], s[26:27], v[152:153], v[234:235] op_sel:[0,0,0] op_sel_hi:[0,1,1] neg_lo:[1,0,0] neg_hi:[1,0,0]\n" \
-  "v_accvgpr_read_b32 v232, a206\n" \
-  "v_accvgpr_read_b32 v233, a207\n" \
-  "v_pk_fma_f32 v[68:69], s[26:27], v[154:155], v[236:237] op_sel:[0,0,0] op_sel_hi:[0,1,1] neg_lo:[1,0,0] neg_hi:[1,0,0]\n" \
-  "v_accvgpr_read_b32 v234, a208\n" \
-  "ds_read_b128 v[250:253], v1 offset:5120\n" \
-  "v_pk_fma_f32 v[70:71], s[26:27], v[156:157], v[230:231] op_sel:[0,0,0] op_sel_hi:[0,1,1] neg_lo:[1,0,0] neg_hi:[1,0,0]\n" \
-  "v_pk_fma_f32 v[72:73], s[26:27], v[158:159], v[232:233] op_sel:[0,0,0] op_sel_hi:[0,1,1] neg_lo:[1,0,0] neg_hi:[1,0,0]\n" \
+  "v_accvgpr_read_b32 v234, a203\n" \
+  "v_accvgpr_read_b32 v235, a204\n" \
+  "v_pk_fma_f32 v[66:67], s[26:27], v[152:153], v[230:231] op_sel:[0,0,0] op_sel_hi:[0,1,1] neg_lo:[1,0,0] neg_hi:[1,0,0]\n" \
+  "v_accvgpr_read_b32 v230, a206\n" \
+  "v_accvgpr_read_b32 v231, a207\n" \
+  "v_pk_fma_f32 v[68:69], s[26:27], v[154:155], v[232:233] op_sel:[0,0,0] op_sel_hi:[0,1,1] neg_lo:[1,0,0] neg_hi:[1,0,0]\n" \
+  "v_accvgpr_read_b32 v232, a208\n" \
+  "v_pk_fma_f32 v[70:71], s[26:27], v[156:157], v[234:235] op_sel:[0,0,0] op_sel_hi:[0,1,1] neg_lo:[1,0,0] neg_hi:[1,0,0]\n" \
+  "v_pk_fma_f32 v[72:73], s[26:27], v[158:159], v[230:231] op_sel:[0,0,0] op_sel_hi:[0,1,1] neg_lo:[1,0,0] neg_hi:[1,0,0]\n" \
   "v_pk_mul_f32 v[74:75], s[26:27], v[160:161] op_sel:[0,0] op_sel_hi:[0,1] neg_lo:[1,0] neg_hi:[1,0]\n" \
-  "v_add_f32 v74, v74, v234\n" \
-  "v_accvgpr_read_b32 v236, a214\n" \
+  "v_add_f32 v74, v74, v232\n" \
+  "v_accvgpr_read_b32 v234, a214\n" \
   "v_pk_mul_f32 v[76:77], s[26:27], v[162:163] op_sel:[0,0] op_sel_hi:[0,1] neg_lo:[1,0] neg_hi:[1,0]\n" \
   "v_pk_mul_f32 v[78:79], s[26:27], v[164:165] op_sel:[0,0] op_sel_hi:[0,1] neg_lo:[1,0] neg_hi:[1,0]\n" \
   "v_accvgpr_read_b32 v230, a227\n" \
   "v_pk_mul_f32 v[80:81], s[26:27], v[166:167] op_sel:[0,0] op_sel_hi:[0,1] neg_lo:[1,0] neg_hi:[1,0]\n" \
-  "v_add_f32 v80, v80, v236\n" \
+  "v_add_f32 v80, v80, v234\n" \
   "v_accvgpr_read_b32 v232, a228\n" \
   "v_pk_mul_f32 v[82:83], s[26:27], v[168:169] op_sel:[0,0] op_sel_hi:[0,1] neg_lo:[1,0] neg_hi:[1,0]\n" \
   "v_accvgpr_read_b32 v234, a229\n" \
   "v_fma_f32 v84, -v230, v170, v210\n" \
   "v_fma_f32 v85, -v232, v171, v211\n" \
   "v_fma_f32 v86, -v234, v172, v212\n" \
-  "s_waitcnt lgkmcnt(3)\n" \
   "v_pk_fma_f32 v[60:61], v[214:215], v[14:15], v[60:61] op_sel:[0,0,0] op_sel_hi:[1,1,1] neg_lo:[0,0,0] neg_hi:[0,0,0]\n" \
   "v_pk_fma_f32 v[62:63], v[216:217], v[16:17], v[62:63] op_sel:[0,0,0] op_sel_hi:[1,1,1] neg_lo:[0,0,0] neg_hi:[0,0,0]\n" \
   "ds_read_b128 v[214:217], v1 offset:6144\n" \
@@ -4877,7 +4877,6 @@
   "v_pk_fma_f32 v[54:55], v[222:223], v[2:3], v[54:55] op_sel:[0,0,0] op_sel_hi:[1,1,1] neg_lo:[0,0,0] neg_hi:[0,0,0]\n" \
   "v_pk_fma_f32 v[60:61], v[224:225], v[8:9], v[60:61] op_sel:[0,0,0] op_sel_hi:[1,1,1] neg_lo:[0,0,0] neg_hi:[0,0,0]\n" \
   "ds_read_b128 v[222:225], v1 offset:8192\n" \
-  "s_waitcnt lgkmcnt(3)\n" \
   "v_pk_fma_f32 v[54:55], v[226:227], v[8:9], v[54:55] op_sel:[0,0,0] op_sel_hi:[1,1,1] neg_lo:[0,0,0] neg_hi:[0,0,0]\n" \
   "v_pk_fma_f32 v[62:63], v[228:229], v[10:11], v[62:63] op_sel:[0,0,0] op_sel_hi:[1,1,1] neg_lo:[0,0,0] neg_hi:[0,0,0]\n" \
   "ds_read_b128 v[226:229], v1 offset:9216\n" \
@@ -5053,190 +5052,180 @@
   "v_accvgpr_read_b32 v236, a38\n" \
   "v_accvgpr_read_b32 v237, a39\n" \
   "v_fmac_f32 v81, v209, v6\n" \
-  "v_accvgpr_read_b32 v230, a40\n" \
+  "v_accvgpr_read_b32 v238, a40\n" \
   "v_pk_fma_f32 v[76:77], v[254:255], v[6:7], v[76:77] op_sel:[0,0,0] op_sel_hi:[1,1,1] neg_lo:[0,0,0] neg_hi:[0,0,0]\n" \
-  "v_accvgpr_read_b32 v232, a41\n" \
+  "v_accvgpr_read_b32 v239, a41\n" \
   "v_pk_fma_f32 v[76:77], v[236:237], v[6:7], v[76:77] op_sel:[0,1,0] op_sel_hi:[1,0,1] neg_lo:[0,0,0] neg_hi:[0,0,0]\n" \
-  "v_accvgpr_read_b32 v234, a42\n" \
-  "v_fmac_f32 v69, v230, v7\n" \
-  "v_accvgpr_read_b32 v236, a43\n" \
-  "v_fmac_f32 v75, v232, v7\n" \
-  "v_accvgpr_read_b32 v230, a44\n" \
-  "v_fmac_f32 v81, v234, v7\n" \
-  "v_accvgpr_read_b32 v232, a45\n" \
-  "v_fmac_f32 v76, v236, v69\n" \
-  "v_accvgpr_read_b32 v234, a46\n" \
-  "v_fmac_f32 v77, v230, v69\n" \
-  "v_accvgpr_read_b32 v236, a47\n" \
-  "v_fmac_f32 v75, v232, v69\n" \
+  "v_accvgpr_read_b32 v240, a42\n" \
+  "v_fmac_f32 v69, v238, v7\n" \
+  "v_accvgpr_read_b32 v241, a43\n" \
+  "v_fmac_f32 v75, v239, v7\n" \
+  "v_accvgpr_read_b32 v242, a44\n" \
+  "v_fmac_f32 v81, v240, v7\n" \
+  "v_accvgpr_read_b32 v243, a45\n" \
+  "v_fmac_f32 v76, v241, v69\n" \
+  "v_accvgpr_read_b32 v244, a46\n" \
+  "v_fmac_f32 v77, v242, v69\n" \
+  "v_accvgpr_read_b32 v245, a47\n" \
+  "v_fmac_f32 v75, v243, v69\n" \
   "v_accvgpr_read_b32 v230, a48\n" \
-  "v_fmac_f32 v81, v234, v69\n" \
+  "v_fmac_f32 v81, v244, v69\n" \
   "v_accvgpr_read_b32 v232, a49\n" \
-  "v_fmac_f32 v77, v236, v76\n" \
+  "v_fmac_f32 v77, v245, v76\n" \
   "v_accvgpr_read_b32 v234, a50\n" \
   "v_fmac_f32 v75, v230, v76\n" \
-  "v_accvgpr_read_b32 v236, a51\n" \
+  "v_accvgpr_read_b32 v230, a51\n" \
   "v_fmac_f32 v81, v232, v76\n" \
-  "v_accvgpr_read_b32 v230, a52\n" \
+  "v_accvgpr_read_b32 v232, a52\n" \
   "v_fmac_f32 v75, v234, v77\n" \
-  "v_accvgpr_read_b32 v232, a62\n" \
-  "v_accvgpr_read_b32 v233, a63\n" \
-  "v_fmac_f32 v81, v236, v77\n" \
-  "v_accvgpr_read_b32 v234, a64\n" \
-  "v_accvgpr_read_b32 v235, a129\n" \
-  "v_fmac_f32 v81, v230, v75\n" \
-  "v_accvgpr_read_b32 v236, a130\n" \
-  "v_accvgpr_read_b32 v237, a131\n" \
-  "v_pk_mul_f32 v[2:3], v[2:3], v[232:233] op_sel:[0,0] op_sel_hi:[1,1] neg_lo:[0,0] neg_hi:[0,0]\n" \
-  "v_accvgpr_read_b32 v230, a65\n" \
-  "v_accvgpr_read_b32 v231, a66\n" \
-  "v_pk_mul_f32 v[4:5], v[4:5], v[234:235] op_sel:[0,0] op_sel_hi:[1,1] neg_lo:[0,0] neg_hi:[0,0]\n" \
-  "v_accvgpr_read_b32 v232, a67\n" \
-  "v_accvgpr_read_b32 v233, a70\n" \
-  "v_pk_mul_f32 v[6:7], v[6:7], v[236:237] op_sel:[0,0] op_sel_hi:[1,1] neg_lo:[0,0] neg_hi:[0,0]\n" \
-  "v_accvgpr_read_b32 v234, a68\n" \
-  "v_accvgpr_read_b32 v235, a69\n" \
-  "v_pk_mul_f32 v[8:9], v[8:9], v[230:231] op_sel:[0,0] op_sel_hi:[1,1] neg_lo:[0,0] neg_hi:[0,0]\n" \
-  "v_accvgpr_read_b32 v236, a53\n" \
-  "v_accvgpr_read_b32 v237, a54\n" \
-  "v_pk_mul_f32 v[10:11], v[10:11], v[232:233] op_sel:[0,0] op_sel_hi:[1,1] neg_lo:[0,0] neg_hi:[0,0]\n" \
+  "v_accvgpr_read_b32 v234, a62\n" \
+  "v_accvgpr_read_b32 v235, a63\n" \
+  "v_fmac_f32 v81, v230, v77\n" \
+  "v_accvgpr_read_b32 v230, a64\n" \
+  "v_accvgpr_read_b32 v231, a129\n" \
+  "v_fmac_f32 v81, v232, v75\n" \
+  "v_accvgpr_read_b32 v232, a130\n" \
+  "v_accvgpr_read_b32 v233, a131\n" \
+  "v_pk_mul_f32 v[2:3], v[2:3], v[234:235] op_sel:[0,0] op_sel_hi:[1,1] neg_lo:[0,0] neg_hi:[0,0]\n" \
+  "v_accvgpr_read_b32 v234, a65\n" \
+  "v_accvgpr_read_b32 v235, a66\n" \
+  "v_pk_mul_f32 v[4:5], v[4:5], v[230:231] op_sel:[0,0] op_sel_hi:[1,1] neg_lo:[0,0] neg_hi:[0,0]\n" \
+  "v_accvgpr_read_b32 v230, a67\n" \
+  "v_accvgpr_read_b32 v231, a70\n" \
+  "v_pk_mul_f32 v[6:7], v[6:7], v[232:233] op_sel:[0,0] op_sel_hi:[1,1] neg_lo:[0,0] neg_hi:[0,0]\n" \
+  "v_accvgpr_read_b32 v232, a68\n" \
+  "v_accvgpr_read_b32 v233, a69\n" \
+  "v_pk_mul_f32 v[8:9], v[8:9], v[234:235] op_sel:[0,0] op_sel_hi:[1,1] neg_lo:[0,0] neg_hi:[0,0]\n" \
+  "v_accvgpr_read_b32 v234, a53\n" \
+  "v_accvgpr_read_b32 v235, a54\n" \
+  "v_pk_mul_f32 v[10:11], v[10:11], v[230:231] op_sel:[0,0] op_sel_hi:[1,1] neg_lo:[0,0] neg_hi:[0,0]\n" \
   "v_accvgpr_read_b32 v230, a55\n" \
   "v_accvgpr_read_b32 v231, a58\n" \
-  "v_pk_mul_f32 v[12:13], v[12:13], v[234:235] op_sel:[0,0] op_sel_hi:[1,1] neg_lo:[0,0] neg_hi:[0,0]\n" \
+  "v_pk_mul_f32 v[12:13], v[12:13], v[232:233] op_sel:[0,0] op_sel_hi:[1,1] neg_lo:[0,0] neg_hi:[0,0]\n" \
   "v_accvgpr_read_b32 v232, a56\n" \
   "v_accvgpr_read_b32 v233, a57\n" \
-  "v_pk_mul_f32 v[14:15], v[14:15], v[236:237] op_sel:[0,0] op_sel_hi:[1,1] neg_lo:[0,0] neg_hi:[0,0]\n" \
+  "v_pk_mul_f32 v[14:15], v[14:15], v[234:235] op_sel:[0,0] op_sel_hi:[1,1] neg_lo:[0,0] neg_hi:[0,0]\n" \
   "v_accvgpr_read_b32 v234, a94\n" \
   "v_accvgpr_read_b32 v235, a97\n" \
   "v_pk_mul_f32 v[16:17], v[16:17], v[230:231] op_sel:[0,0] op_sel_hi:[1,1] neg_lo:[0,0] neg_hi:[0,0]\n" \
-  "v_accvgpr_read_b32 v236, a100\n" \
-  "v_accvgpr_read_b32 v237, a109\n" \
+  "v_accvgpr_read_b32 v230, a100\n" \
+  "v_accvgpr_read_b32 v231, a109\n" \
   "v_pk_mul_f32 v[18:19], v[18:19], v[232:233] op_sel:[0,0] op_sel_hi:[1,1] neg_lo:[0,0] neg_hi:[0,0]\n" \
-  "v_accvgpr_read_b32 v230, a105\n" \
-  "v_accvgpr_read_b32 v231, a107\n" \
+  "v_accvgpr_read_b32 v232, a105\n" \
+  "v_accvgpr_read_b32 v233, a107\n" \
   "v_pk_mul_f32 v[20:21], v[20:21], v[234:235] op_sel:[0,0] op_sel_hi:[1,1] neg_lo:[0,0] neg_hi:[0,0]\n" \
-  "v_accvgpr_read_b32 v232, a92\n" \
-  "v_accvgpr_read_b32 v233, a95\n" \
-  "v_pk_mul_f32 v[22:23], v[22:23], v[236:237] op_sel:[0,0] op_sel_hi:[1,1] neg_lo:[0,0] neg_hi:[0,0]\n" \
-  "v_accvgpr_read_b32 v234, a98\n" \
-  "v_accvgpr_read_b32 v235, a103\n" \
-  "v_pk_mul_f32 v[24:25], v[24:25], v[230:231] op_sel:[0,0] op_sel_hi:[1,1] neg_lo:[0,0] neg_hi:[0,0]\n" \
-  "v_accvgpr_read_b32 v236, a101\n" \
-  "v_accvgpr_read_b32 v237, a102\n" \
-  "v_pk_mul_f32 v[26:27], v[26:27], v[232:233] op_sel:[0,0] op_sel_hi:[1,1] neg_lo:[0,0] neg_hi:[0,0]\n" \
-  "v_accvgpr_read_b32 v230, a71\n" \
-  "v_accvgpr_read_b32 v231, a72\n" \
-  "v_pk_mul_f32 v[28:29], v[28:29], v[234:235] op_sel:[0,0] op_sel_hi:[1,1] neg_lo:[0,0] neg_hi:[0,0]\n" \
-  "v_accvgpr_read_b32 v232, a73\n" \
-  "v_accvgpr_read_b32 v233, a76\n" \
-  "v_pk_mul_f32 v[30:31], v[30:31], v[236:237] op_sel:[0,0] op_sel_hi:[1,1] neg_lo:[0,0] neg_hi:[0,0]\n" \
-  "v_accvgpr_read_b32 v234, a74\n" \
-  "v_accvgpr_read_b32 v235, a75\n" \
-  "v_pk_mul_f32 v[32:33], v[32:33], v[230:231] op_sel:[0,0] op_sel_hi:[1,1] neg_lo:[0,0] neg_hi:[0,0]\n" \
-  "v_accvgpr_read_b32 v236, a118\n" \
-  "v_accvgpr_read_b32 v237, a113\n" \
-  "v_pk_mul_f32 v[34:35], v[34:35], v[232:233] op_sel:[0,0] op_sel_hi:[1,1] neg_lo:[0,0] neg_hi:[0,0]\n" \
+  "v_accvgpr_read_b32 v234, a92\n" \
+  "v_accvgpr_read_b32 v235, a95\n" \
+  "v_pk_mul_f32 v[22:23], v[22:23], v[230:231] op_sel:[0,0] op_sel_hi:[1,1] neg_lo:[0,0] neg_hi:[0,0]\n" \
+  "v_accvgpr_read_b32 v230, a98\n" \
+  "v_accvgpr_read_b32 v231, a103\n" \
+  "v_pk_mul_f32 v[24:25], v[24:25], v[232:233] op_sel:[0,0] op_sel_hi:[1,1] neg_lo:[0,0] neg_hi:[0,0]\n" \
+  "v_accvgpr_read_b32 v232, a101\n" \
+  "v_accvgpr_read_b32 v233, a102\n" \
+  "v_pk_mul_f32 v[26:27], v[26:27], v[234:235] op_sel:[0,0] op_sel_hi:[1,1] neg_lo:[0,0] neg_hi:[0,0]\n" \
+  "v_accvgpr_read_b32 v234, a71\n" \
+  "v_accvgpr_read_b32 v235, a72\n" \
+  "v_pk_mul_f32 v[28:29], v[28:29], v[230:231] op_sel:[0,0] op_sel_hi:[1,1] neg_lo:[0,0] neg_hi:[0,0]\n" \
+  "v_accvgpr_read_b32 v230, a73\n" \
+  "v_accvgpr_read_b32 v231, a76\n" \
+  "v_pk_mul_f32 v[30:31], v[30:31], v[232:233] op_sel:[0,0] op_sel_hi:[1,1] neg_lo:[0,0] neg_hi:[0,0]\n" \
+  "v_accvgpr_read_b32 v232, a74\n" \
+  "v_accvgpr_read_b32 v233, a75\n" \
+  "v_pk_mul_f32 v[32:33], v[32:33], v[234:235] op_sel:[0,0] op_sel_hi:[1,1] neg_lo:[0,0] neg_hi:[0,0]\n" \
+  "v_accvgpr_read_b32 v234, a118\n" \
+  "v_accvgpr_read_b32 v235, a113\n" \
+  "v_pk_mul_f32 v[34:35], v[34:35], v[230:231] op_sel:[0,0] op_sel_hi:[1,1] neg_lo:[0,0] neg_hi:[0,0]\n" \
   "v_accvgpr_read_b32 v230, a114\n" \
   "v_accvgpr_read_b32 v231, a119\n" \
-  "v_pk_mul_f32 v[36:37], v[36:37], v[234:235] op_sel:[0,0] op_sel_hi:[1,1] neg_lo:[0,0] neg_hi:[0,0]\n" \
+  "v_pk_mul_f32 v[36:37], v[36:37], v[232:233] op_sel:[0,0] op_sel_hi:[1,1] neg_lo:[0,0] neg_hi:[0,0]\n" \
   "v_accvgpr_read_b32 v232, a115\n" \
   "v_accvgpr_read_b32 v233, a116\n" \
-  "v_pk_mul_f32 v[38:39], v[38:39], v[236:237] op_sel:[0,0] op_sel_hi:[1,1] neg_lo:[0,0] neg_hi:[0,0]\n" \
+  "v_pk_mul_f32 v[38:39], v[38:39], v[234:235] op_sel:[0,0] op_sel_hi:[1,1] neg_lo:[0,0] neg_hi:[0,0]\n" \
   "v_accvgpr_read_b32 v234, a117\n" \
   "v_accvgpr_read_b32 v235, a123\n" \
   "v_pk_mul_f32 v[40:41], v[40:41], v[230:231] op_sel:[0,0] op_sel_hi:[1,1] neg_lo:[0,0] neg_hi:[0,0]\n" \
-  "v_accvgpr_read_b32 v236, a124\n" \
+  "v_accvgpr_read_b32 v230, a124\n" \
   "v_pk_mul_f32 v[42:43], v[42:43], v[232:233] op_sel:[0,0] op_sel_hi:[1,1] neg_lo:[0,0] neg_hi:[0,0]\n" \
-  "v_accvgpr_read_b32 v230, a77\n" \
-  "v_accvgpr_read_b32 v231, a78\n" \
+  "v_accvgpr_read_b32 v232, a77\n" \
+  "v_accvgpr_read_b32 v233, a78\n" \
   "v_pk_mul_f32 v[44:45], v[44:45], v[234:235] op_sel:[0,0] op_sel_hi:[1,1] neg_lo:[0,0] neg_hi:[0,0]\n" \
-  "v_accvgpr_read_b32 v232, a79\n" \
-  "v_accvgpr_read_b32 v233, a82\n" \
-  "v_mul_f32 v46, v236, v46\n" \
-  "v_accvgpr_read_b32 v234, a80\n" \
-  "v_accvgpr_read_b32 v235, a81\n" \
-  "v_pk_mul_f32 v[48:49], v[48:49], v[230:231] op_sel:[0,0] op_sel_hi:[1,1] neg_lo:[0,0] neg_hi:[0,0]\n" \
-  "v_accvgpr_read_b32 v236, a93\n" \
-  "v_accvgpr_read_b32 v237, a96\n" \
-  "v_pk_mul_f32 v[50:51], v[50:51], v[232:233] op_sel:[0,0] op_sel_hi:[1,1] neg_lo:[0,0] neg_hi:[0,0]\n" \
-  "v_accvgpr_read_b32 v230, a99\n" \
-  "v_accvgpr_read_b32 v231, a108\n" \
-  "v_pk_mul_f32 v[52:53], v[52:53], v[234:235] op_sel:[0,0] op_sel_hi:[1,1] neg_lo:[0,0] neg_hi:[0,0]\n" \
-  "v_accvgpr_read_b32 v232, a104\n" \
-  "v_accvgpr_read_b32 v233, a106\n" \
-  "v_pk_mul_f32 v[54:55], v[54:55], v[236:237] op_sel:[0,0] op_sel_hi:[1,1] neg_lo:[0,0] neg_hi:[0,0]\n" \
-  "v_accvgpr_read_b32 v234, a83\n" \
-  "v_accvgpr_read_b32 v235, a84\n" \
-  "v_pk_mul_f32 v[56:57], v[56:57], v[230:231] op_sel:[0,0] op_sel_hi:[1,1] neg_lo:[0,0] neg_hi:[0,0]\n" \
-  "v_accvgpr_read_b32 v236, a85\n" \
-  "v_accvgpr_read_b32 v237, a88\n" \
-  "v_pk_mul_f32 v[58:59], v[58:59], v[232:233] op_sel:[0,0] op_sel_hi:[1,1] neg_lo:[0,0] neg_hi:[0,0]\n" \
+  "v_accvgpr_read_b32 v234, a79\n" \
+  "v_accvgpr_read_b32 v235, a82\n" \
+  "v_mul_f32 v46, v230, v46\n" \
+  "v_accvgpr_read_b32 v230, a80\n" \
+  "v_accvgpr_read_b32 v231, a81\n" \
+  "v_pk_mul_f32 v[48:49], v[48:49], v[232:233] op_sel:[0,0] op_sel_hi:[1,1] neg_lo:[0,0] neg_hi:[0,0]\n" \
+  "v_accvgpr_read_b32 v232, a93\n" \
+  "v_accvgpr_read_b32 v233, a96\n" \
+  "v_pk_mul_f32 v[50:51], v[50:51], v[234:235] op_sel:[0,0] op_sel_hi:[1,1] neg_lo:[0,0] neg_hi:[0,0]\n" \
+  "v_accvgpr_read_b32 v234, a99\n" \
+  "v_accvgpr_read_b32 v235, a108\n" \
+  "v_pk_mul_f32 v[52:53], v[52:53], v[230:231] op_sel:[0,0] op_sel_hi:[1,1] neg_lo:[0,0] neg_hi:[0,0]\n" \
+  "v_accvgpr_read_b32 v230, a104\n" \
+  "v_accvgpr_read_b32 v231, a106\n" \
+  "v_pk_mul_f32 v[54:55], v[54:55], v[232:233] op_sel:[0,0] op_sel_hi:[1,1] neg_lo:[0,0] neg_hi:[0,0]\n" \
+  "v_accvgpr_read_b32 v232, a83\n" \
+  "v_accvgpr_read_b32 v233, a84\n" \
+  "v_pk_mul_f32 v[56:57], v[56:57], v[234:235] op_sel:[0,0] op_sel_hi:[1,1] neg_lo:[0,0] neg_hi:[0,0]\n" \
+  "v_accvgpr_read_b32 v234, a85\n" \
+  "v_accvgpr_read_b32 v235, a88\n" \
+  "v_pk_mul_f32 v[58:59], v[58:59], v[230:231] op_sel:[0,0] op_sel_hi:[1,1] neg_lo:[0,0] neg_hi:[0,0]\n" \
   "v_accvgpr_read_b32 v230, a86\n" \
   "v_accvgpr_read_b32 v231, a87\n" \
-  "v_pk_mul_f32 v[60:61], v[60:61], v[234:235] op_sel:[0,0] op_sel_hi:[1,1] neg_lo:[0,0] neg_hi:[0,0]\n" \
+  "v_pk_mul_f32 v[60:61], v[60:61], v[232:233] op_sel:[0,0] op_sel_hi:[1,1] neg_lo:[0,0] neg_hi:[0,0]\n" \
   "v_accvgpr_read_b32 v232, a89\n" \
   "v_accvgpr_read_b32 v233, a90\n" \
-  "v_pk_mul_f32 v[62:63], v[62:63], v[236:237] op_sel:[0,0] op_sel_hi:[1,1] neg_lo:[0,0] neg_hi:[0,0]\n" \
+  "v_pk_mul_f32 v[62:63], v[62:63], v[234:235] op_sel:[0,0] op_sel_hi:[1,1] neg_lo:[0,0] neg_hi:[0,0]\n" \
   "v_accvgpr_read_b32 v234, a91\n" \
   "v_accvgpr_read_b32 v235, a132\n" \
   "v_pk_mul_f32 v[64:65], v[64:65], v[230:231] op_sel:[0,0] op_sel_hi:[1,1] neg_lo:[0,0] neg_hi:[0,0]\n" \
-  "v_accvgpr_read_b32 v236, a125\n" \
-  "v_accvgpr_read_b32 v237, a127\n" \
+  "v_accvgpr_read_b32 v230, a125\n" \
+  "v_accvgpr_read_b32 v231, a127\n" \
   "v_pk_mul_f32 v[66:67], v[66:67], v[232:233] op_sel:[0,0] op_sel_hi:[1,1] neg_lo:[0,0] neg_hi:[0,0]\n" \
-  "v_accvgpr_read_b32 v230, a110\n" \
-  "v_accvgpr_read_b32 v231, a111\n" \
+  "v_accvgpr_read_b32 v232, a110\n" \
+  "v_accvgpr_read_b32 v233, a111\n" \
   "v_pk_mul_f32 v[68:69], v[68:69], v[234:235] op_sel:[0,0] op_sel_hi:[1,1] neg_lo:[0,0] neg_hi:[0,0]\n" \
-  "v_accvgpr_read_b32 v232, a112\n" \
-  "v_accvgpr_read_b32 v233, a135\n" \
-  "v_pk_mul_f32 v[70:71], v[70:71], v[236:237] op_sel:[0,0] op_sel_hi:[1,1] neg_lo:[0,0] neg_hi:[0,0]\n" \
-  "v_accvgpr_read_b32 v234, a133\n" \
-  "v_accvgpr_read_b32 v235, a134\n" \
-  "v_pk_mul_f32 v[72:73], v[72:73], v[230:231] op_sel:[0,0] op_sel_hi:[1,1] neg_lo:[0,0] neg_hi:[0,0]\n" \
-  "v_accvgpr_read_b32 v236, a120\n" \
-  "v_accvgpr_read_b32 v237, a121\n" \
-  "v_pk_mul_f32 v[74:75], v[74:75], v[232:233] op_sel:[0,0] op_sel_hi:[1,1] neg_lo:[0,0] neg_hi:[0,0]\n" \
-  "v_accvgpr_read_b32 v230, a122\n" \
-  "v_accvgpr_read_b32 v231, a136\n" \
-  "v_pk_mul_f32 v[76:77], v[76:77], v[234:235] op_sel:[0,0] op_sel_hi:[1,1] neg_lo:[0,0] neg_hi:[0,0]\n" \
-  "v_accvgpr_read_b32 v232, a126\n" \
-  "v_accvgpr_read_b32 v233, a128\n" \
-  "v_pk_mul_f32 v[78:79], v[78:79], v[236:237] op_sel:[0,0] op_sel_hi:[1,1] neg_lo:[0,0] neg_hi:[0,0]\n" \
-  "v_accvgpr_read_b32 v234, a59\n" \
-  "v_accvgpr_read_b32 v235, a60\n" \
-  "v_pk_mul_f32 v[80:81], v[80:81], v[230:231] op_sel:[0,0] op_sel_hi:[1,1] neg_lo:[0,0] neg_hi:[0,0]\n" \
-  "v_accvgpr_read_b32 v236, a61\n" \
-  "v_pk_mul_f32 v[82:83], v[82:83], v[232:233] op_sel:[0,0] op_sel_hi:[1,1] neg_lo:[0,0] neg_hi:[0,0]\n" \
+  "v_accvgpr_read_b32 v234, a112\n" \
+  "v_accvgpr_read_b32 v235, a135\n" \
+  "v_pk_mul_f32 v[70:71], v[70:71], v[230:231] op_sel:[0,0] op_sel_hi:[1,1] neg_lo:[0,0] neg_hi:[0,0]\n" \
+  "v_accvgpr_read_b32 v230, a133\n" \
+  "v_accvgpr_read_b32 v231, a134\n" \
+  "v_pk_mul_f32 v[72:73], v[72:73], v[232:233] op_sel:[0,0] op_sel_hi:[1,1] neg_lo:[0,0] neg_hi:[0,0]\n" \
+  "v_accvgpr_read_b32 v232, a120\n" \
+  "v_accvgpr_read_b32 v233, a121\n" \
+  "v_pk_mul_f32 v[74:75], v[74:75], v[234:235] op_sel:[0,0] op_sel_hi:[1,1] neg_lo:[0,0] neg_hi:[0,0]\n" \
+  "v_accvgpr_read_b32 v234, a122\n" \
+  "v_accvgpr_read_b32 v235, a136\n" \
+  "v_pk_mul_f32 v[76:77], v[76:77], v[230:231] op_sel:[0,0] op_sel_hi:[1,1] neg_lo:[0,0] neg_hi:[0,0]\n" \
+  "v_accvgpr_read_b32 v230, a126\n" \
+  "v_accvgpr_read_b32 v231, a128\n" \
+  "v_pk_mul_f32 v[78:79], v[78:79], v[232:233] op_sel:[0,0] op_sel_hi:[1,1] neg_lo:[0,0] neg_hi:[0,0]\n" \
+  "v_accvgpr_read_b32 v232, a59\n" \
+  "v_accvgpr_read_b32 v233, a60\n" \
+  "v_pk_mul_f32 v[80:81], v[80:81], v[234:235] op_sel:[0,0] op_sel_hi:[1,1] neg_lo:[0,0] neg_hi:[0,0]\n" \
+  "v_accvgpr_read_b32 v234, a61\n" \
+  "v_pk_mul_f32 v[82:83], v[82:83], v[230:231] op_sel:[0,0] op_sel_hi:[1,1] neg_lo:[0,0] neg_hi:[0,0]\n" \
   "v_accvgpr_read_b32 v230, a52\n" \
-  "v_pk_mul_f32 v[84:85], v[84:85], v[234:235] op_sel:[0,0] op_sel_hi:[1,1] neg_lo:[0,0] neg_hi:[0,0]\n" \
+  "v_pk_mul_f32 v[84:85], v[84:85], v[232:233] op_sel:[0,0] op_sel_hi:[1,1] neg_lo:[0,0] neg_hi:[0,0]\n" \
   "v_accvgpr_read_b32 v232, a51\n" \
-  "v_mul_f32 v86, v236, v86\n" \
+  "v_mul_f32 v86, v234, v86\n" \
   "v_accvgpr_read_b32 v234, a50\n" \
   "v_fmac_f32 v75, v230, v81\n" \
-  "v_accvgpr_read_b32 v236, a49\n" \
+  "v_accvgpr_read_b32 v230, a49\n" \
   "v_fmac_f32 v77, v232, v81\n" \
-  "v_accvgpr_read_b32 v230, a48\n" \
+  "v_accvgpr_read_b32 v232, a48\n" \
   "v_fmac_f32 v77, v234, v75\n" \
-  "v_accvgpr_read_b32 v232, a47\n" \
-  "v_fmac_f32 v76, v236, v81\n" \
-  "v_accvgpr_read_b32 v234, a46\n" \
-  "v_fmac_f32 v76, v230, v75\n" \
-  "v_accvgpr_read_b32 v236, a45\n" \
-  "v_fmac_f32 v76, v232, v77\n" \
-  "v_accvgpr_read_b32 v230, a44\n" \
-  "v_fmac_f32 v69, v234, v81\n" \
-  "v_accvgpr_read_b32 v232, a43\n" \
-  "v_fmac_f32 v69, v236, v75\n" \
-  "v_accvgpr_read_b32 v234, a42\n" \
-  "v_fmac_f32 v69, v230, v77\n" \
-  "v_accvgpr_read_b32 v236, a41\n" \
-  "v_fmac_f32 v69, v232, v76\n" \
-  "v_accvgpr_read_b32 v230, a40\n" \
-  "v_fmac_f32 v7, v234, v81\n" \
-  "v_accvgpr_read_b32 v232, a39\n" \
-  "v_accvgpr_read_b32 v233, a38\n" \
-  "v_fmac_f32 v7, v236, v75\n" \
-  "v_fmac_f32 v7, v230, v69\n" \
-  "v_pk_fma_f32 v[6:7], v[232:233], v[76:77], v[6:7] op_sel:[0,1,0] op_sel_hi:[1,0,1] neg_lo:[0,0,0] neg_hi:[0,0,0]\n" \
+  "v_fmac_f32 v76, v230, v81\n" \
+  "v_fmac_f32 v76, v232, v75\n" \
+  "v_fmac_f32 v76, v245, v77\n" \
+  "v_fmac_f32 v69, v244, v81\n" \
+  "v_fmac_f32 v69, v243, v75\n" \
+  "v_fmac_f32 v69, v242, v77\n" \
+  "v_fmac_f32 v69, v241, v76\n" \
+  "v_fmac_f32 v7, v240, v81\n" \
+  "v_fmac_f32 v7, v239, v75\n" \
+  "v_fmac_f32 v7, v238, v69\n" \
+  "v_pk_fma_f32 v[6:7], v[236:237], v[76:77], v[6:7] op_sel:[1,1,0] op_sel_hi:[0,0,1] neg_lo:[0,0,0] neg_hi:[0,0,0]\n" \
   "v_pk_fma_f32 v[6:7], v[254:255], v[76:77], v[6:7] op_sel:[0,0,0] op_sel_hi:[1,1,1] neg_lo:[0,0,0] neg_hi:[0,0,0]\n" \
   "v_fmac_f32 v6, v209, v81\n" \
   "v_fmac_f32 v6, v208, v75\n" \
```

After: 543.3 million, median of 6. Within noise of the previous version (+0.9%).
